# iKrishneel/fcn_object_detector

Hardware: AMD Instinct MI355X
Metric: frames/sec forward 448x448 @1 GPU; train imgs/sec @1/2/4/8 GPUs (higher is better)
Workload: dtype f32; 1 GPU; configs[1]: single-GPU forward, DetectNet GoogLeNet conv stack + coverage/bbox heads (graph of models/deploy.prototxt), batch=1, 448x448, random-init weights; global_batch=1, parallelism=replicas x1, frames_in_flight=4

## Files before the change

fcn_object_detector_amd/csrc/conv_fwd.hip:

```cpp
#include <cstddef>
#include <algorithm>
#include <mutex>
#include <unordered_map>
#include <type_traits>

#include "common.h"
#include "conv_common.h"

using namespace fcn;

namespace fcn {

const float* zero_page_for_current_device(int* rc) {
    static std::mutex mu;
    static const float* pages[64] = {nullptr};
    int dev = 0;
    *rc = 0;
    if (hipGetDevice(&dev) != hipSuccess || dev < 0 || dev >= 64) {
        *rc = set_err(FCN_E_STATE, "conv: no current device");
        return nullptr;
    }
    std::lock_guard<std::mutex> lock(mu);
    if (!pages[dev]) {
        void* ptr = nullptr;
// ... 813 lines not shown
    const bool out_f16 = (p.flags & FCN_CONV_OUT_F16) != 0;
    const bool half_out = (F16 && !out_f32) || (!F16 && out_f16);
    const bool vec = n + 3 < p.Cout && ((p.y_cstride | p.y_coffset) & 3) == 0 && ((p.y2_cstride | p.y2_coffset) & 3) == 0 &&
                     ((unsigned)(size_t)p.y & 15) == 0 && ((unsigned)(size_t)p.y2 & 15) == 0;
    const int wn_t = (4 * c4) / (32 * WTN), jt = ((4 * c4) / 32) % WTN, lc = (4 * c4) & 31;
    const float* lds_col = smem + (size_t)(wn_t * WAVES_K * WTM * WTN + jt) * 1024 + lc;
#pragma unroll 1
    for (int it = tid / C4; it < BM; it += C::NT / C4) {
        const int m = m0 + it;
        if (m >= p.M) break;
        const int wm_t = it / (32 * WTM), i_t = (it / 32) % WTM;
        const float* src = lds_col + (size_t)(wm_t * WAVES_N * WAVES_K * WTM * WTN + i_t * WTN) * 1024 + (it & 31) * 32;
        v4f v = *(const v4f*)src;
#pragma unroll
        for (int s = 1; s < WAVES_K; ++s) v += *(const v4f*)(src + (size_t)s * WTM * WTN * 1024);
#pragma unroll
        for (int e = 0; e < 4; ++e) v[e] += bias_v[e];
        const size_t o = (size_t)m * p.y_cstride + p.y_coffset + n;
        const size_t o2 = (size_t)m * p.y2_cstride + p.y2_coffset + n;
        if (half_out) {
            typedef f16_t v4h __attribute__((ext_vector_type(4)));
            f16_t* dst = reinterpret_cast<f16_t*>(p.y) + o;
            if (vec) {
                if (do_accum) { const v4h old = *(const v4h*)dst; for (int e = 0; e < 4; ++e) v[e] += (float)old[e]; }
                if (do_relu) for (int e = 0; e < 4; ++e) v[e] = fmaxf(v[e], 0.f);
                v4h h;
                for (int e = 0; e < 4; ++e) h[e] = (f16_t)v[e];
                *(v4h*)dst = h;
            } else {
                for (int e = 0; e < 4; ++e)
                    if (n + e < p.Cout) {
                        float t = v[e];
                        if (do_accum) t += (float)dst[e];
                        if (do_relu) t = fmaxf(t, 0.f);
                        dst[e] = (f16_t)t;
                    }
            }
        } else if (vec) {
            float* dst = p.y + o;
            if (do_accum) v += *(const v4f*)dst;
            if (do_relu) for (int e = 0; e < 4; ++e) v[e] = fmaxf(v[e], 0.f);
            if (do_mask) { const v4f a = *(const v4f*)(p.y2 + o2); for (int e = 0; e < 4; ++e) v[e] = a[e] > 0.f ? v[e] : 0.f; }
            *(v4f*)dst = v;
            if (do_sig2) {
                v4f sg;
                for (int e = 0; e < 4; ++e) sg[e] = 1.f / (1.f + expf(-v[e]));
                *(v4f*)(p.y2 + o2) = sg;
            }
        } else {
            for (int e = 0; e < 4; ++e)
                if (n + e < p.Cout) {
                    float t = v[e];
                    if (do_accum) t += p.y[o + e];
                    if (do_relu) t = fmaxf(t, 0.f);
                    if (do_mask) t = p.y2[o2 + e] > 0.f ? t : 0.f;
                    p.y[o + e] = t;
                    if (do_sig2) p.y2[o2 + e] = 1.f / (1.f + expf(-t));
                }
        }
    }
#ifdef FCN_CONV_STAMPS
    FCN_STAMP(5);
    wait_vmcnt<0>();
    FCN_STAMP(6);
    if (g_conv_stamps && (int)blockIdx.x < g_conv_stamps_cap && threadIdx.x == 0) {
        unsigned xcc = 0, hwid = 0;
        asm volatile("s_getreg_b32 %0, hwreg(HW_REG_XCC_ID)" : "=s"(xcc));
        asm volatile("s_getreg_b32 %0, hwreg(HW_REG_HW_ID)" : "=s"(hwid));
        g_conv_stamps[(size_t)blockIdx.x * kStampWords + 30] = xcc;
        g_conv_stamps[(size_t)blockIdx.x * kStampWords + 31] = hwid;
    }
#endif
}

__device__ __forceinline__ const GroupArgs& group_of(const GroupArgs& a) { return a; }
__device__ __forceinline__ const GroupArgs& group_of(const GroupArgsTail& a) { return a.g; }
#ifdef FCN_EXP_TAIL_NOLDS
constexpr int kTailLdsFloats = 0;
#else
constexpr int kTailLdsFloats = kTailRows * 32 + 4;
#endif

template <typename T, int WTM, int WTN, int WAVES_M, int WAVES_N, int WAVES_K, int BK, int NBUF, bool PF, bool TAIL = false>
__global__ __launch_bounds__((Cfg<WTM, WTN, WAVES_M, WAVES_N, WAVES_K, BK, NBUF, PF>::NT)) void conv_fwd_group(const int nprob, const int te0, const int te1, const int te2,
                                                                                  const int te3, const int te4, const int te5, const int te6,
                                                                                  const int te7, const int pool_wgs, const int snake,
                                                                                  const std::conditional_t<TAIL, GroupArgsTail, GroupArgs> a_) {
    __shared__ __attribute__((aligned(16))) float smem[Cfg<WTM, WTN, WAVES_M, WAVES_N, WAVES_K, BK, NBUF, PF>::LDS_FLOATS + (TAIL ? kTailLdsFloats : 0)];
    const GroupArgs& a = group_of(a_);
    typedef unsigned u32x16 __attribute__((ext_vector_type(16)));
    typedef unsigned u32x8 __attribute__((ext_vector_type(8)));
    typedef const GroupArgs __attribute__((address_space(4))) * karg_ptr;
    static_assert(alignof(GroupArgsTail) == alignof(GroupArgs) && offsetof(GroupArgsTail, g) == 0, "the group leads its tail");
    constexpr size_t kArgsOffset = (11 * sizeof(int) + alignof(GroupArgs) - 1) / alignof(GroupArgs) * alignof(GroupArgs);
    karg_ptr ka = (karg_ptr)((const char __attribute__((address_space(4)))*)__builtin_amdgcn_kernarg_segment_ptr() + kArgsOffset);
    const int head[1 + kMaxGroup] = {nprob, te0, te1, te2, te3, te4, te5, te6, te7};
    static_assert(kMaxGroup == 8, "the tile prefix travels as eight scalar kernel arguments");
    const int pool_first = pool_wgs > 0 ? pool_wgs : 0;
    if ((int)blockIdx.x < pool_first || (pool_wgs < 0 && (int)blockIdx.x >= te7)) {
        const int w = pool_wgs < 0 ? (int)blockIdx.x - te7 : (int)blockIdx.x;
        if (w < a.pool[0].wg_end) pool_body<T, Cfg<WTM, WTN, WAVES_M, WAVES_N, WAVES_K, BK, NBUF, PF>::NT>(a.pool[0], w);
        else pool_body<T, Cfg<WTM, WTN, WAVES_M, WAVES_N, WAVES_K, BK, NBUF, PF>::NT>(a.pool[1], w - a.pool[0].wg_end);
        return;
    }
    int pos = blockIdx.x;
    if (snake > 0) {
        const int sh = snake & 255, rounds = snake >> 8;
        const int r = pos >> sh, j = pos & ((1 << sh) - 1);
        if (r > 0 && r < rounds - 1 && ((rounds - 1 - r) & 1)) pos = (r << sh) + ((1 << sh) - 1 - j);
    }
    int tile = pos - pool_first;
    if (snake == (int)0x80000000) {
        const int x = pos & 7, sl = pos >> 3, q = te7 >> 3, r = te7 & 7;
        tile = x * q + (x < r ? x : r) + sl;
    } else if (snake < 0) {
        tile += snake;
        tile += tile < 0 ? te7 : 0;
    }
    int pi = 0, begin = 0;
#pragma unroll
    for (int i = 0; i < kMaxGroup - 1; ++i) {
        const int end_i = head[1 + i];
        const bool past = i + 1 < nprob && tile >= end_i;
        pi += past ? 1 : 0;
        begin = past ? end_i : begin;
    }
    u32x16 ra, rb;
    u32x8 rc;
    pi = __builtin_amdgcn_readfirstlane(pi);
    begin = __builtin_amdgcn_readfirstlane(begin);
    const ConvP __attribute__((address_space(4)))* pbase = &ka->p[pi];
    asm volatile("s_load_dwordx16 %0, %3, 0x0\n\ts_load_dwordx16 %1, %3, 0x40\n\ts_load_dwordx8 %2, %3, 0x80\n\ts_waitcnt lgkmcnt(0)"
                 : "=&s"(ra), "=&s"(rb), "=&s"(rc)
                 : "s"(pbase)
                 : "memory");
    ConvP prob;
    __builtin_memcpy((char*)&prob, &ra, 64);
    __builtin_memcpy((char*)&prob + 64, &rb, 64);
    __builtin_memcpy((char*)&prob + 128, &rc, 32);
    if constexpr (TAIL) {
        tail_kptr tp = (tail_kptr)((const char __attribute__((address_space(4)))*)ka + offsetof(GroupArgsTail, tail));
        conv_body<T, WTM, WTN, WAVES_M, WAVES_N, WAVES_K, BK, NBUF, PF, true>(prob, tile - begin, smem, tp);
    } else {
        conv_body<T, WTM, WTN, WAVES_M, WAVES_N, WAVES_K, BK, NBUF, PF>(prob, tile - begin, smem);
    }
}

template <typename T, int WTM, int WTN, int WAVES_M, int WAVES_N, int WAVES_K, int BK, int NBUF, bool PF>
__global__ __launch_bounds__((Cfg<WTM, WTN, WAVES_M, WAVES_N, WAVES_K, BK, NBUF, PF>::NT)) void conv_fwd_one(ConvP p) {
    __shared__ __attribute__((aligned(16))) float smem[Cfg<WTM, WTN, WAVES_M, WAVES_N, WAVES_K, BK, NBUF, PF>::LDS_FLOATS];
    conv_body<T, WTM, WTN, WAVES_M, WAVES_N, WAVES_K, BK, NBUF, PF>(p, blockIdx.x, smem);
}

constexpr int kD7Th = 8, kD7Tw = 32;
constexpr int kD7Ph = 2 * kD7Th + 5, kD7Pw = 2 * kD7Tw + 6;
constexpr int kD7RowF = kD7Pw * 3;
constexpr int kD7PatchF = kD7Ph * kD7RowF;
constexpr int kD7WRowF = 22, kD7WPitchF = 7 * kD7WRowF;
constexpr int kD7WOff = (kD7PatchF + 3) / 4 * 4;
constexpr int kD7EpiPitch = 68;
constexpr int kD7StageF = kD7WOff + 64 * kD7WPitchF;
constexpr int kD7EpiF = 4 * 2 * 32 * kD7EpiPitch;
constexpr int kD7LdsBytes = (kD7StageF > kD7EpiF ? kD7StageF : kD7EpiF) * 4;
constexpr int kD7Threads = 256;
static_assert(kD7LdsBytes <= 80 * 1024, "first-layer kernel: two workgroups per CU");

__global__ __launch_bounds__(kD7Threads) void conv_first7_kernel(const ConvP p) {
#if defined(__HIP_DEVICE_COMPILE__)
    __shared__ __attribute__((aligned(16))) float smem[kD7LdsBytes / 4];
    const int tid = threadIdx.x, lane = tid & 63, wave = __builtin_amdgcn_readfirstlane(tid >> 6);
    FCN_STAMP(0);
    const int tiles_x = (p.OW + kD7Tw - 1) / kD7Tw, tiles_y = (p.OH + kD7Th - 1) / kD7Th;
    int t = blockIdx.x;
    const int tx = t % tiles_x;
    t /= tiles_x;
    const int ty = t % tiles_y, n = t / tiles_y;
    const int oy0 = ty * kD7Th, ox0 = tx * kD7Tw;
    const int iy0 = 2 * oy0 - 3, ix0 = 2 * ox0 - 3;
    const v4f zero4 = {0.f, 0.f, 0.f, 0.f};
    constexpr int PI = (kD7Ph * kD7Pw + kD7Threads - 1) / kD7Threads, WI = (64 * 49 + kD7Threads - 1) / kD7Threads;
    v4f px[PI], wv[WI];
    const float* xn = p.x + (size_t)n * p.H * p.W * 4;
#pragma unroll
    for (int i = 0; i < PI; ++i) {
        const int s = tid + kD7Threads * i;
        const int pr = s / kD7Pw, pc = s - pr * kD7Pw;
        const int iy = iy0 + pr, ix = ix0 + pc;
        const bool ok = s < kD7Ph * kD7Pw && (unsigned)iy < (unsigned)p.H && (unsigned)ix < (unsigned)p.W;
        px[i] = ok ? *reinterpret_cast<const v4f*>(xn + ((size_t)iy * p.W + ix) * 4) : zero4;
    }
#pragma unroll
    for (int i = 0; i < WI; ++i) {
        const int tp = tid + kD7Threads * i;
        wv[i] = tp < p.Cout * 49 ? *reinterpret_cast<const v4f*>(p.w + (size_t)tp * 4) : zero4;
    }
#pragma unroll
    for (int i = 0; i < PI; ++i) {
        const int s = tid + kD7Threads * i;
        if (s < kD7Ph * kD7Pw) {
            float* d = smem + s * 3;
            d[0] = px[i][0]; d[1] = px[i][1]; d[2] = px[i][2];
        }
    }
#pragma unroll
    for (int i = 0; i < WI; ++i) {
        const int tp = tid + kD7Threads * i;
        if (tp < 64 * 49) {
            const int co = tp / 49, rq = tp - co * 49;
            const int r = rq / 7, q = rq - r * 7;
            float* d = smem + kD7WOff + co * kD7WPitchF + r * kD7WRowF + q * 3;
            d[0] = wv[i][0]; d[1] = wv[i][1]; d[2] = wv[i][2];
        }
    }
    for (int i = tid; i < 64 * 7; i += kD7Threads) smem[kD7WOff + i * kD7WRowF + 21] = 0.f;
    const int c4 = (lane & 15) * 4;
    const v4f bias_v = (p.bias && c4 < p.Cout) ? *reinterpret_cast<const v4f*>(p.bias + c4) : zero4;
    FCN_STAMP(1);
    const int nl = lane & 31, h = lane >> 5;
    const float* a_base = smem + (4 * wave) * kD7RowF + 6 * nl + h;
    const float* b_base = smem + kD7WOff + nl * kD7WPitchF + h;
    typedef float v16f __attribute__((ext_vector_type(16)));
    v16f acc[2][2];
#pragma unroll
    for (int i = 0; i < 2; ++i)
#pragma unroll
        for (int j = 0; j < 2; ++j)
#pragma unroll
            for (int e = 0; e < 16; ++e) acc[i][j][e] = 0.f;
    __syncthreads();
    FCN_STAMP(2);
    auto frag = [&](const int step, float (&a)[2], float (&b)[2]) {
        const int r = step / 11, j = step - 11 * r;
#pragma unroll
        for (int mt = 0; mt < 2; ++mt) a[mt] = a_base[(2 * mt + r) * kD7RowF + 2 * j];
#pragma unroll
        for (int nt = 0; nt < 2; ++nt) b[nt] = b_base[nt * 32 * kD7WPitchF + r * kD7WRowF + 2 * j];
    };
    float fa[3][2], fb[3][2];
    frag(0, fa[0], fb[0]);
    frag(1, fa[1], fb[1]);
#pragma unroll
    for (int step = 0; step < 77; ++step) {
        if (step + 2 < 77) frag(step + 2, fa[(step + 2) % 3], fb[(step + 2) % 3]);
        __builtin_amdgcn_sched_barrier(0);
#pragma unroll
        for (int mt = 0; mt < 2; ++mt)
#pragma unroll
            for (int nt = 0; nt < 2; ++nt)
                acc[mt][nt] = __builtin_amdgcn_mfma_f32_32x32x2f32(fa[step % 3][mt], fb[step % 3][nt], acc[mt][nt], 0, 0, 0);
    }
    FCN_STAMP(3);
    __syncthreads();
    float* epi = smem + wave * (2 * 32 * kD7EpiPitch);
#pragma unroll
    for (int mt = 0; mt < 2; ++mt)
#pragma unroll
        for (int nt = 0; nt < 2; ++nt)
#pragma unroll
            for (int v = 0; v < 16; ++v) epi[(mt * 32 + (v & 3) + 8 * (v >> 2) + 4 * h) * kD7EpiPitch + nl + 32 * nt] = acc[mt][nt][v];
    asm volatile("s_waitcnt lgkmcnt(0)" ::: "memory");
    __builtin_amdgcn_sched_barrier(0);
    const bool do_relu = (p.flags & FCN_CONV_RELU) != 0;
#pragma unroll
    for (int mt = 0; mt < 2; ++mt) {
        const int oy = oy0 + 2 * wave + mt;
        float* yrow = p.y + ((size_t)(n * p.OH + oy) * p.OW + ox0) * p.y_cstride + p.y_coffset + c4;
#pragma unroll
        for (int i = 0; i < 8; ++i) {
            const int ox = (lane >> 4) + 4 * i;
            v4f v = *reinterpret_cast<const v4f*>(epi + (mt * 32 + ox) * kD7EpiPitch + c4) + bias_v;
            if (do_relu)
#pragma unroll
                for (int e = 0; e < 4; ++e) v[e] = fmaxf(v[e], 0.f);
            if (oy < p.OH && ox0 + ox < p.OW && c4 < p.Cout) *reinterpret_cast<v4f*>(yrow + (size_t)ox * p.y_cstride) = v;
        }
    }
#ifdef FCN_CONV_STAMPS
    FCN_STAMP(5);
    wait_vmcnt<0>();
    FCN_STAMP(6);
#endif
#endif
}

constexpr int kH7PatchSlots = (kD7Ph * kD7Pw + 63) / 64 * 64;
constexpr int kH7EpiOff = 2 * kH7PatchSlots * 16;
constexpr int kH7EpiPitch = 144;
constexpr int kH7LdsBytes = kH7EpiOff + 4 * 64 * kH7EpiPitch;
static_assert(kH7LdsBytes <= 160 * 1024, "half-float first-layer kernel: LDS image");

__global__ __launch_bounds__(kD7Threads) void conv_first7_f16_kernel(const ConvP p, const int ntiles) {
#if defined(__HIP_DEVICE_COMPILE__)
    __shared__ __attribute__((aligned(16))) char smem[kH7LdsBytes];
    const int tid = threadIdx.x, lane = tid & 63, wave = __builtin_amdgcn_readfirstlane(tid >> 6);
    const int tiles_x = (p.OW + kD7Tw - 1) / kD7Tw, tiles_y = (p.OH + kD7Th - 1) / kD7Th;
    const f16_t* xh = reinterpret_cast<const f16_t*>(p.x);
    const f16_t* wh = reinterpret_cast<const f16_t*>(p.w);
    f16_t* yh = reinterpret_cast<f16_t*>(p.y);
    const v4f zero4 = {0.f, 0.f, 0.f, 0.f};
    constexpr int PI = (kD7Ph * kD7Pw + kD7Threads - 1) / kD7Threads;
    auto fetch_patch = [&](const int tile, v4f (&px)[PI]) {
        int t = tile;
        const int tx = t % tiles_x;
        t /= tiles_x;
        const int ty = t % tiles_y, n = t / tiles_y;
        const int iy0 = 2 * ty * kD7Th - 3, ix0 = 2 * tx * kD7Tw - 3;
// ... 557 lines not shown
    }
    return best;
}

int plan_tiles_cfg(int cfg, ConvP* ps, int n) {
    if (cfg == kDot1x1Cfg) {
        if (!dot1x1_ok(ps, n)) return -2;
        for (int i = 0; i < n; ++i) {
            ps[i].tiles_m = cdiv(ps[0].M, kDotPx);
            ps[i].tiles_n = 1;
            ps[i].tiles_n_magic = 0;
            ps[i].lean_chunks = 0;
            ps[i].tile_end = ps[i].tiles_m;
        }
        return ps[0].tiles_m;
    }
    if (cfg == kFirst7Cfg) {
        if (n != 1 || !(first7_ok(ps[0]) || first7_f16_ok(ps[0]))) return -2;
        ps[0].tiles_m = ps[0].N * cdiv(ps[0].OH, kD7Th) * cdiv(ps[0].OW, kD7Tw);
        ps[0].tiles_n = 1;
        ps[0].tiles_n_magic = 0;
        ps[0].lean_chunks = 0;
        ps[0].tile_end = ps[0].tiles_m;
        return ps[0].tiles_m;
    }
    if (is_stream_cfg(cfg)) {
        const StreamCfgInfo sc = stream_cfg_info(cfg - kStreamCfg0);
        int total = 0;
        for (int i = 0; i < n; ++i) {
            ConvP& q = ps[i];
            const long long xb = (((long long)q.N * q.H * q.W - 1) * q.x_cstride + q.Cin) * 2, wb = (long long)q.Cout * q.K * 2;
            const long long yb = (((long long)q.M - 1) * q.y_cstride + q.y_coffset + q.Cout) * 2;
            const int k = q.kh, pw = q.W + 2 * q.pad;
            const int wraps = (sc.bm - 2 + q.W) / q.W;
            const int rows = sc.bm - 1 + 2 * q.pad * wraps + 2 * q.pad + 1;
            if ((q.flags & ~FCN_CONV_RELU) != FCN_CONV_F16 || (q.Cout | q.y_cstride | q.y_coffset) % 8 != 0 || ((uintptr_t)q.y & 15) != 0 ||
                ((uintptr_t)q.bias & 15) != 0 || xb >= (1ll << 31) || wb >= (1ll << 31) || yb >= (1ll << 31) ||
                q.kh != q.kw || (k != 1 && k != 3 && k != 5) || q.stride != 1 || q.pad != (k - 1) / 2 || rows > sc.slab_rows ||
                (k == 1 && sc.slab_buffers < 3) || pw < 16 || (long long)q.N * q.H * pw * pw >= (1ll << 32))
                return -2;
            q.tiles_m = cdiv(q.M, sc.bm);
            q.tiles_n = cdiv(q.Cout, sc.bn);
            q.tiles_n_magic = q.tiles_n > 1 ? (unsigned)(((1ull << 32) + q.tiles_n - 1) / q.tiles_n) : 0u;
            total += q.tiles_m * q.tiles_n;
            q.tile_end = total;
            static const bool pack_ok = !(getenv("FCN_STREAM_PACK") && atoi(getenv("FCN_STREAM_PACK")) == 0);
            int tsh = 0;
            if (pack_ok && k > 1 && q.x_cstride == q.Cin && ((uintptr_t)q.x & 15) == 0) tsh = q.Cin == 16 ? 2 : q.Cin == 32 ? 1 : 0;
            if (tsh && cdiv(k, 1 << tsh) < 2) tsh = 0;
            q.lean_chunks = tsh;
            q.cin_magic24 = (unsigned)(((1ull << 32) + pw - 1) / pw);
        }
        return total;
    }
    const int bm = kCfgs[cfg].bm, bn = kCfgs[cfg].bn;
    if (n > 1) std::stable_sort(ps, ps + n, [&](const ConvP& a, const ConvP& b) { return cdiv(a.K, kCfgs[cfg].bk) > cdiv(b.K, kCfgs[cfg].bk); });
    static const bool lean_ok = !(getenv("FCN_CONV_LEAN") && atoi(getenv("FCN_CONV_LEAN")) == 0);
    int total = 0;
    for (int i = 0; i < n; ++i) {
        ps[i].tiles_m = cdiv(ps[i].M, bm);
        ps[i].tiles_n = cdiv(ps[i].Cout, bn);
        const long long tl = (long long)ps[i].tiles_m * ps[i].tiles_n;
        if (tl * ps[i].tiles_n >= (1ll << 32)) return -1;
        ps[i].tiles_n_magic = ps[i].tiles_n > 1 ? (unsigned)(((1ull << 32) + ps[i].tiles_n - 1) / ps[i].tiles_n) : 0u;
        total += ps[i].tiles_m * ps[i].tiles_n;
        ps[i].tile_end = total;
        const int esz = (ps[i].flags & FCN_CONV_F16) ? 2 : 4;
        const int bke = kCfgs[cfg].bk * 4 / esz;
        const int taps = ps[i].kh * ps[i].kw, cpt = cdiv(ps[i].Cin, bke);
        const long long xb = (((long long)ps[i].N * ps[i].H * ps[i].W - 1) * ps[i].x_cstride + ps[i].Cin) * esz;
        const long long wb = (long long)ps[i].Cout * ps[i].K * esz;
        const bool lean = lean_ok && xb < (1ll << 31) && wb < (1ll << 31) && taps <= 31 && (taps == 1 || 2ll * cpt * bke <= 3ll * ps[i].Cin);
        ps[i].lean_chunks = lean ? taps * cpt : 0;
        static const int light_min = getenv("FCN_CONV_LIGHT") ? atoi(getenv("FCN_CONV_LIGHT")) : 4;
        ps[i].kw_magic = (65536 + ps[i].kw - 1) / ps[i].kw;
        const bool big_tile = bm * bn > 32 * 32;
        if (lean && kCfgRoles[cfg] && light_min > 0 && (taps == 1 || cpt >= light_min || big_tile)) ps[i].kw_magic = -1;
    }
    return total;
}

int device_cus() {
    static int cached[64] = {};
    int dev = 0;
    if (hipGetDevice(&dev) != hipSuccess || dev < 0 || dev >= 64) return 256;
    if (cached[dev] == 0) {
        int v = 0;
        cached[dev] = (hipDeviceGetAttribute(&v, hipDeviceAttributeMultiprocessorCount, dev) == hipSuccess && v > 0) ? v : 256;
    }
    return cached[dev];
}

template <typename T>
void launch_one_cfg(int cfg, const ConvP& p, int total, hipStream_t st) {
    if (cfg == kFirst7Cfg) {
        if (p.flags & FCN_CONV_F16) {
            static const bool x4_ok = !(getenv("FCN_FIRST7_X4") && atoi(getenv("FCN_FIRST7_X4")) == 0);
            const bool small = (long long)p.N * p.H * p.W * 16 < (1ll << 31) &&
                               (((long long)p.N * p.OH * p.OW - 1) * p.y_cstride + p.y_coffset + p.Cout) * 2 < (1ll << 31);
            if ((p.flags & FCN_CONV_IMAGE_ONES) && x4_ok && small) {
                const int grid = total < 2 * device_cus() ? total : 2 * device_cus();
                hipLaunchKernelGGL(conv_first7_f16x4_kernel, dim3(grid), dim3(kD7Threads), 0, st, p, total);
                return;
            }
            const int grid = total < device_cus() ? total : device_cus();
            hipLaunchKernelGGL(conv_first7_f16_kernel, dim3(grid), dim3(kD7Threads), 0, st, p, total);
        } else {
            hipLaunchKernelGGL(conv_first7_kernel, dim3(total), dim3(kD7Threads), 0, st, p);
        }
        return;
    }
    switch (cfg) {
#define X(I, A, B, C_, D, E, F, G, H)                                                                                                 \
    case I:                                                                                                                           \
        hipLaunchKernelGGL((conv_fwd_one<T, A, B, C_, D, E, F, G, H>), dim3(total), dim3(Cfg<A, B, C_, D, E, F, G, H>::NT), 0, st, p); \
        break;
        FCN_CONV_CONFIGS(X)
#undef X
    }
}

template <typename T>
void launch_group_cfg(int cfg, const GroupArgs& ga, int pool_wgs, int snake, int total, hipStream_t st) {
    switch (cfg) {
#define X(I, A, B, C_, D, E, F, G, H)                                                                                                     \
    case I:                                                                                                                               \
        hipLaunchKernelGGL((conv_fwd_group<T, A, B, C_, D, E, F, G, H>), dim3(total), dim3(Cfg<A, B, C_, D, E, F, G, H>::NT), 0, st, ga.nprob,      \
                           ga.tile_end[0], ga.tile_end[1], ga.tile_end[2], ga.tile_end[3], ga.tile_end[4], ga.tile_end[5], ga.tile_end[6],          \
                           ga.tile_end[7], pool_wgs, snake, ga);                                                                                   \
        break;
        FCN_CONV_CONFIGS(X)
#undef X
    }
}

constexpr bool tail_cfg_ok(int cfg) { return cfg == 23 || cfg == 24 || cfg == 25 || cfg == 27; }
void launch_group_tail(int cfg, const GroupArgsTail& ga, int pool_wgs, int snake, int total, hipStream_t st) {
    const GroupArgs& g = ga.g;
    switch (cfg) {
#define XT(I, A, B, C_, D, E, F, G, H)                                                                                                         \
    case I:                                                                                                                                    \
        hipLaunchKernelGGL((conv_fwd_group<float, A, B, C_, D, E, F, G, H, true>), dim3(total), dim3(Cfg<A, B, C_, D, E, F, G, H>::NT), 0, st, g.nprob, \
                           g.tile_end[0], g.tile_end[1], g.tile_end[2], g.tile_end[3], g.tile_end[4], g.tile_end[5], g.tile_end[6],             \
                           g.tile_end[7], pool_wgs, snake, ga);                                                                                \
        break;
        XT(23, 1, 1, 1, 1, 4, 32, 16 + 4, true)
        XT(24, 1, 1, 1, 1, 4, 64, 16 + 4, true)
        XT(25, 1, 1, 2, 1, 2, 32, 16 + 4, true)
        XT(27, 1, 1, 1, 1, 4, 32, 16 + 6, true)
#undef XT
    }
}

struct HostTail { bool on; int finalize; int n; fcn_conv_desc heads[kTailMaxSlices]; float* scratch; unsigned* arrive; TailP t; };
struct HostGroup { int n; ConvP ps[16]; int npool; PoolP pools[kMaxPool]; HostTail tail; };
std::unordered_map<const void*, HostTail> g_tails;
std::mutex g_groups_mu;
std::unordered_map<const void*, HostGroup> g_groups;

}

extern "C" {

#ifdef FCN_CONV_STAMPS
int fcn_debug_conv_stamps(void* d_buf, int cap) {
    FCN_HIP(hipMemcpyToSymbol(HIP_SYMBOL(g_conv_stamps), &d_buf, sizeof(d_buf)));
    FCN_HIP(hipMemcpyToSymbol(HIP_SYMBOL(g_conv_stamps_cap), &cap, sizeof(cap)));
    return 0;
}
#endif

int fcn_conv2d_fwd_f32(const fcn_conv_desc* h_desc, fcn_stream_t s) {
    FCN_REQUIRE(h_desc, FCN_E_ARG, "fcn_conv2d_fwd_f32: null desc");
    int rc = validate(*h_desc);
    if (rc) return rc;
    const float* zp = zero_page_for_current_device(&rc);
    if (rc) return rc;
    ConvP p;
    fill(p, *h_desc, zp);
    const int cfg = choose_cfg(&p, 1);
    const int total = plan_tiles_cfg(cfg, &p, 1);
    FCN_REQUIRE(total > 0, FCN_E_UNSUPPORTED, "conv: too many tiles for the 32-bit tile decode");
    if (h_desc->flags & FCN_CONV_F16) launch_one_cfg<f16_t>(cfg, p, total, as_stream(s));
    else launch_one_cfg<float>(cfg, p, total, as_stream(s));
    FCN_LAUNCH_CHECK("conv_fwd_one");
    return 0;
}

size_t fcn_conv2d_group_workspace_bytes(int n) { return sizeof(ConvP) * (size_t)(n > 0 ? n : 0); }

int fcn_conv2d_num_configs(void) { return num_cfgs(); }

int fcn_conv2d_first_layer_config(void) { return kFirst7Cfg; }

int fcn_conv2d_config_lds_bytes(int cfg) {
    if (is_stream_cfg(cfg)) return stream_cfg_info(cfg - kStreamCfg0).lds_bytes;
    return cfg == kFirst7Cfg ? kD7LdsBytes :       cfg == kDot1x1Cfg ? kDotMaxSlices * kDotRedPx * kDotOut * kDotRedPitch * 4 : cfg >= 0 && cfg < kNumTileCfg ? kCfgLdsBytes[cfg] : -1;
}

int fcn_conv2d_config_waves_k(int cfg) { return cfg == kFirst7Cfg || cfg == kDot1x1Cfg || is_stream_cfg(cfg) ? 1 : cfg >= 0 && cfg < kNumTileCfg ? kCfgWavesK[cfg] : -1; }

int fcn_conv2d_group_prepare(const fcn_conv_desc* h_descs, int n, void* d_workspace, int cfg_request, fcn_conv_group* h_out) {
    return fcn_conv2d_group_prepare_fused(h_descs, n, nullptr, 0, d_workspace, cfg_request, h_out);
}

int fcn_conv2d_group_prepare_fused(const fcn_conv_desc* h_descs, int n, const fcn_pool_desc* h_pools, int npools, void* d_workspace,
                                   int cfg_request, fcn_conv_group* h_out) {
    FCN_REQUIRE(h_descs && h_out && d_workspace && n > 0 && n <= 16, FCN_E_ARG, "fcn_conv2d_group_prepare: need 1..16 problems, workspace, out");
    FCN_REQUIRE(cfg_request >= -1 && cfg_request < num_cfgs(), FCN_E_ARG, "fcn_conv2d_group_prepare: tile configuration %d out of range", cfg_request);
    FCN_REQUIRE(npools >= 0 && npools <= kMaxPool && (npools == 0 || (h_pools && n <= kMaxGroup)), FCN_E_ARG,
                "fcn_conv2d_group_prepare_fused: at most %d poolings, and only beside at most %d convolutions", kMaxPool, kMaxGroup);
    ConvP ps[16];
    int zrc = 0;
    const float* zp = zero_page_for_current_device(&zrc);
    if (zrc) return zrc;
    for (int i = 0; i < n; ++i) {
        int rc = validate(h_descs[i]);
        if (rc) return rc;
        FCN_REQUIRE(((h_descs[i].flags ^ h_descs[0].flags) & FCN_CONV_F16) == 0, FCN_E_ARG, "conv group: f32 and f16 problems cannot share a launch");
        fill(ps[i], h_descs[i], zp);
    }
    const int group_f16 = (h_descs[0].flags & FCN_CONV_F16) ? 1 : 0;
    PoolP pools[kMaxPool] = {};
    for (int i = 0; i < npools; ++i) {
        const fcn_pool_desc& d = h_pools[i];
        FCN_REQUIRE(d.x && d.y && d.N > 0 && d.H > 0 && d.W > 0 && d.C > 0 && d.k > 0 && d.stride > 0 && d.pad >= 0 && d.pad < d.k && d.OH > 0 &&
                        d.OW > 0, FCN_E_ARG, "fused maxpool: bad args");
        FCN_REQUIRE((d.OH - 1) * d.stride - d.pad < d.H && (d.OW - 1) * d.stride - d.pad < d.W, FCN_E_ARG,
                    "fused maxpool: last window starts outside the image");
        const int peps = group_f16 ? 8 : 4;
        FCN_REQUIRE((d.f16 ? 1 : 0) == group_f16, FCN_E_ARG, "fused maxpool: element type differs from the group's convolutions");
        FCN_REQUIRE(d.C % peps == 0 && d.x_cstride % peps == 0 && d.y_cstride % peps == 0 && d.y_coffset % peps == 0 && d.x_cstride >= d.C &&
                        d.y_coffset >= 0 && d.y_cstride >= d.y_coffset + d.C, FCN_E_ALIGN, "fused maxpool: channels / strides must be multiples of %d", peps);
        FCN_REQUIRE((((uintptr_t)d.x | (uintptr_t)d.y | (uintptr_t)d.idx) & 15) == 0, FCN_E_ALIGN, "fused maxpool: pointers must be 16-byte aligned");
        FCN_REQUIRE((long long)d.N * d.OH * d.OW * (d.C / peps) < (1ll << 30), FCN_E_UNSUPPORTED, "fused maxpool: too large");
        PoolP& q = pools[i];
        q.x = d.x; q.y = d.y; q.idx = d.idx;
        q.N = d.N; q.H = d.H; q.W = d.W; q.C = d.C; q.x_cstride = d.x_cstride; q.k = d.k; q.stride = d.stride; q.pad = d.pad;
        q.OH = d.OH; q.OW = d.OW; q.y_cstride = d.y_cstride; q.y_coffset = d.y_coffset;
        q.items = d.N * d.OH * d.OW * (d.C / peps);
        q.wg_end = 0;
    }
    HostTail tail = {};
    {
        std::lock_guard<std::mutex> lock(g_groups_mu);
        auto it = g_tails.find(d_workspace);
        if (it != g_tails.end()) tail = it->second;
    }
    if (tail.on) {
        const fcn_conv_desc& h0 = tail.heads[0];
        int contributors = 0;
        FCN_REQUIRE(n <= kMaxGroup && !group_f16, FCN_E_UNSUPPORTED, "conv tail: at most %d float32 problems in the launch", kMaxGroup);
        for (int i = 0; i < n; ++i) {
            const ConvP& q = ps[i];
            if ((const float*)q.y != h0.x) continue;
            FCN_REQUIRE(q.y_cstride == h0.x_cstride && q.M == h0.N * h0.H * h0.W && q.Cout % 32 == 0 && q.y_coffset % 32 == 0 && q.y_coffset + q.Cout <= h0.Cin &&
                            (q.flags & ~FCN_CONV_RELU) == 0 && ((uintptr_t)q.y & 15) == 0 && q.y_cstride % 4 == 0 && (!q.bias || ((uintptr_t)q.bias & 15) == 0),
                        FCN_E_UNSUPPORTED, "conv tail: a producer of the narrow problems' input must be a float32 bias + ReLU convolution over the same pixels "
                                           "that writes whole 32-channel groups of it");
            ps[i].flags |= FCN_CONV_TAILF;
            ++contributors;
        }
        FCN_REQUIRE(contributors > 0, FCN_E_ARG, "conv tail: no problem of this group writes the narrow problems' input");
    }
    int cfg = cfg_request >= 0 ? cfg_request : choose_cfg(ps, n);
    if (tail.on && cfg_request < 0 && !tail_cfg_ok(cfg)) cfg = 23;
    FCN_REQUIRE(!tail.on || tail_cfg_ok(cfg), FCN_E_UNSUPPORTED, "conv tail: configuration %d has no tail variant (23, 24, 25, 27 do)", cfg);
    const int total = plan_tiles_cfg(cfg, ps, n);
    if (tail.on && total > 0) {
        TailP& t = tail.t;
        t = TailP{};
        t.h.scratch = tail.scratch;
        t.h.arrive = tail.arrive;
        t.h.K = tail.heads[0].Cin;
        t.h.M = tail.heads[0].N * tail.heads[0].H * tail.heads[0].W;
        t.h.nslices = tail.n;
        int rows = 0;
        for (int i = 0; i < tail.n; ++i) {
            const fcn_conv_desc& h = tail.heads[i];
            TailSlice& sl = t.s[i];
            sl.bias = h.bias; sl.y = h.y; sl.y2 = h.y2;
            sl.o0 = rows; sl.nout = h.Cout; sl.y_cstride = h.y_cstride; sl.y_coffset = h.y_coffset; sl.y2_cstride = h.y2_cstride; sl.y2_coffset = h.y2_coffset;
            sl.flags = h.flags;
            for (int r = 0; r < h.Cout; r += 4) t.h.gw[(rows + r) / 4] = h.w + (size_t)r * h.Cin;
            rows += h.Cout;
        }
        for (int j = rows / 4; j < kTailRows / 4; ++j) t.h.gw[j] = t.h.gw[0];
        t.h.rows = rows;
        t.h.dbg = getenv("FCN_TAIL_DEBUG") ? atoi(getenv("FCN_TAIL_DEBUG")) : 0;
        t.h.need = 0;
        if (tail.finalize)
            for (int i = 0; i < n; ++i)
                if (ps[i].flags & FCN_CONV_TAILF) t.h.need += ps[i].tiles_n;
    }
    FCN_REQUIRE(!(is_stream_cfg(cfg) && (total == -2 || npools || n > kMaxGroup)), FCN_E_UNSUPPORTED,
                "conv group: configuration %d (persistent half-float streaming kernel) takes at most %d half problems with half outputs, "
                "bias + ReLU only, Cout / y_cstride / y_coffset multiples of 8, stride-1 1x1 / 3x3 / 5x5 filters with pad (k - 1) / 2 on images wide "
                "enough for its slab buffer (1x1 filters: the configurations with three slab buffers), and no poolings", cfg, kMaxGroup);
    FCN_REQUIRE(total != -2 && !((cfg == kFirst7Cfg || cfg == kDot1x1Cfg) && npools), FCN_E_UNSUPPORTED,
                "conv group: configuration %d is shape-specific (%d: one 7x7 / stride 2 / pad 3 problem on 4-channel pixels, 33..64 outputs; "
                "%d: 1x1 / stride 1 float32 problems over the same pixels, at most 32 output channels in slices of 8) and takes no poolings",
                cfg, kFirst7Cfg, kDot1x1Cfg);
    FCN_REQUIRE(total > 0, FCN_E_UNSUPPORTED, "conv group: too many tiles for the 32-bit tile decode");
    FCN_HIP(hipMemcpy(d_workspace, ps, sizeof(ConvP) * n, hipMemcpyHostToDevice));
    {
        std::lock_guard<std::mutex> lock(g_groups_mu);
        HostGroup& hg = g_groups[d_workspace];
        hg.n = n;
        for (int i = 0; i < n; ++i) hg.ps[i] = ps[i];
        hg.npool = npools;
        for (int i = 0; i < kMaxPool; ++i) hg.pools[i] = pools[i];
        hg.tail = tail;
    }
    h_out->d_probs = d_workspace;
    h_out->n = n;
    h_out->cfg = cfg;
    h_out->total_tiles = total;
    return 0;
}

int fcn_conv2d_group_release(void* d_workspace) {
    std::lock_guard<std::mutex> lock(g_groups_mu);
    g_groups.erase(d_workspace);
    g_tails.erase(d_workspace);
    return 0;
}

namespace {
int tail_check(const fcn_conv_tail* t) {
    FCN_REQUIRE(t && t->n >= 1 && t->n <= kTailMaxSlices, FCN_E_ARG, "conv tail: 1..%d narrow problems", kTailMaxSlices);
    int rows = 0;
    const fcn_conv_desc& h0 = t->heads[0];
    for (int i = 0; i < t->n; ++i) {
        const fcn_conv_desc& h = t->heads[i];
        int rc = validate(h);
        if (rc) return rc;
        FCN_REQUIRE(h.kh == 1 && h.kw == 1 && h.stride == 1 && h.pad == 0 && (h.flags & ~(FCN_CONV_RELU | FCN_CONV_SIGMOID2)) == 0, FCN_E_UNSUPPORTED,
                    "conv tail: the narrow problems are float32 1x1 / stride 1 convolutions (bias, ReLU, sigmoid second output)");
        FCN_REQUIRE(h.x == h0.x && h.x_cstride == h0.x_cstride && h.Cin == h0.Cin && h.N == h0.N && h.H == h0.H && h.W == h0.W, FCN_E_ARG,
                    "conv tail: the narrow problems read the same blob");
        FCN_REQUIRE(h.Cout % 4 == 0 && h.Cin % 32 == 0 && h.Cin <= 1024 && h.y_cstride % 4 == 0 && h.y_coffset % 4 == 0 && ((uintptr_t)h.y & 15) == 0 &&
                        (!h.bias || ((uintptr_t)h.bias & 15) == 0) && (!h.y2 || (((uintptr_t)h.y2 & 15) == 0 && h.y2_cstride % 4 == 0 && h.y2_coffset % 4 == 0)),
                    FCN_E_UNSUPPORTED, "conv tail: outputs in whole, 16-byte aligned groups of four channels; input channels in whole groups of 32, at most 1024");
        rows += h.Cout;
    }
    FCN_REQUIRE(rows <= kTailRows, FCN_E_UNSUPPORTED, "conv tail: at most %d output channels in all", kTailRows);
    return 0;
}
}

size_t fcn_conv2d_tail_scratch_bytes(const fcn_conv_tail* t) {
    if (tail_check(t)) return 0;
    size_t rows = 0;
    for (int i = 0; i < t->n; ++i) rows += (size_t)t->heads[i].Cout;
    return (size_t)(t->heads[0].Cin / 32) * (size_t)t->heads[0].N * t->heads[0].H * t->heads[0].W * rows * sizeof(float);
}

size_t fcn_conv2d_tail_arrive_bytes(const fcn_conv_tail* t) {
    if (tail_check(t)) return 0;
    return ((size_t)t->heads[0].N * t->heads[0].H * t->heads[0].W / 32 + 1) * sizeof(unsigned);
}

int fcn_conv2d_group_attach_tail(void* d_workspace, const fcn_conv_tail* t) {
    FCN_REQUIRE(d_workspace, FCN_E_ARG, "fcn_conv2d_group_attach_tail: null workspace");
    if (!t) {
        std::lock_guard<std::mutex> lock(g_groups_mu);
        g_tails.erase(d_workspace);
        return 0;
    }
    int rc = tail_check(t);
    if (rc) return rc;
    FCN_REQUIRE(t->scratch && t->arrive && ((uintptr_t)t->scratch & 15) == 0, FCN_E_ARG, "fcn_conv2d_group_attach_tail: scratch (16-byte aligned) and arrival words");
    HostTail ht = {};
    ht.on = true;
    ht.finalize = t->finalize ? 1 : 0;
    ht.n = t->n;
    for (int i = 0; i < t->n; ++i) ht.heads[i] = t->heads[i];
    ht.scratch = t->scratch;
    ht.arrive = reinterpret_cast<unsigned*>(t->arrive);
    std::lock_guard<std::mutex> lock(g_groups_mu);
    g_tails[d_workspace] = ht;
    return 0;
}

int fcn_conv2d_fwd_group_f32(const fcn_conv_group* g, fcn_stream_t s) {
    FCN_REQUIRE(g && g->d_probs && g->n > 0 && g->total_tiles > 0, FCN_E_ARG, "fcn_conv2d_fwd_group_f32: unprepared group");
    FCN_REQUIRE(g->cfg >= 0 && g->cfg < num_cfgs(), FCN_E_ARG, "fcn_conv2d_fwd_group_f32: bad cfg %d", g->cfg);
    HostGroup hg;
    {
        std::lock_guard<std::mutex> lock(g_groups_mu);
        auto it = g_groups.find(g->d_probs);
        FCN_REQUIRE(it != g_groups.end() && it->second.n == g->n, FCN_E_STATE, "fcn_conv2d_fwd_group_f32: group was not prepared by this library instance");
        hg = it->second;
    }
    if (g->cfg == kDot1x1Cfg) {
        FCN_REQUIRE(hg.npool == 0 && dot1x1_ok(hg.ps, hg.n), FCN_E_STATE, "fcn_conv2d_fwd_group_f32: group was not prepared for the lane-split 1x1 kernel");
        DotArgs da = {};
        da.M = hg.ps[0].M;
        for (int i = 0; i < hg.n; ++i)
            for (int n0 = 0; n0 < hg.ps[i].Cout; n0 += kDotOut) {
                const ConvP& q = hg.ps[i];
                DotSlice& d = da.s[da.nslices++];
                d.x = q.x; d.w = q.w + (size_t)n0 * q.K; d.bias = q.bias ? q.bias + n0 : nullptr; d.y = q.y; d.y2 = q.y2;
                d.K = q.K; d.x_cstride = q.x_cstride; d.y_cstride = q.y_cstride; d.y_coffset = q.y_coffset + n0;
                d.y2_cstride = q.y2_cstride; d.y2_coffset = q.y2_coffset + n0;
                d.nout = q.Cout - n0 < kDotOut ? q.Cout - n0 : kDotOut;
                d.flags = q.flags;
            }
        hipLaunchKernelGGL(conv_dot1x1_kernel, dim3(g->total_tiles), dim3(64 * kDotMaxSlices), 0, as_stream(s), da);
        FCN_LAUNCH_CHECK("conv_dot1x1");
        return 0;
    }
    if (g->cfg == kFirst7Cfg) {
        FCN_REQUIRE(hg.n == 1 && hg.npool == 0 && (first7_ok(hg.ps[0]) || first7_f16_ok(hg.ps[0])), FCN_E_STATE,
                    "fcn_conv2d_fwd_group_f32: group was not prepared for the first-layer kernel");
        launch_one_cfg<float>(kFirst7Cfg, hg.ps[0], g->total_tiles, as_stream(s));
        FCN_LAUNCH_CHECK("conv_first7");
        return 0;
    }
    if (is_stream_cfg(g->cfg)) {
        FCN_REQUIRE(hg.npool == 0 && hg.n <= kMaxGroup && (hg.ps[0].flags & FCN_CONV_F16), FCN_E_STATE, "fcn_conv2d_fwd_group_f32: group was not prepared for the streaming kernel");
        GroupArgs ga;
        ga.npool = 0;
        for (int i = 0; i < kMaxPool; ++i) ga.pool[i] = PoolP{};
        ga.nprob = hg.n;
        for (int i = 0; i < kMaxGroup; ++i) {
            const ConvP& src = hg.ps[i < hg.n ? i : hg.n - 1];
            ga.p[i] = src;
            ga.tile_end[i] = src.tile_end;
        }
        launch_stream(g->cfg - kStreamCfg0, ga, g->total_tiles, as_stream(s));
        FCN_LAUNCH_CHECK("conv_stream_f16");
        return 0;
    }
    for (int first = 0; first < hg.n; first += kMaxGroup) {
        GroupArgs ga;
        ga.npool = 0;
        for (int i = 0; i < kMaxPool; ++i) ga.pool[i] = PoolP{};
        ga.nprob = hg.n - first < kMaxGroup ? hg.n - first : kMaxGroup;
        const int base = first ? hg.ps[first - 1].tile_end : 0;
        for (int i = 0; i < kMaxGroup; ++i) {
            const ConvP& src = hg.ps[first + (i < ga.nprob ? i : ga.nprob - 1)];
            ga.p[i] = src;
            ga.tile_end[i] = src.tile_end - base;
        }
        int grid = ga.tile_end[ga.nprob - 1];
        int pool_wgs = 0;
        if (hg.npool > 0) {
            int end = 0;
            ga.npool = hg.npool;
            for (int i = 0; i < kMaxPool; ++i) {
                ga.pool[i] = hg.pools[i < hg.npool ? i : hg.npool - 1];
                const int per_wg = kCfgThreads[g->cfg] * (ga.pool[i].items <= kPoolSmallItems ? 1 : kPoolItemsPerThread);
                if (i < hg.npool) end += (ga.pool[i].items + per_wg - 1) / per_wg;
                ga.pool[i].wg_end = end;
            }
            grid += end;
            static const bool pool_last = getenv("FCN_POOL_LAST") && atoi(getenv("FCN_POOL_LAST")) == 1;
            pool_wgs = pool_last ? -end : end;
        }
        int snake = 0;
        {
            static const bool snake_ok = !(getenv("FCN_CONV_SNAKE") && atoi(getenv("FCN_CONV_SNAKE")) == 0);
            const int cus = device_cus();
            if (snake_ok && ga.nprob > 1 && (cus & (cus - 1)) == 0 && grid > 2 * cus && pool_wgs >= 0 && pool_wgs < cus) {
                int sh = 0;
                while ((1 << sh) < cus) ++sh;
                snake = ((grid + cus - 1) / cus) << 8 | sh;
            } else if (getenv("FCN_CONV_XCD") && atoi(getenv("FCN_CONV_XCD")) == 1 && pool_wgs == 0 && first == 0 && hg.n <= kMaxGroup) {
                snake = (int)0x80000000;
            } else if (snake_ok && ga.nprob > 1 && pool_wgs == 0 && grid > cus && grid <= 2 * cus) {
                snake = -(grid - cus);
            }
        }
        if (hg.tail.on) {
            FCN_REQUIRE(tail_cfg_ok(g->cfg) && hg.n <= kMaxGroup, FCN_E_STATE, "fcn_conv2d_fwd_group_f32: group was not prepared with its tail");
            GroupArgsTail gt;
            gt.g = ga;
            gt.tail = hg.tail.t;
            launch_group_tail(g->cfg, gt, pool_wgs, snake, grid, as_stream(s));
        } else if (hg.ps[0].flags & FCN_CONV_F16) launch_group_cfg<f16_t>(g->cfg, ga, pool_wgs, snake, grid, as_stream(s));
        else launch_group_cfg<float>(g->cfg, ga, pool_wgs, snake, grid, as_stream(s));
        FCN_LAUNCH_CHECK("conv_fwd_group");
    }
    return 0;
}

}
```

fcn_object_detector_amd/detector.py:

```python
from __future__ import annotations

import ctypes as C
import os
import math
from typing import Dict, List, Optional, Sequence, Tuple

import numpy as np

from . import lib as L
from .engine import DeviceBuffer, Engine, PinnedArray, replica_streams

F32 = np.float32


class HeadMapping:

    def __init__(self, cvg_blob: str, bbox_blob: str, stride: int, skip_background: bool):
        self.cvg_blob, self.bbox_blob, self.stride, self.skip_background = cvg_blob, bbox_blob, int(stride), bool(skip_background)

    @classmethod
    def reference_node(cls) -> "HeadMapping":
        return cls("pool_score", "upscore_pool5_bbox", 8, True)

    @classmethod
# ... 262 lines not shown
                offs.append(off)
                off += f.nbytes if same else (f.nbytes + 15) // 16 * 16
            L.call("fcn_memcpy_h2d_async", self._frame_dev.ptr, stage.ctypes.data, off, eng.stream)
            self._enqueue_batch(self._frame_dev.ptr, [(o, f.shape[0], f.shape[1]) for o, f in zip(offs, frames)], same)
            self._outstanding = [f.shape for f in frames]

    def _enqueue_batch(self, dev_ptr: int, layout: Sequence[Tuple[int, int, int]], same: bool) -> None:
        eng = self.engine
        data = eng.blobs["data"]
        if same:
            L.call("fcn_preprocess_bgr8_batch", dev_ptr, len(layout), layout[0][1], layout[0][2], data.ptr, self._half_flag(data),
                   self.im_height, self.im_width, data.cstride, data.upload_shift, self._minmax_batch_holder[0].ptr, eng.stream)
        else:
            for i, (off, h, w) in enumerate(layout):
                L.call("fcn_preprocess_bgr8_batch", dev_ptr + off, 1, h, w, data.ptr + data.esize * i * self.im_height * self.im_width * data.cstride,
                       self._half_flag(data), self.im_height, self.im_width, data.cstride, data.upload_shift, self._minmax.ptr, eng.stream)
        eng.forward_enqueue()
        self.decoder.launch(*self._cvg_args, *self._box_args, eng.stream)
        self.decoder.fetch_begin(eng.stream)
        data.host_valid = False

    def run_detector2(self, frame: np.ndarray, stride: int = 2) -> Tuple[np.ndarray, List[Tuple[np.ndarray, np.ndarray]]]:
        eng = self.engine
        frame = np.ascontiguousarray(frame, np.uint8)
        if frame.ndim != 3 or frame.shape[2] != 3:
            raise ValueError("expected a BGR uint8 frame")
        rects = detection_window_roi(frame.shape, stride)
        if len(rects) != self.batch:
            raise ValueError("stride %d makes %d windows; the engine's batch is %d" % (stride, len(rects), self.batch))
        if getattr(self, "_outstanding", None) is not None:
            raise RuntimeError("a batch is already in flight: collect it first")
        h, w, _c = frame.shape
        with eng.lock:
            L.call("fcn_init", eng.device)
            if self._frame_dev is None or self._frame_dev.nbytes < frame.nbytes:
                self._frame_dev = DeviceBuffer(frame.nbytes, zero=False)
                self._frame_pinned = PinnedArray(((frame.nbytes + 3) // 4,))
            stage = self._frame_pinned.array.view(np.uint8)[:frame.nbytes]
            stage[...] = frame.reshape(-1)
            data = eng.blobs["data"]
            L.call("fcn_memcpy_h2d_async", self._frame_dev.ptr, stage.ctypes.data, frame.nbytes, eng.stream)
            L.call("fcn_preprocess_bgr8_rois", self._frame_dev.ptr, h, w, rects.ctypes.data, len(rects), data.ptr, self._half_flag(data),
                   self.im_height, self.im_width, data.cstride, data.upload_shift, self._minmax.ptr, eng.stream)
            eng.forward_enqueue()
            self.decoder.launch(*self._cvg_args, *self._box_args, eng.stream)
            self.decoder.fetch_begin(eng.stream)
            data.host_valid = False
            res = self.decoder.fetch(eng.stream, begun=True)
        out = []
        for (x, y, rw, rh), (dets, labels) in zip(rects.tolist(), res):
            boxes = np.asarray(dets, dtype=np.int64).reshape(-1, 5)
            if len(boxes):
                boxes = resize_detection((rh, rw), boxes, self.im_width, self.im_height)
                boxes[:, 0] += x; boxes[:, 2] += x
                boxes[:, 1] += y; boxes[:, 3] += y
            out.append((boxes, labels))
        return rects, out

    def run_detector2_masks(self, frame: np.ndarray, stride: int = 1, score_blob: str = "score", padding: int = 10):
        eng = self.engine
        frame = np.ascontiguousarray(frame, np.uint8)
        if frame.ndim != 3 or frame.shape[2] != 3:
            raise ValueError("expected a BGR uint8 frame")
        rects = detection_window_roi(frame.shape, stride)
        if len(rects) != self.batch:
            raise ValueError("stride %d makes %d windows; the engine's batch is %d" % (stride, len(rects), self.batch))
        sb = eng.blobs[score_blob]
        if sb.esize != 4 or len(sb.shape) != 4:
            raise NotImplementedError("score blob %s must be a 4-d float32 blob" % score_blob)
        h, w, _c = frame.shape
        _n, C_, sh, sw = sb.shape
        key = (len(rects), C_, int(rects[0][2]), int(rects[0][3]), h, w)
        if getattr(self, "_score_masks_key", None) != key:
            self._score_masks = ScoreMasks(*key)
            self._score_masks_key = key
        with eng.lock:
            L.call("fcn_init", eng.device)
            if self._frame_dev is None or self._frame_dev.nbytes < frame.nbytes:
                self._frame_dev = DeviceBuffer(frame.nbytes, zero=False)
                self._frame_pinned = PinnedArray(((frame.nbytes + 3) // 4,))
            stage = self._frame_pinned.array.view(np.uint8)[:frame.nbytes]
            stage[...] = frame.reshape(-1)
            data = eng.blobs["data"]
            L.call("fcn_memcpy_h2d_async", self._frame_dev.ptr, stage.ctypes.data, frame.nbytes, eng.stream)
            L.call("fcn_preprocess_bgr8_rois", self._frame_dev.ptr, h, w, rects.ctypes.data, len(rects), data.ptr, self._half_flag(data),
                   self.im_height, self.im_width, data.cstride, data.upload_shift, self._minmax.ptr, eng.stream)
            eng.forward_enqueue()
            for op in eng._lazy_blob_ops.get(score_blob, ()):
                op.run(eng.stream)
            self._score_masks.launch(sb.buf.ptr, sh, sw, sb.cstride, sb.coffset, rects, self.prob_thresh, eng.stream)
            data.host_valid = False
            return self._score_masks.fetch(eng.stream, padding)

    def collect_batch(self) -> List[Tuple[np.ndarray, np.ndarray]]:
        if getattr(self, "_outstanding", None) is None:
            raise RuntimeError("no batch in flight")
        shapes, self._outstanding = self._outstanding, None
        with self.engine.lock:
            res = self.decoder.fetch(self.engine.stream, begun=True)
        out = []
        for shape, (dets, labels) in zip(shapes, res):
            boxes = np.asarray(dets, dtype=np.int64).reshape(-1, 5)
            out.append((resize_detection(shape, boxes, self.im_width, self.im_height) if len(boxes) else boxes, labels))
        return out

    def submit(self, frame: np.ndarray) -> None:
        eng = self.engine
        if self.batch != 1:
            raise ValueError("run_detector handles one frame; build the engine with batch 1")
        if getattr(self, "_outstanding", None) is not None:
            raise RuntimeError("a frame is already in flight: collect() it first")
        frame = np.ascontiguousarray(frame, np.uint8)
        if frame.ndim != 3 or frame.shape[2] != 3:
            raise ValueError("expected a BGR uint8 frame")
        h, w, _c = frame.shape
        with eng.lock:
            L.call("fcn_init", eng.device)
            if self._frame_dev is None or self._frame_dev.nbytes < frame.nbytes:
                self._frame_dev = DeviceBuffer(frame.nbytes, zero=False)
                self._frame_pinned = PinnedArray(((frame.nbytes + 3) // 4,))
            stage = self._frame_pinned.array.view(np.uint8)[:frame.nbytes]
            stage[...] = frame.reshape(-1)
            data = eng.blobs["data"]
            L.call("fcn_memcpy_h2d_async", self._frame_dev.ptr, stage.ctypes.data, frame.nbytes, eng.stream)
            L.call("fcn_preprocess_bgr8_batch", self._frame_dev.ptr, 1, h, w, data.ptr, self._half_flag(data), self.im_height, self.im_width,
                   data.cstride, data.upload_shift, self._minmax.ptr, eng.stream)
            eng.forward_enqueue()
            self.decoder.launch(*self._cvg_args, *self._box_args, eng.stream)
            self.decoder.fetch_begin(eng.stream)
            data.host_valid = False
            self._outstanding = frame.shape

    def collect(self) -> Tuple[np.ndarray, np.ndarray]:
        if getattr(self, "_outstanding", None) is None:
            raise RuntimeError("no frame in flight")
        shape, self._outstanding = self._outstanding, None
        with self.engine.lock:
            dets, labels = self.decoder.fetch(self.engine.stream, begun=True)[0]
        boxes = np.asarray(dets, dtype=np.int64).reshape(-1, 5)
        if not len(boxes):
            return boxes, labels
        return resize_detection(shape, boxes, self.im_width, self.im_height), labels

    def run_detector(self, frame: np.ndarray) -> Tuple[np.ndarray, np.ndarray]:
        self.submit(frame)
        return self.collect()


class DetectorPipeline:

    def __init__(self, make_engine, depth: int = 3, **detector_kw):
        self.detectors: List[FCNObjectDetector] = []
        first = None
        with replica_streams():
            for _ in range(max(int(depth), 1)):
                eng = make_engine(first)
                first = first or eng
                self.detectors.append(FCNObjectDetector(eng, **detector_kw))
        self._queue: List[FCNObjectDetector] = []
        self._next = 0

    def submit(self, frame: np.ndarray) -> None:
        if len(self._queue) >= len(self.detectors):
            raise RuntimeError("DetectorPipeline: %d frames already in flight" % len(self._queue))
        d = self.detectors[self._next]
        self._next = (self._next + 1) % len(self.detectors)
        d.submit(frame)
        self._queue.append(d)

    def collect(self) -> Tuple[np.ndarray, np.ndarray]:
        if not self._queue:
            raise RuntimeError("DetectorPipeline: nothing in flight")
        return self._queue.pop(0).collect()

    def run_detector_batches(self, batches) -> List[List[Tuple[np.ndarray, np.ndarray]]]:
        out, queue, nxt = [], [], 0
        for frames in batches:
            if len(queue) == len(self.detectors):
                out.append(queue.pop(0).collect_batch())
            d = self.detectors[nxt]
            nxt = (nxt + 1) % len(self.detectors)
            d.submit_batch(frames)
            queue.append(d)
        while queue:
            out.append(queue.pop(0).collect_batch())
        return out

    def run_detector_stream(self, frames) -> List[Tuple[np.ndarray, np.ndarray]]:
        out = []
        for f in frames:
            if len(self._queue) == len(self.detectors):
                out.append(self.collect())
            self.submit(f)
        while self._queue:
            out.append(self.collect())
        return out

    def close(self) -> None:
        for d in self.detectors:
            d.engine.close()
```

fcn_object_detector_amd/engine.py:

```python
from __future__ import annotations

import ctypes as C
import os
import threading
from collections import namedtuple
from dataclasses import dataclass, field
from typing import Callable, Dict, List, Optional, Sequence, Tuple, Union

import numpy as np

from . import lib as L
from . import region as RG
from . import ssd as SSD
from . import storage as S
from . import tune as T
from .netspec import Layer, NetSpec, bn_global_stats, crop_window, interp_size, is_rectangular, kernel_stride_pad, layer_dilation, layer_geometry
from .storage import _r4, _ra, ip_pack_bank, ip_unpack_bank

F32 = np.float32


def graphs_enabled() -> bool:
    return os.environ.get("FCN_NO_GRAPH", "0") in ("", "0")


_replica_ctx = threading.local()


class replica_streams:

    def __enter__(self) -> "replica_streams":
        self._outer = getattr(_replica_ctx, "next", None)
        _replica_ctx.next = 0
        return self

    def __exit__(self, *exc) -> None:
        _replica_ctx.next = self._outer


def _take_replica_index() -> Optional[int]:
    i = getattr(_replica_ctx, "next", None)
    if i is not None:
        _replica_ctx.next = i + 1
    return i


def dropout_layer_salt(spec: NetSpec, l: Layer) -> int:
    k = [q.name for q in spec.layers if q.type == "Dropout"].index(l.name)
    return (k << 28) & 0xFFFFFFFF


class ConvGeom(namedtuple("ConvGeom", "n cin h w cout oh ow k s pad")):
    __slots__ = ()

    @property
    def flops(self) -> float:
        return 2.0 * self.n * self.cout * self.oh * self.ow * self.cin * self.k * self.k

    def swapped(self) -> "ConvGeom":
        return self._replace(cin=self.cout, h=self.oh, w=self.ow, cout=self.cin, oh=self.h, ow=self.w)


def conv_desc(x: "Blob", y: "Blob", g: ConvGeom, w: Optional[int] = None, bias: Optional[int] = None, flags: int = 0) -> L.ConvDesc:
    d = L.ConvDesc()
    d.x, d.w, d.bias, d.y = x.ptr, w, bias, y.buf.ptr
    d.N, d.H, d.W, d.Cin, d.x_cstride = g.n, g.h, g.w, g.cin, x.cstride
    d.Cout, d.kh, d.kw, d.pad, d.stride, d.OH, d.OW = g.cout, g.k, g.k, g.pad, g.s, g.oh, g.ow
    d.y_cstride, d.y_coffset = y.cstride, y.coffset
    d.flags = flags
    return d


def tconv_desc(a: "Blob", b: "Blob", g: ConvGeom, bank: int, bias: Optional[int] = None, flags: int = 0) -> L.TConvDesc:
    d = L.TConvDesc()
    d.a, d.w, d.bias, d.b = a.ptr, bank, bias, b.buf.ptr
    d.N, d.H, d.W, d.Ca, d.a_cstride = g.n, g.h, g.w, g.cin, a.cstride
    d.Cb, d.kh, d.kw, d.pad, d.stride, d.OH, d.OW = g.cout, g.k, g.k, g.pad, g.s, g.oh, g.ow
    d.b_cstride, d.b_coffset = b.cstride, b.coffset
    d.flags = flags
    return d


class RectGeom(namedtuple("RectGeom", "n cin h w cout oh ow kh kw sh sw ph pw d")):
    __slots__ = ()

    @property
    def flops(self) -> float:
        return 2.0 * self.n * self.oh * self.ow * self.cin * self.cout * self.kh * self.kw

    @property
    def bytes(self) -> float:
        return 4.0 * (self.n * self.cin * self.h * self.w + self.n * self.cout * self.oh * self.ow + self.cout * self.cin * self.kh * self.kw + self.cout)

    def swapped(self) -> "RectGeom":
        return self._replace(cin=self.cout, h=self.oh, w=self.ow, cout=self.cin, oh=self.h, ow=self.w)


def rconv_desc(x: "Blob", y: "Blob", g: RectGeom, w: Optional[int] = None, bias: Optional[int] = None, flags: int = 0) -> L.RConvDesc:
    d = L.RConvDesc()
    d.x, d.w, d.bias, d.y = x.ptr, w, bias, y.buf.ptr
    d.N, d.H, d.W, d.Cin, d.x_cstride = g.n, g.h, g.w, g.cin, x.cstride
    d.Cout, d.kh, d.kw, d.pad_h, d.pad_w, d.stride_h, d.stride_w, d.OH, d.OW = g.cout, g.kh, g.kw, g.ph, g.pw, g.sh, g.sw, g.oh, g.ow
    d.y_cstride, d.y_coffset = y.cstride, y.coffset
    d.flags, d.dilation = flags, g.d
    return d


class DwGeom(namedtuple("DwGeom", "n c h w oh ow kh kw sh sw ph pw d")):
    __slots__ = ()

    @property
    def flops(self) -> float:
        return 2.0 * self.n * self.oh * self.ow * self.c * self.kh * self.kw

    @property
    def bytes(self) -> float:
        return 4.0 * (self.n * self.h * self.w * self.c + self.n * self.oh * self.ow * self.c + self.kh * self.kw * self.c + self.c)


def dwconv_desc(x: "Blob", y: "Blob", g: DwGeom, w: Optional[int] = None, bias: Optional[int] = None, flags: int = 0) -> L.DwConvDesc:
    return L.dwconv_desc(x.ptr, w, bias, y.buf.ptr, g.n, g.h, g.w, g.c, x.cstride, g.kh, g.kw, g.ph, g.pw, g.sh, g.sw, g.d,
                         y.cstride, y.coffset, flags)


class DeviceBuffer:

    def __init__(self, nbytes: int, zero: bool = True):
        p = C.c_void_p()
        L.call("fcn_malloc", C.byref(p), nbytes)
        self.ptr = int(p.value)
        self.nbytes = int(nbytes)
        if zero:
            L.call("fcn_memset_async", self.ptr, 0, self.nbytes, None)
            L.call("fcn_device_sync")

    def free(self) -> None:
        if getattr(self, "ptr", 0):
            try:
                L.load().fcn_free(self.ptr)
            finally:
                self.ptr = 0

    def __del__(self):
        try:
            self.free()
        except Exception:
            pass


class DevView:

    __slots__ = ("ptr", "nbytes")

    def __init__(self, ptr: int, nbytes: int):
        self.ptr, self.nbytes = int(ptr), int(nbytes)


class PinnedArray:

    def __init__(self, shape: Tuple[int, ...]):
        n = int(np.prod(shape)) if len(shape) else 1
        p = C.c_void_p()
        L.call("fcn_host_malloc", C.byref(p), max(n, 1) * 4)
        self.ptr = int(p.value)
        buf = (C.c_float * max(n, 1)).from_address(self.ptr)
        self.array = np.frombuffer(buf, dtype=F32, count=n).reshape(shape)
        self.array[...] = 0

    def free(self) -> None:
        if getattr(self, "ptr", 0):
            self.array = None
            try:
                L.load().fcn_host_free(self.ptr)
            finally:
                self.ptr = 0

    def __del__(self):
        try:
            self.free()
        except Exception:
            pass


class Blob:

    def __init__(self, name: str, shape: Tuple[int, ...]):
        self.name = name
        self.shape = tuple(shape)
        self.buf: Optional[DeviceBuffer] = None
        self.coffset = 0
        self.cstride = 0
        self.esize = 4
        self.lazy_shift = 0.0
        self.upload_shift = 0.0
        self.host: Optional[np.ndarray] = None
        self.pinned: Optional[PinnedArray] = None
        self.host_valid = False
        self.is_input = False
        self.rows = False

    @property
    def nchw(self) -> Optional[Tuple[int, int, int, int]]:
        return S.blob_nchw(self.shape, self.rows)

    @property
    def channels(self) -> int:
        return self.nchw[1] if self.nchw is not None else 1

    @property
    def pixels(self) -> int:
        g = self.nchw
        return g[0] * g[2] * g[3] if g is not None else 1

    @property
    def ptr(self) -> int:
        return self.buf.ptr + self.esize * self.coffset

    @property
    def contiguous(self) -> bool:
        return self.coffset == 0 and self.cstride == self.channels


class Op:

    def __init__(self, kind: str, name: str, run: Callable[[Optional[int]], None], flops: float = 0.0, bytes_: float = 0.0):
        self.kind = kind
        self.name = name
        self.run = run
        self.flops = flops
        self.bytes = bytes_


Range = Tuple[int, int, int]


@dataclass(eq=False)
class ConvTask:
    layer: Layer
    desc: L.ConvDesc
    flops: float
    bytes: float
    reads: List[Range]
    writes: List[Range]


@dataclass(eq=False)
class OpTask:
    layer: Layer
    ops: List[Op]
    reads: List[Range]
    writes: List[Range]
    pool_desc: Optional[L.PoolDesc] = None
    rconv: Optional[L.RConvDesc] = None
    dwconv: Optional[L.DwConvDesc] = None


Task = Union[ConvTask, OpTask]


@dataclass(eq=False)
class BnChain:
    x: str
    y: str
    bn: Optional[Layer] = None
    scale: Optional[Layer] = None
    relu: Optional[Layer] = None
    mids: List[str] = field(default_factory=list)
    save: Optional["DeviceBuffer"] = None
    global_stats: bool = False


def ranges_hit(a: Sequence[Range], b: Sequence[Range]) -> bool:
    return any(x[0] == y[0] and x[1] < y[2] and y[1] < x[2] for x in a for y in b)


def task_waits(later: Task, earlier: Task) -> bool:
    return ranges_hit(later.reads, earlier.writes) or ranges_hit(later.writes, earlier.writes) or ranges_hit(later.writes, earlier.reads)


def task_levels(tasks: Sequence[Task], group_convs: bool = True) -> List[int]:
    levels: List[int] = []
    for i, ti in enumerate(tasks):
        levels.append(max([levels[j] + 1 for j in range(i) if task_waits(ti, tasks[j])], default=0) if group_convs else i)
    return levels


def task_floats(tasks: Sequence[Task], levels: Sequence[int], i: int) -> bool:
    return not any(levels[j] == levels[i] + 1 and task_waits(tj, tasks[i]) for j, tj in enumerate(tasks) if j != i)


class Engine:

    def __init__(self, spec: NetSpec, data_shapes: Optional[Dict[str, Tuple[int, ...]]] = None,
                 params: Optional[Dict[str, List[np.ndarray]]] = None, device: int = 0,
                 fuse: bool = True, group_convs: bool = True, autotune: bool = True, dtype: str = "f32",
                 tune_from: Optional["Engine"] = None, tune_max_lds_kb: Optional[int] = None,
                 share_params: Optional["Engine"] = None, score_outputs: bool = False, replica: Optional[int] = None):
        if dtype not in ("f32", "f16"):
            raise ValueError("dtype must be 'f32' or 'f16'")
        if share_params is not None and (dtype != "f32" or share_params.f16):
            raise NotImplementedError("share_params: only between float32 engines (a half-float engine packs its weights differently)")
        self._share_from = share_params
        self.shared_layers: set = set()
        self.score_outputs = bool(score_outputs)
        self.score_acc: Dict[str, DeviceBuffer] = {}
        self.graph_score: Optional[int] = None
        if dtype == "f16" and spec.phase != "TEST":
            raise NotImplementedError("the half-float path is inference only (BASELINE configs[4])")
        self.dtype, self.f16 = dtype, dtype == "f16"
        self.spec = spec
        self.device = device
        self.fuse = fuse
        self.group_convs = group_convs
        self.autotune = autotune
        L.call("fcn_init", device)
        sp = C.c_void_p()
        self.replica = replica if replica is not None else _take_replica_index()
        if self.replica is None:
            L.call("fcn_stream_create", C.byref(sp))
        else:
            L.call("fcn_stream_create_replica", C.byref(sp), int(self.replica))
        self.stream = int(sp.value)
        yes = C.c_int(0)
        L.call("fcn_stream_is_prioritized", self.stream, C.byref(yes))
        self.stream_prioritized = bool(yes.value)
        self.lock = threading.RLock()
        self.shapes = spec.infer(data_shapes)
        self.blobs: Dict[str, Blob] = {}
        self.params_host: Dict[str, List[np.ndarray]] = {}
        self.params_dev: Dict[str, List[DevView]] = {}
        self.ops: List[Op] = []
        self.graph_io: Optional[int] = None
        self.graph_core: Optional[int] = None
        self._staging: Dict[str, DeviceBuffer] = {}
        self._keep: List[object] = []
        self._conv_layer_meta: Dict[str, dict] = {}
        self._group_workspaces: List[DeviceBuffer] = []
        self.aux_dev: Dict[str, DeviceBuffer] = {}
        self._bn_chains: Dict[str, BnChain] = {}
        self._bn_ws_bytes = 0
        self._bn_ws: Optional[DeviceBuffer] = None
        self._lazy_blob_ops: Dict[str, List[Op]] = {}
        self.loss_blobs: Dict[str, float] = {}
        self.device_fed: set = set()
        self.dropout_seed = 0
        self.dropout_index_offset = 0
        self.inputs = spec.data_tops()
        self.outputs = [b for b in spec.output_blobs() if b in self.shapes and b not in spec.mask_blobs]
        max_lds = int(tune_max_lds_kb if tune_max_lds_kb is not None else os.environ.get("FCN_TUNE_MAX_LDS_KB", "160")) * 1024
        self.tuner = T.Tuner(self.stream, T.key_suffix(self.shapes.get(self.inputs[0], ()) if self.inputs else None, self.f16, max_lds),
                             spec.phase == "TEST", max_lds, tune_from._chosen_cfgs if tune_from is not None else None)
        self._plan_buffers()
        self._alloc_params(params)
        self._build_ops()
        self.tuner.release()

    @property
    def _chosen_cfgs(self) -> Dict[str, object]:
        return self.tuner.chosen

    def _plan_buffers(self) -> None:
        plan = S.plan_blobs(self.spec, self.shapes, self.inputs, self.outputs, self.f16, self.fuse, os.environ.get("FCN_F16_IMAGE", "1") != "0")
        self.producers, self.consumers = plan.producers, plan.consumers
        self.alias, self.shift, self.copy_concats, self.copy_slices = plan.alias, plan.shift, plan.copy_concats, plan.copy_slices
        self._half_inputs = plan.half_inputs
        self.permutes, self.gathers, self.detections = plan.permutes, plan.gathers, plan.detections
        self.pair_softmax, self.rpn_views = plan.pair_softmax, plan.rpn_views
        self.roi_counts: Dict[str, DeviceBuffer] = {}
        self._roi_count_host: Dict[str, "PinnedArray"] = {}
        self._roi_caps: Dict[str, int] = {}
        self._counts_valid = False
        bufs = {root: DeviceBuffer(nbytes) for root, nbytes in plan.root_bytes.items()}
        for name, v in plan.views.items():
            b = self.blobs[name] = Blob(name, v.shape)
            b.esize, b.rows, b.is_input = v.esize, v.rows, name in self.inputs
            b.buf, b.coffset, b.cstride = bufs[v.root], v.coffset, v.cstride
            b.upload_shift, b.lazy_shift = v.upload_shift, v.lazy_shift
        self._upload_priors()
        for d in self._half_inputs:
            b = self.blobs[d]
            ones = np.zeros((b.pixels, b.cstride), np.float16)
            ones[:, 3:5] = 1.0
            L.call("fcn_memcpy_h2d_async", b.buf.ptr, ones.ctypes.data, ones.nbytes, None)
            L.call("fcn_device_sync")

    def _upload_priors(self) -> None:
        self.prior_consts: Dict[str, np.ndarray] = {}
        for name, l in self.spec.prior_blobs.items():
            if l.type == "PriorBox":
                _, _, fh, fw = self.shapes[l.bottoms[0]]
                _, _, dh, dw = self.shapes[l.bottoms[1]]
                a = SSD.prior_boxes(SSD.priorbox_params(l), fh, fw, dh, dw)
            else:
                a = np.concatenate([self.prior_consts[b] for b in l.bottoms], axis=2)
            if a.shape != tuple(self.shapes[name]):
                raise RuntimeError("layer %s: %s prior constants for the blob %s" % (l.name, a.shape, self.shapes[name]))
            self.prior_consts[name] = a = np.ascontiguousarray(a, F32)
            b = self.blobs[name]
            if b.coffset or b.cstride != a.size:
                raise NotImplementedError("layer %s: the prior blob %s is a window of another buffer" % (l.name, name))
            L.call("fcn_memcpy_h2d_async", b.buf.ptr, a.ctypes.data, a.nbytes, None)
            L.call("fcn_device_sync")

    def _alloc_params(self, params: Optional[Dict[str, List[np.ndarray]]]) -> None:
        from .netspec import fill_params
        if params is None:
            params = fill_params(self.spec, seed=0)
        self.param_segs: Dict[Tuple[str, int], S.ParamSeg] = {}
        src = self._share_from
        if src is not None:
            self._shared_keep = [src.param_flat] + list(getattr(src, "_shared_keep", []))
            for l in self.spec.param_layers():
                if l.name not in src.params_dev:
                    continue
                mine, theirs = [tuple(x) for x in self.spec.param_shapes[l.name]], [tuple(x) for x in src.spec.param_shapes[l.name]]
                if mine != theirs:
                    raise ValueError("share_params: layer %s has blobs %s here and %s in the source net" % (l.name, mine, theirs))
                self.shared_layers.add(l.name)
                self.params_host[l.name] = src.params_host[l.name]
                self.params_dev[l.name] = [DevView(v.ptr, v.nbytes) for v in src.params_dev[l.name]]
                self.param_segs.update({(l.name, i): src.param_segs[(l.name, i)] for i in range(len(mine))})
        self.param_layout, self.param_count = S.param_layout(self.spec, self.blobs, self.f16, self.shared_layers)
        for l in self.spec.param_layers():
            if l.name in self.shared_layers:
                continue
            shapes = self.spec.param_shapes[l.name]
            blobs = params.get(l.name)
            if blobs is None:
                raise KeyError("no parameters for layer %s" % l.name)
            host = []
            for arr, shp in zip(blobs, shapes):
                a = np.ascontiguousarray(arr, dtype=F32)
                if a.shape != tuple(shp):
                    if a.size != int(np.prod(shp)):
                        raise ValueError("layer %s: parameter shape %s does not match %s" % (l.name, a.shape, shp))
                    a = a.reshape(shp)
                host.append(a.copy())
            self.params_host[l.name] = host
        self.param_flat = DeviceBuffer(max(self.param_count, 4) * 4, zero=True)
        for seg in self.param_layout:
            self.param_segs[(seg.layer, seg.index)] = seg
            self.params_dev.setdefault(seg.layer, []).append(DevView(self.param_flat.ptr + 4 * seg.offset, seg.nbytes))
        for l in self.spec.param_layers():
            if l.name not in self.shared_layers:
                self._upload_params(l)

    def _folded_shift(self, l: Layer) -> float:
        return next((sh for t, sh in self._half_inputs.values() if t == l.bottoms[0]), 0.0) if l.type == "Convolution" else 0.0

    def _upload_params(self, l: Layer) -> None:
        if l.name in self.shared_layers:
            raise RuntimeError("layer %s reads the parameters of another engine (share_params): set them there" % l.name)
        packed = [S.pack(self.param_segs[(l.name, i)], h, self._folded_shift(l) if i == 0 else 0.0) for i, h in enumerate(self.params_host[l.name])]
        for arr, dev in zip(packed, self.params_dev[l.name]):
            L.call("fcn_memcpy_h2d_async", dev.ptr, arr.ctypes.data, arr.nbytes, None)
        L.call("fcn_device_sync")

    def set_params(self, layer: str, blobs: Sequence[np.ndarray]) -> None:
        lay = next(l for l in self.spec.layers if l.name == layer)
        if layer in self.shared_layers:
            raise RuntimeError("layer %s reads the parameters of another engine (share_params): set them there" % layer)
        shapes = self.spec.param_shapes[layer]
        self.params_host[layer] = [np.ascontiguousarray(b, dtype=F32).reshape(s).copy() for b, s in zip(blobs, shapes)]
        self._upload_params(lay)

    def read_param(self, layer: str, index: int) -> np.ndarray:
        with self.lock:
# ... 372 lines not shown
            return [OpTask(l, [Op("pair_softmax", l.name, run, 0.0, 16.0 * pix * a)], reads=[self._range(src)], writes=[self._range(dst)])]
        if t == "Proposal":
            pp = RG.proposal_params(l)
            RG.proposal_shapes(l, [self.shapes[b] for b in l.bottoms])
            sb, db, ib = (B[b] for b in l.bottoms)
            rb = B[l.tops[0]]
            tb = B[l.tops[1]] if len(l.tops) > 1 else None
            if any(x.esize != 4 for x in (sb, db, ib)) or rb.cstride < rb.coffset + 8 or (tb is not None and tb.cstride < tb.coffset + 4):
                raise NotImplementedError("layer %s: a top of Proposal is a channel window that ends inside a 16-byte group" % l.name)
            base = RG.anchors(pp.base_size, pp.ratios, pp.scales).astype(F32).reshape(-1)
            par = L.ProposalParams()
            par.H, par.W, par.A, par.feat_stride = sb.shape[2], sb.shape[3], base.size // 4, pp.feat_stride
            par.pre_nms_topn, par.post_nms_topn, par.min_size, par.nms_thresh = pp.pre_nms_topn, pp.post_nms_topn, pp.min_size, pp.nms_thresh
            par.score_cstride, par.score_coffset, par.delta_cstride, par.delta_coffset = sb.cstride, sb.coffset, db.cstride, db.coffset
            par.rois_cstride, par.rois_coffset = rb.cstride, rb.coffset
            par.top_score_cstride, par.top_score_coffset = (tb.cstride, tb.coffset) if tb is not None else (0, 0)
            for i, v in enumerate(base):
                par.anchors[i] = float(v)
            nbytes = int(lib.fcn_proposal_workspace_bytes(C.byref(par)))
            if nbytes <= 0:
                L.check(lib.fcn_proposal_f32(None, None, None, C.byref(par), None, None, None, None, 0, None))
                raise RuntimeError("layer %s: Proposal has no plan" % l.name)
            ws, cnt = DeviceBuffer(nbytes, zero=True), DeviceBuffer(16, zero=True)
            self.roi_counts[l.name], self._roi_caps[l.name] = cnt, pp.post_nms_topn
            self._keep.extend([ws, par])
            m, k = par.H * par.W * par.A, min(pp.pre_nms_topn, par.H * par.W * par.A)
            run = lambda st: L.check(lib.fcn_proposal_f32(sb.buf.ptr, db.buf.ptr, ib.ptr, C.byref(par), rb.buf.ptr, tb.buf.ptr if tb is not None else None,
                                                          cnt.ptr, ws.ptr, nbytes, st))
            return [OpTask(l, [Op("proposal", l.name, run, 30.0 * m + 2.0 * m * m + 20.0 * k * k / 2, 24.0 * m + 8.0 * m * ((m + 255) // 256) + k * k / 4.0)],
                           reads=[self._range(b) for b in l.bottoms], writes=[self._range(tp) for tp in l.tops])]
        xb, rb, yb = B[l.bottoms[0]], B[l.bottoms[1]], B[l.tops[0]]
        if any(x.esize != 4 for x in (xb, rb, yb)) or yb.cstride < yb.coffset + _r4(yb.channels):
            raise NotImplementedError("layer %s: the top %s is a channel window that ends inside a 16-byte group" % (l.name, l.tops[0]))
        n, c, h, w = xb.nchw
        r = rb.shape[0]
        if t == "ROIPooling":
            rp = RG.roi_pool_params(l)
            run = lambda st: L.check(lib.fcn_roi_pool_fwd_f32(xb.buf.ptr, rb.buf.ptr, yb.buf.ptr, None, n, h, w, c, xb.cstride, xb.coffset, r, rb.cstride,
                                                              rb.coffset, rp.pooled_h, rp.pooled_w, rp.spatial_scale, yb.cstride, yb.coffset, st))
            return [OpTask(l, [Op("roi_pool", l.name, run, 0.0, 4.0 * (n * h * w * c + r * rp.pooled_h * rp.pooled_w * c))],
                           reads=[self._range(b) for b in l.bottoms], writes=[self._range(l.tops[0])])]
        if t == "PSROIPooling":
            sp = RG.psroi_pool_params(l)
            RG.psroi_pool_shape(l, [self.shapes[b] for b in l.bottoms])
            run = lambda st: L.check(lib.fcn_psroi_pool_fwd_f32(xb.buf.ptr, rb.buf.ptr, yb.buf.ptr, n, h, w, c, xb.cstride, xb.coffset, r, rb.cstride,
                                                                rb.coffset, sp.output_dim, sp.group_size, sp.spatial_scale, yb.cstride, yb.coffset, st))
            return [OpTask(l, [Op("psroi_pool", l.name, run, 1.0 * r * c * 4, 4.0 * (n * h * w * c + r * c))],
                           reads=[self._range(b) for b in l.bottoms], writes=[self._range(l.tops[0])])]
        raise NotImplementedError("layer type %r (layer %s) has no forward kernel yet" % (t, l.name))

    def _download_counts(self, stream: Optional[int]) -> None:
        for name, cnt in self.roi_counts.items():
            host = self._roi_count_host.get(name)
            if host is None:
                host = self._roi_count_host[name] = PinnedArray((4,))
            L.check(L.load().fcn_memcpy_d2h_async(host.array.ctypes.data, cnt.ptr, 4, stream))

    def _roi_count(self, name: str) -> int:
        if not self._counts_valid:
            with self.lock:
                self._download_counts(self.stream)
                L.call("fcn_stream_sync", self.stream)
                self._counts_valid = True
        return min(max(int(self._roi_count_host[name].array.view(np.int32)[0]), 0), self._roi_caps[name])

    def _cut_rois(self, name: str, a: np.ndarray) -> np.ndarray:
        if name not in self.spec.roi_blobs or not getattr(self, "_ran", False):
            return a
        return a[:self._roi_count(self.spec.roi_blobs[name].name)]

    def _compose_detections(self, name: str) -> np.ndarray:
        raw = self.blobs[name].host
        cap = self.detections[name]
        count = int(raw[7 * cap:7 * cap + 1].view(np.int32)[0])
        l = self.spec.detection_blobs[name]
        return SSD.compose_detections(raw, min(max(count, 0), cap), self.shapes[l.bottoms[0]][0])

    def _dwconv_task(self, li: int, l: Layer, skip: set) -> OpTask:
        lib = L.load()
        g = self._dwgeom(l)
        xb, yb = self.blobs[l.bottoms[0]], self.blobs[l.tops[0]]
        eps = 16 // xb.esize
        if xb.coffset % eps or xb.cstride % eps:
            raise NotImplementedError("depthwise Convolution %s: input view is not 16-byte aligned" % l.name)
        if xb.esize == 4 and yb.esize != 4:
            raise NotImplementedError("f16 engine: depthwise Convolution %s reads the float32 blob %s and writes halves" % (l.name, l.bottoms[0]))
        relu = self._relu_after(li, l, skip)
        self._conv_layer_meta[l.name] = dict(relu=relu, sigmoid_top=None)
        pd = self.params_dev[l.name]
        flags = (L.CONV_RELU if relu else 0) | (L.CONV_OUT_F32 if xb.esize == 2 and yb.esize == 4 else 0)
        d = dwconv_desc(xb, yb, g, pd[0].ptr, pd[1].ptr if len(pd) > 1 else None, flags)
        fn = lib.fcn_dwconv2d_fwd_f16 if xb.esize == 2 else lib.fcn_dwconv2d_fwd_f32
        op = Op("dwconv", "%s [%dx%d]" % (l.name, g.kh, g.kw), lambda st: L.check(fn(C.byref(d), -1, st)), g.flops, g.bytes)
        return OpTask(l, [op], reads=[self._range(l.bottoms[0])], writes=[self._range(l.tops[0])], dwconv=d)

    def _rconv_task(self, li: int, l: Layer, skip: set) -> OpTask:
        rect, dil, ng = is_rectangular(l), layer_dilation(l), self._conv_groups(l)
        who = "rectangular Convolution %s (%dx%d stride %dx%d pad %dx%d)" % (l.name, *layer_geometry(l)) if rect else \
            "Convolution %s with dilation %d" % (l.name, dil)
        if self.f16:
            raise NotImplementedError("f16 engine: %s has no half-float kernel" % who)
        if ng > 1:
            raise NotImplementedError("%s: group %d" % (who, ng) if rect else "Convolution %s: group %d together with dilation %d" % (l.name, ng, dil))
        g = self._rgeom(l)
        xb, yb = self.blobs[l.bottoms[0]], self.blobs[l.tops[0]]
        if xb.coffset % 4 or xb.cstride % 4:
            raise NotImplementedError("%s Convolution %s: input view is not 16-byte aligned" % ("rectangular" if rect else "dilated", l.name))
        relu = self._relu_after(li, l, skip)
        self._conv_layer_meta[l.name] = dict(relu=relu, sigmoid_top=None)
        pd = self.params_dev[l.name]
        d = rconv_desc(xb, yb, g, pd[0].ptr, pd[1].ptr if len(pd) > 1 else None, L.CONV_RELU if relu else 0)
        return OpTask(l, [], reads=[self._range(l.bottoms[0])], writes=[self._range(l.tops[0])], rconv=d)

    def _emit_rconvs(self, items: List[OpTask]) -> None:
        lib = L.load()
        groups: Dict[Tuple[bool, Range], List[OpTask]] = {}
        for it in items:
            groups.setdefault((is_rectangular(it.layer), it.reads[0]), []).append(it)
        for (rect, _), chunk in sorted(groups.items(), key=lambda kv: kv[0][0]):
            arr = (L.RConvDesc * len(chunk))(*[it.rconv for it in chunk])
            ws = DeviceBuffer(int(lib.fcn_rconv2d_workspace_bytes(arr, len(chunk))), zero=False)
            plan = L.RConvPlan()
            L.call("fcn_rconv2d_prepare", arr, len(chunk), ws.ptr, -1, C.byref(plan))
            self._keep.extend([arr, ws, plan])
            geoms = [self._rgeom(it.layer) for it in chunk]
            shows = ",".join("%dx%d" % (g.kh, g.kw) for g in geoms) if rect else "d" + ",".join(str(g.d) for g in geoms)
            label = "%s [%s %dwg]" % ("+".join(it.layer.name for it in chunk), shows, plan.total_tiles)
            self.ops.append(Op("rconv" if rect else "dconv", label, lambda st, p=plan: L.check(lib.fcn_rconv2d_f32(C.byref(p), st)),
                               sum(g.flops for g in geoms), sum(g.bytes for g in geoms)))

    def _emit_group(self, chunk: List[ConvTask], fused: List[OpTask], tail: Optional[dict]) -> None:
        lib = L.load()
        name = "+".join(it.layer.name for it in chunk)
        flops = sum(it.flops for it in chunk)
        byts = sum(it.bytes for it in chunk)
        arr = (L.ConvDesc * len(chunk))(*[it.desc for it in chunk])
        ws = DeviceBuffer(int(lib.fcn_conv2d_group_workspace_bytes(len(chunk))), zero=False)
        self._group_workspaces.append(ws)
        grp = L.ConvGroup()
        parr = (L.PoolDesc * max(len(fused), 1))(*[pt.pool_desc for pt in fused])
        tune_key = name + ("{+%d pool}" % len(fused) if fused else "")
        tailed = tail is not None and any(id(it) in tail["producers"] for it in chunk)
        if tailed:
            fin = 1 if any(tail["producers"][id(it)] == tail["final_level"] for it in chunk if id(it) in tail["producers"]) else 0
            tail["desc"].finalize = fin
            L.call("fcn_conv2d_group_attach_tail", ws.ptr, C.byref(tail["desc"]))
            tune_key += "{+tail%d}" % fin
            if fin:
                flops += sum(ht.flops for ht in tail["heads"])
                byts += sum(4.0 * ht.desc.Cout * (ht.desc.N * ht.desc.OH * ht.desc.OW + ht.desc.Cin) for ht in tail["heads"])
        cfg = self.tuner.conv_cfg(tune_key, arr, len(chunk), ws, parr, len(fused)) if self.autotune else -1
        L.call("fcn_conv2d_group_prepare_fused", arr, len(chunk), parr, len(fused), ws.ptr, cfg, C.byref(grp))
        self._keep.extend([arr, parr, ws, grp])
        kind = "conv_group" if len(chunk) > 1 else "conv"
        label = "%s [cfg%d %dwg]" % (name, grp.cfg, grp.total_tiles)
        if fused:
            label = "%s {+%s}" % (label, "+".join(pt.layer.name for pt in fused))
            byts += sum(pt.ops[0].bytes for pt in fused)
        if tailed:
            label = "%s {%s %s}" % (label, "tail:" if tail["desc"].finalize else "partial sums of", "+".join(ht.layer.name for ht in tail["heads"]))
        self.ops.append(Op(kind, label, lambda st, g=grp: L.check(lib.fcn_conv2d_fwd_group_f32(C.byref(g), st)), flops, byts))

    def _emit_convs(self, items: List[ConvTask], pools: List[OpTask], tail: Optional[dict]) -> None:
        for base in range(0, len(items), 16):
            chunk = items[base:base + 16]
            fused = pools[:2] if base == 0 and len(chunk) <= 8 else []
            parts = [chunk]
            if self.f16 and self.autotune and not fused and len(chunk) > 1:
                parts = self.tuner.split_level(chunk)
            for part in parts:
                self._emit_group(part, fused, tail)
                fused = []
            if base == 0 and len(chunk) <= 8:
                del pools[:2]
        for pt in pools:
            self.ops.extend(pt.ops)
        pools.clear()

    def _emit_score_ops(self) -> None:
        lib = L.load()
        for nm in self.outputs:
            b = self.blobs[nm]
            if b.esize != 4 or b.lazy_shift:
                raise NotImplementedError("score_outputs: output blob %s is not a plain float32 blob" % nm)
            count = int(np.prod(b.shape)) if b.shape else 1
            acc = DeviceBuffer(max(4 * count, 16), zero=True)
            self.score_acc[nm] = acc
            if b.nchw is not None:
                n, c, h, w = b.nchw
                args = (acc.ptr, b.buf.ptr, n, h * w, c, b.cstride, b.coffset)
            else:
                args = (acc.ptr, b.ptr, 1, 1, count, count, 0)
            self.ops.append(Op("score", "score:" + nm, lambda st, a=args: L.check(lib.fcn_score_accumulate_f32(*a, st)), 0.0, 12.0 * count))

    def _plan_tail(self, tasks: List[Task], levels: List[int]) -> Optional[dict]:
        if self.f16 or self.spec.phase != "TEST" or not (self.fuse and self.group_convs) or os.environ.get("FCN_CONV_TAIL", "0") != "1":
            return None
        conv_idx = [i for i, t in enumerate(tasks) if isinstance(t, ConvTask)]
        if not conv_idx:
            return None
        lh = max(levels[i] for i in conv_idx)
        heads = [i for i in conv_idx if levels[i] == lh]
        if any(levels[i] >= lh for i, t in enumerate(tasks) if not isinstance(t, ConvTask)) or not 1 <= len(heads) <= 4:
            return None
        d0 = tasks[heads[0]].desc
        m = d0.N * d0.OH * d0.OW
        rows = 0
        for i in heads:
            d = tasks[i].desc
            if (d.kh, d.kw, d.stride, d.pad) != (1, 1, 1, 0) or d.x != d0.x or d.x_cstride != d0.x_cstride or d.Cin != d0.Cin or d.Cin % 32 or d.Cin > 1024 or d.Cout % 4 \
                    or (d.flags & ~(L.CONV_RELU | L.CONV_SIGMOID2)) or d.y_cstride % 4 or d.y_coffset % 4 or (d.y2 and (d.y2_cstride % 4 or d.y2_coffset % 4)):
                return None
            rows += d.Cout
        if rows > 24 or m > 4096:
            return None
        xr = tasks[heads[0]].reads
        producers: Dict[int, int] = {}
        covered = 0
        for i, t in enumerate(tasks):
            if i in heads or not ranges_hit(t.writes, xr):
                continue
            if not isinstance(t, ConvTask):
                return None
            d = t.desc
            if levels[i] not in (lh - 1, lh - 2) or d.y != d0.x or d.y_cstride != d0.x_cstride or d.N * d.OH * d.OW != m \
                    or d.Cout % 32 or d.y_coffset % 32 or d.y_coffset + d.Cout > d0.Cin or (d.flags & ~L.CONV_RELU) or d.y_cstride % 4:
                return None
            producers[id(t)] = levels[i]
            covered += d.Cout
        if covered != d0.Cin or not producers:
            return None
        for lv in set(producers.values()):
            if sum(1 for i in conv_idx if levels[i] == lv) > 8:
                return None
        lib = L.load()
        desc = L.ConvTail()
        desc.n = len(heads)
        for j, i in enumerate(heads):
            desc.heads[j] = tasks[i].desc
        sb, ab = int(lib.fcn_conv2d_tail_scratch_bytes(C.byref(desc))), int(lib.fcn_conv2d_tail_arrive_bytes(C.byref(desc)))
        if sb <= 0 or ab <= 0:
            return None
        scratch, arrive = DeviceBuffer(sb, zero=False), DeviceBuffer(ab, zero=True)
        desc.scratch, desc.arrive = scratch.ptr, arrive.ptr
        self._keep.extend([scratch, arrive, desc])
        return dict(desc=desc, heads=[tasks[i] for i in heads], producers=producers, final_level=max(producers.values()))

    def _fuse_pool_lrn(self, tasks: List[Task]) -> List[Task]:
        B, lib = self.blobs, L.load()
        out: List[Task] = []
        i = 0
        while i < len(tasks):
            a = tasks[i]
            b = tasks[i + 1] if i + 1 < len(tasks) else None
            op = None
            if isinstance(a, OpTask) and isinstance(b, OpTask):
                la, lb = a.layer, b.layer
                if {la.type, lb.type} == {"Pooling", "LRN"} and len(la.tops) == 1 and lb.bottoms == [la.tops[0]] and la.tops[0] != la.bottoms[0]:
                    op = self._pool_lrn_op(la, lb)
            if op is None:
                out.append(a)
                i += 1
                continue
            self._lazy_blob_ops[a.layer.tops[0]] = list(a.ops)
            c = tasks[i + 2] if i + 2 < len(tasks) else None
            op3 = self._pool_lrn_conv_op(a.layer, b.layer, c) if isinstance(c, ConvTask) else None
            if op3 is not None:
                self._lazy_blob_ops[b.layer.tops[0]] = [op]
                out.append(OpTask(c.layer, [op3], reads=a.reads, writes=c.writes))
                i += 3
                continue
            out.append(OpTask(b.layer, [op], reads=a.reads, writes=b.writes))
            i += 2
        return out

    def _pool_lrn_conv_op(self, la: Layer, lb: Layer, ct: ConvTask) -> Optional[Op]:
        if os.environ.get("FCN_FUSE_POOL_LRN_CONV", "1") == "0" or la.type != "Pooling":
            return None
        B, lib = self.blobs, L.load()
        lc, d = ct.layer, ct.desc
        mid = lb.tops[0]
        if lc.bottoms != [mid] or [q.name for q in self.consumers.get(mid, [])] != [lc.name] or len(self.producers.get(mid, [])) != 1 \
                or mid in self.outputs or mid in self.alias:
            return None
        xb, nb = B[la.bottoms[0]], B[mid]
        k, s, pad = kernel_stride_pad(la.sub("pooling_param"))
        lp = lb.sub("lrn_param")
        esz = xb.esize
        want = (L.CONV_F16 if esz == 2 else 0)
        if (d.kh, d.kw, d.stride, d.pad) != (1, 1, 1, 0) or d.Cin != 64 or d.Cout != 64 or xb.channels != 64 or k != 3 or nb.esize != esz \
                or (d.flags & ~L.CONV_RELU) != want or d.in_shift != 0.0 or nb.coffset or d.y_cstride % (16 // esz) or d.y_coffset % (16 // esz) or B[lc.tops[0]].esize != esz:
            return None
        n, c, h, w = xb.shape
        oh, ow = d.OH, d.OW
        if (oh + 3) // 4 > 65535 or n > 65535:
            return None
        if esz == 2 and ((s, pad) != (2, 0) or n * c * h * w < 1 << 22):
            return None
        al, be, kk = float(lp.get("alpha", 1.0)), float(lp.get("beta", 0.75)), float(lp.get("k", 1.0))
        relu = 1 if d.flags & L.CONV_RELU else 0
        fn = lib.fcn_maxpool_lrn5_conv1x1_fwd_f16 if esz == 2 else lib.fcn_maxpool_lrn5_conv1x1_fwd_f32
        return Op("pool_lrn_conv", "%s+%s+%s" % (la.name, lb.name, lc.name), lambda st: L.check(fn(
            xb.ptr, n, h, w, c, xb.cstride, k, s, pad, oh, ow, al, be, kk, d.w, d.bias, d.Cout, relu, d.y, d.y_cstride, d.y_coffset, st)),
            ct.flops, float(esz) * (xb.pixels * c + n * oh * ow * d.Cout))

    def _pool_lrn_op(self, la: Layer, lb: Layer) -> Optional[Op]:
        B, lib = self.blobs, L.load()
        pool, lrn = (la, lb) if la.type == "Pooling" else (lb, la)
# ... 703 lines not shown
    def forward_end(self) -> Dict[str, np.ndarray]:
        with self.lock:
            L.call("fcn_stream_sync", self.stream)
            for b in self.blobs.values():
                b.host_valid = False
            self._ran = self._counts_valid = True
            out = {}
            for nm in self.outputs:
                b = self.blobs[nm]
                if b.lazy_shift:
                    b.host += F32(b.lazy_shift)
                b.host_valid = True
                out[nm] = self._cut_rois(nm, b.host) if nm not in self.detections else self._compose_detections(nm)
            for nm in self.inputs:
                self.blobs[nm].host_valid = nm not in self.device_fed
            return out

    def upload_inputs(self) -> None:
        with self.lock:
            for nm in self.inputs:
                self._enqueue_upload(nm, self.stream)
            L.call("fcn_stream_sync", self.stream)

    def forward_enqueue(self) -> None:
        with self.lock:
            if graphs_enabled():
                if self.graph_core is None:
                    self.graph_core = self._capture(with_io=False)
                L.call("fcn_graph_launch", self.graph_core, self.stream)
            else:
                self.run_ops(self.stream)
            for b in self.blobs.values():
                if not b.is_input:
                    b.host_valid = False
            self._ran, self._counts_valid = True, False

    def forward_resident(self, iters: int = 1, use_graph: bool = True) -> float:
        use_graph = use_graph and graphs_enabled()
        with self.lock:
            L.call("fcn_init", self.device)
            if use_graph and self.graph_core is None:
                self.graph_core = self._capture(with_io=False)
            e0, e1 = C.c_void_p(), C.c_void_p()
            L.call("fcn_event_create", C.byref(e0))
            L.call("fcn_event_create", C.byref(e1))
            L.call("fcn_event_record", e0, self.stream)
            for _ in range(iters):
                if use_graph:
                    L.call("fcn_graph_launch", self.graph_core, self.stream)
                else:
                    self.run_ops(self.stream)
            L.call("fcn_event_record", e1, self.stream)
            L.call("fcn_event_sync", e1)
            ms = C.c_float()
            L.call("fcn_event_elapsed_ms", e0, e1, C.byref(ms))
            L.call("fcn_event_destroy", e0)
            L.call("fcn_event_destroy", e1)
            for b in self.blobs.values():
                if not b.is_input:
                    b.host_valid = False
            self._counts_valid = False
            return float(ms.value)

    def time_ops(self, reps: int = 20, ops: Optional[Sequence["Op"]] = None) -> List[Tuple[str, str, float, float, float]]:
        out = []
        with self.lock:
            e0, e1 = C.c_void_p(), C.c_void_p()
            L.call("fcn_event_create", C.byref(e0))
            L.call("fcn_event_create", C.byref(e1))
            for op in (self.ops if ops is None else ops):
                op.run(self.stream)
                L.call("fcn_event_record", e0, self.stream)
                for _ in range(reps):
                    op.run(self.stream)
                L.call("fcn_event_record", e1, self.stream)
                L.call("fcn_event_sync", e1)
                ms = C.c_float()
                L.call("fcn_event_elapsed_ms", e0, e1, C.byref(ms))
                out.append((op.kind, op.name, ms.value / reps, op.flops, op.bytes))
            L.call("fcn_event_destroy", e0)
            L.call("fcn_event_destroy", e1)
        return out

    def time_ops_in_sequence(self, reps: int = 10) -> List[Tuple[str, str, float, float, float]]:
        out = []
        with self.lock:
            e0, e1 = C.c_void_p(), C.c_void_p()
            L.call("fcn_event_create", C.byref(e0))
            L.call("fcn_event_create", C.byref(e1))
            ms = C.c_float()
            empty = []
            for _ in range(10):
                self.ops[0].run(self.stream)
                L.call("fcn_event_record", e0, self.stream)
                L.call("fcn_event_record", e1, self.stream)
                L.call("fcn_event_sync", e1)
                L.call("fcn_event_elapsed_ms", e0, e1, C.byref(ms))
                empty.append(ms.value)
            floor = float(np.median(empty))
            for i, op in enumerate(self.ops):
                acc = []
                for _ in range(reps):
                    for prev in self.ops[:i]:
                        prev.run(self.stream)
                    L.call("fcn_event_record", e0, self.stream)
                    op.run(self.stream)
                    L.call("fcn_event_record", e1, self.stream)
                    L.call("fcn_event_sync", e1)
                    L.call("fcn_event_elapsed_ms", e0, e1, C.byref(ms))
                    acc.append(ms.value)
                out.append((op.kind, op.name, float(np.median(acc)), op.flops, op.bytes))
            L.call("fcn_event_destroy", e0)
            L.call("fcn_event_destroy", e1)
        self.event_pair_floor_ms = floor
        return out

    def close(self) -> None:
        with self.lock:
            lib = L.load()
            for g in (self.graph_io, self.graph_core, self.graph_score):
                if g:
                    lib.fcn_graph_destroy(g)
            self.graph_io = self.graph_core = self.graph_score = None
            if self.stream:
                lib.fcn_stream_sync(self.stream)
                lib.fcn_stream_destroy(self.stream)
                self.stream = 0
            for ws in getattr(self, "_group_workspaces", []):
                if ws.ptr:
                    lib.fcn_conv2d_group_release(ws.ptr)
                    ws.free()
            self._group_workspaces = []
            self.ops = []
            self.tuner.release()

    def __del__(self):
        try:
            self.close()
        except Exception:
            pass


class ForwardPipeline:

    def __init__(self, make_spec: Callable[[], NetSpec], params: Optional[Dict[str, List[np.ndarray]]] = None, device: int = 0, depth: int = 4,
                 max_lds_kb: Optional[int] = 36, **engine_kw):
        if depth < 1:
            raise ValueError("depth must be at least 1")
        self.engines: List[Engine] = []
        if os.environ.get("FCN_PIPE_LDS_KB"):
            max_lds_kb = int(os.environ["FCN_PIPE_LDS_KB"]) or None
        if max_lds_kb is not None:
            engine_kw.setdefault("tune_max_lds_kb", max_lds_kb)
        for i in range(depth):
            self.engines.append(Engine(make_spec(), params=params, device=device, tune_from=self.engines[0] if i else None, replica=i,
                                       **engine_kw))
        self._pending: List[Engine] = []
        self._next = 0

    @property
    def depth(self) -> int:
        return len(self.engines)

    def submit(self, inputs: Dict[str, np.ndarray]) -> None:
        if len(self._pending) >= len(self.engines):
            raise RuntimeError("ForwardPipeline: %d frames already in flight, collect() one first" % len(self._pending))
        eng = self.engines[self._next]
        self._next = (self._next + 1) % len(self.engines)
        for nm, arr in inputs.items():
            eng.host_array(nm)[...] = arr
        eng.forward_begin()
        self._pending.append(eng)

    def collect(self) -> Dict[str, np.ndarray]:
        if not self._pending:
            raise RuntimeError("ForwardPipeline: nothing in flight")
        eng = self._pending.pop(0)
        return {k: v.copy() for k, v in eng.forward_end().items()}

    def map(self, frames: Sequence[Dict[str, np.ndarray]]) -> List[Dict[str, np.ndarray]]:
        out: List[Dict[str, np.ndarray]] = []
        for f in frames:
            if len(self._pending) == len(self.engines):
                out.append(self.collect())
            self.submit(f)
        while self._pending:
            out.append(self.collect())
        return out

    def calibrate(self, depths: Sequence[int] = (3, 4), iters: int = 60) -> int:
        best, best_t = None, 1e30
        for d in depths:
            if 1 <= d <= len(self.engines):
                self.run_resident(iters, depth=d)
                t = self.run_resident(iters, depth=d)
                if t < best_t:
                    best, best_t = d, t
        self.active = best or len(self.engines)
        return self.active

    def run_resident(self, iters: int, depth: Optional[int] = None) -> float:
        import time
        lib = L.load()
        engines = self.engines[:depth or getattr(self, "active", None) or len(self.engines)]
        return self._run_resident(engines, iters, lib, time)

    def run_io(self, iters: int, depth: Optional[int] = None) -> float:
        import time
        engines = self.engines[:depth or getattr(self, "active", None) or len(self.engines)]
        pending: List[Engine] = []
        t0 = time.perf_counter()
        for i in range(iters):
            e = engines[i % len(engines)]
            if len(pending) == len(engines):
                pending.pop(0).forward_end()
            e.forward_begin()
            pending.append(e)
        while pending:
            pending.pop(0).forward_end()
        return time.perf_counter() - t0

    def warm_io(self, depth: Optional[int] = None) -> None:
        for e in self.engines[:depth or getattr(self, "active", None) or len(self.engines)]:
            e.forward_begin()
            e.forward_end()

    def _run_resident(self, engines, iters, lib, time) -> float:
        for e in engines:
            if e.graph_core is None:
                e.forward_resident(1)
            L.call("fcn_stream_sync", e.stream)
        no_graph = not graphs_enabled()
        t0 = time.perf_counter()
        for i in range(iters):
            e = engines[i % len(engines)]
            if no_graph:
                e.run_ops(e.stream)
            else:
                L.check(lib.fcn_graph_launch(e.graph_core, e.stream))
        for e in engines:
            L.call("fcn_stream_sync", e.stream)
        return time.perf_counter() - t0

    def close(self) -> None:
        for e in self.engines:
            e.close()
```

fcn_object_detector_amd/lib.py:

```python
from __future__ import annotations

import ctypes as C
import os
import threading
from typing import Optional

_HERE = os.path.dirname(os.path.abspath(__file__))
LIB_PATH = os.environ.get("FCN_LIB_PATH") or os.path.join(_HERE, "libfcnhip.so")


class FcnLibraryError(RuntimeError):
    pass


class FcnError(RuntimeError):
    def __init__(self, code: int, msg: str):
        super().__init__("libfcnhip error %d: %s" % (code, msg))
        self.code = code


class ConvDesc(C.Structure):
    _fields_ = [
        ("x", C.c_void_p), ("w", C.c_void_p), ("bias", C.c_void_p), ("y", C.c_void_p), ("y2", C.c_void_p),
        ("N", C.c_int32), ("H", C.c_int32), ("W", C.c_int32), ("Cin", C.c_int32), ("x_cstride", C.c_int32),
        ("Cout", C.c_int32), ("kh", C.c_int32), ("kw", C.c_int32), ("pad", C.c_int32), ("stride", C.c_int32),
        ("OH", C.c_int32), ("OW", C.c_int32),
        ("y_cstride", C.c_int32), ("y_coffset", C.c_int32), ("y2_cstride", C.c_int32), ("y2_coffset", C.c_int32),
        ("flags", C.c_int32), ("in_shift", C.c_float),
    ]


class ConvTail(C.Structure):
    _fields_ = [("n", C.c_int32), ("finalize", C.c_int32), ("heads", ConvDesc * 4), ("scratch", C.c_void_p), ("arrive", C.c_void_p)]


class ConvGroup(C.Structure):
    _fields_ = [("d_probs", C.c_void_p), ("n", C.c_int32), ("cfg", C.c_int32), ("total_tiles", C.c_int32)]


class TConvDesc(C.Structure):
    _fields_ = [
        ("a", C.c_void_p), ("w", C.c_void_p), ("bias", C.c_void_p), ("b", C.c_void_p), ("y2", C.c_void_p),
        ("N", C.c_int32), ("H", C.c_int32), ("W", C.c_int32), ("Ca", C.c_int32), ("a_cstride", C.c_int32),
        ("Cb", C.c_int32), ("kh", C.c_int32), ("kw", C.c_int32), ("pad", C.c_int32), ("stride", C.c_int32),
        ("OH", C.c_int32), ("OW", C.c_int32),
        ("b_cstride", C.c_int32), ("b_coffset", C.c_int32), ("y2_cstride", C.c_int32), ("y2_coffset", C.c_int32),
        ("flags", C.c_int32),
    ]


class TConvPlan(C.Structure):
    _fields_ = [("d_probs", C.c_void_p), ("n", C.c_int32), ("cfg", C.c_int32), ("grid_x", C.c_int32), ("grid_y", C.c_int32),
                ("total_tiles", C.c_int32)]


class RConvDesc(C.Structure):
    _fields_ = [
        ("x", C.c_void_p), ("w", C.c_void_p), ("bias", C.c_void_p), ("y", C.c_void_p), ("y2", C.c_void_p),
        ("N", C.c_int32), ("H", C.c_int32), ("W", C.c_int32), ("Cin", C.c_int32), ("x_cstride", C.c_int32),
        ("Cout", C.c_int32), ("kh", C.c_int32), ("kw", C.c_int32), ("pad_h", C.c_int32), ("pad_w", C.c_int32),
        ("stride_h", C.c_int32), ("stride_w", C.c_int32), ("OH", C.c_int32), ("OW", C.c_int32),
        ("y_cstride", C.c_int32), ("y_coffset", C.c_int32), ("y2_cstride", C.c_int32), ("y2_coffset", C.c_int32),
        ("flags", C.c_int32), ("dilation", C.c_int32),
    ]


class RConvPlan(C.Structure):
    _fields_ = [("d_probs", C.c_void_p), ("n", C.c_int32), ("cfg", C.c_int32), ("grid_x", C.c_int32), ("grid_y", C.c_int32),
                ("total_tiles", C.c_int32)]


class DwConvDesc(C.Structure):
    _fields_ = [
        ("x", C.c_void_p), ("w", C.c_void_p), ("bias", C.c_void_p), ("y", C.c_void_p), ("y2", C.c_void_p),
        ("N", C.c_int32), ("H", C.c_int32), ("W", C.c_int32), ("C", C.c_int32), ("x_cstride", C.c_int32),
        ("kh", C.c_int32), ("kw", C.c_int32), ("pad_h", C.c_int32), ("pad_w", C.c_int32),
        ("stride_h", C.c_int32), ("stride_w", C.c_int32), ("OH", C.c_int32), ("OW", C.c_int32),
        ("y_cstride", C.c_int32), ("y_coffset", C.c_int32), ("y2_cstride", C.c_int32), ("y2_coffset", C.c_int32),
        ("flags", C.c_int32), ("dilation", C.c_int32),
    ]


def dwconv_desc(x: int, w: Optional[int], bias: Optional[int], y: int, n: int, h: int, wd: int, c: int, x_cstride: int, kh: int, kw: int,
                ph: int, pw: int, sh: int, sw: int, dilation: int, y_cstride: int, y_coffset: int, flags: int = 0) -> DwConvDesc:
    d = DwConvDesc()
    d.x, d.w, d.bias, d.y = x, w, bias, y
    d.N, d.H, d.W, d.C, d.x_cstride = n, h, wd, c, x_cstride
    d.kh, d.kw, d.pad_h, d.pad_w, d.stride_h, d.stride_w = kh, kw, ph, pw, sh, sw
    d.OH = (h + 2 * ph - (dilation * (kh - 1) + 1)) // sh + 1
    d.OW = (wd + 2 * pw - (dilation * (kw - 1) + 1)) // sw + 1
    d.y_cstride, d.y_coffset, d.flags, d.dilation = y_cstride, y_coffset, flags, dilation
    return d


class SolverSeg(C.Structure):
    _fields_ = [("offset", C.c_uint64), ("count", C.c_uint64), ("lr_mult", C.c_float), ("decay_mult", C.c_float)]


class LayoutDesc(C.Structure):
    _fields_ = [("src", C.c_void_p), ("dst", C.c_void_p)] + [(k, C.c_int32) for k in ("N", "C", "H", "W", "src_cstride", "src_coffset")]


class PoolDesc(C.Structure):
    _fields_ = [("x", C.c_void_p), ("y", C.c_void_p), ("idx", C.c_void_p)] + [(k, C.c_int32) for k in (
        "N", "H", "W", "C", "x_cstride", "k", "stride", "pad", "OH", "OW", "y_cstride", "y_coffset", "f16")]


class SceneObj(C.Structure):
    _fields_ = [("img", C.c_void_p), ("mask", C.c_void_p)] + [(k, C.c_int32) for k in (
        "src_h", "src_w", "flip", "roi_x", "roi_y", "roi_w", "roi_h", "out_w", "out_h", "cx", "cy", "label1")]


class ColorParams(C.Structure):
    _fields_ = [("sharpen_centre", C.c_float), ("sharpen_off", C.c_float), ("add", C.c_int32 * 3), ("mul", C.c_float * 3),
                ("gray_alpha", C.c_float), ("gray_keep", C.c_float)]


GAUSS_MAX_RADIUS = 15
REPLICA_STREAMS = 4


class FlipSeg(C.Structure):
    _fields_ = [("w_offset", C.c_uint64), ("wt_offset", C.c_uint64), ("Cout", C.c_int32), ("kh", C.c_int32), ("kw", C.c_int32),
                ("Cin", C.c_int32), ("Cin4", C.c_int32), ("Cout4", C.c_int32)]


class DetectParams(C.Structure):
    _fields_ = [
        ("num_classes", C.c_int32), ("gy", C.c_int32), ("gx", C.c_int32), ("cell_w", C.c_int32), ("cell_h", C.c_int32),
        ("cvg_cstride", C.c_int32), ("cvg_coffset", C.c_int32), ("box_cstride", C.c_int32), ("box_coffset", C.c_int32),
        ("prob_thresh", C.c_float), ("group_thresh", C.c_int32), ("eps", C.c_double), ("min_height", C.c_int32),
        ("round_mode", C.c_int32), ("max_out", C.c_int32),
    ]


class SsdHead(C.Structure):
    _fields_ = [("src", C.c_void_p)] + [(k, C.c_int32) for k in ("pixels", "C", "cstride", "coffset", "dst_col", "reserved")]


class DetOutParams(C.Structure):
    _fields_ = [(k, C.c_int32) for k in ("N", "P", "num_classes", "background", "code_type", "variance_encoded", "top_k", "keep_top_k")] + [
        ("conf_threshold", C.c_float), ("nms_threshold", C.c_float)] + [(k, C.c_int32) for k in ("loc_rstride", "conf_rstride", "capacity", "reserved")]


class ProposalParams(C.Structure):
    _fields_ = [(k, C.c_int32) for k in ("H", "W", "A", "feat_stride", "pre_nms_topn", "post_nms_topn")] + [
        ("min_size", C.c_float), ("nms_thresh", C.c_float)] + [(k, C.c_int32) for k in (
            "score_cstride", "score_coffset", "delta_cstride", "delta_coffset", "rois_cstride", "rois_coffset", "top_score_cstride",
            "top_score_coffset")] + [("anchors", C.c_float * 128)]


PROPOSAL_MAX_ANCHORS = 32
PROPOSAL_MAX_CANDIDATES = 65536
PROPOSAL_MAX_PRE_NMS = 6144
SSD_MAX_HEADS = 16
DETOUT_MAX_TOPK = 1024
CODE_CORNER, CODE_CENTER_SIZE = 1, 2
CONV_RELU, CONV_SIGMOID2, CONV_ACCUM, CONV_OUT_F32, CONV_F16, CONV_OUT_F16, CONV_MASK = 1, 2, 4, 8, 16, 32, 64
IP_MAX_ROWS = 32
IP_WEIGHTS_NT = 256
CONV_IMAGE_ONES = 128
ELT_PROD, ELT_SUM, ELT_MAX = 0, 1, 2
SOLVER_KINDS = {"SGD": 0, "NESTEROV": 1, "ADAGRAD": 2, "RMSPROP": 3, "ADADELTA": 4, "ADAM": 5}
REG_L2, REG_L1 = 0, 1
RECT_ROUND_NEAREST_EVEN, RECT_ROUND_TRUNCATE = 0, 1

_vp, _i, _f, _d, _sz = C.c_void_p, C.c_int, C.c_float, C.c_double, C.c_size_t

PROTOTYPES = {
    "fcn_abi_version": (_i, []),
    "fcn_last_error_string": (C.c_char_p, []),
    "fcn_device_count": (_i, [C.POINTER(_i)]),
    "fcn_init": (_i, [_i]),
    "fcn_device_name": (_i, [C.c_char_p, _i]),
    "fcn_device_sync": (_i, []),
    "fcn_malloc": (_i, [C.POINTER(_vp), _sz]),
    "fcn_free": (_i, [_vp]),
    "fcn_host_malloc": (_i, [C.POINTER(_vp), _sz]),
    "fcn_host_free": (_i, [_vp]),
    "fcn_memset_async": (_i, [_vp, _i, _sz, _vp]),
    "fcn_memcpy_h2d_async": (_i, [_vp, _vp, _sz, _vp]),
    "fcn_memcpy_d2h_async": (_i, [_vp, _vp, _sz, _vp]),
    "fcn_memcpy_d2d_async": (_i, [_vp, _vp, _sz, _vp]),
    "fcn_stream_create": (_i, [C.POINTER(_vp)]),
    "fcn_stream_destroy": (_i, [_vp]),
    "fcn_stream_sync": (_i, [_vp]),
    "fcn_event_create": (_i, [C.POINTER(_vp)]),
    "fcn_event_destroy": (_i, [_vp]),
    "fcn_event_record": (_i, [_vp, _vp]),
    "fcn_event_sync": (_i, [_vp]),
    "fcn_event_elapsed_ms": (_i, [_vp, _vp, C.POINTER(_f)]),
    "fcn_graph_begin": (_i, [_vp]),
    "fcn_graph_end": (_i, [_vp, C.POINTER(_vp)]),
    "fcn_graph_launch": (_i, [_vp, _vp]),
    "fcn_graph_destroy": (_i, [_vp]),
    "fcn_stream_create_replica": (_i, [C.POINTER(_vp), _i]),
    "fcn_stream_is_prioritized": (_i, [_vp, C.POINTER(_i)]),
    "fcn_nchw_to_nhwc_f32": (_i, [_vp, _vp, _i, _i, _i, _i, _i, _i, _f, _vp]),
    "fcn_nhwc_to_nchw_f32": (_i, [_vp, _vp, _i, _i, _i, _i, _i, _i, _vp]),
    "fcn_nhwc_to_nchw_multi_f32": (_i, [C.POINTER(LayoutDesc), _i, _vp]),
    "fcn_conv2d_fwd_f32": (_i, [C.POINTER(ConvDesc), _vp]),
    "fcn_conv2d_group_workspace_bytes": (_sz, [_i]),
    "fcn_conv2d_num_configs": (_i, []),
    "fcn_conv2d_first_layer_config": (_i, []),
    "fcn_conv2d_config_lds_bytes": (_i, [_i]),
    "fcn_conv2d_config_waves_k": (_i, [_i]),
    "fcn_conv2d_group_prepare": (_i, [C.POINTER(ConvDesc), _i, _vp, _i, C.POINTER(ConvGroup)]),
    "fcn_conv2d_group_prepare_fused": (_i, [C.POINTER(ConvDesc), _i, C.POINTER(PoolDesc), _i, _vp, _i, C.POINTER(ConvGroup)]),
    "fcn_conv2d_fwd_group_f32": (_i, [C.POINTER(ConvGroup), _vp]),
    "fcn_conv2d_group_release": (_i, [_vp]),
    "fcn_conv2d_tail_scratch_bytes": (C.c_size_t, [C.POINTER(ConvTail)]),
    "fcn_conv2d_tail_arrive_bytes": (C.c_size_t, [C.POINTER(ConvTail)]),
    "fcn_conv2d_group_attach_tail": (_i, [_vp, C.POINTER(ConvTail)]),
    "fcn_maxpool_fwd_f32": (_i, [_vp, _vp, _vp] + [_i] * 12 + [_vp]),
    "fcn_avepool_fwd_f32": (_i, [_vp, _vp] + [_i] * 12 + [_vp]),
    "fcn_lrn_fwd_f32": (_i, [_vp, _vp, _vp, _i, _i, _i, _i, _i, _f, _f, _f, _vp]),
    "fcn_maxpool_lrn5_fwd_f32": (_i, [_vp, _vp] + [_i] * 12 + [_f, _f, _f, _vp]),
    "fcn_maxpool_lrn5_fwd_f16": (_i, [_vp, _vp] + [_i] * 12 + [_f, _f, _f, _vp]),
    "fcn_maxpool_lrn5_conv1x1_fwd_f32": (_i, [_vp] + [_i] * 10 + [_f, _f, _f, _vp, _vp, _i, _i, _vp, _i, _i, _vp]),
    "fcn_maxpool_lrn5_conv1x1_fwd_f16": (_i, [_vp] + [_i] * 10 + [_f, _f, _f, _vp, _vp, _i, _i, _vp, _i, _i, _vp]),
    "fcn_relu_fwd_f32": (_i, [_vp, _vp, _sz, _f, _vp]),
    "fcn_sigmoid_fwd_f32": (_i, [_vp, _vp, _sz, _vp]),
    "fcn_power_fwd_f32": (_i, [_vp, _vp, _sz, _f, _f, _f, _vp]),
    "fcn_eltwise_fwd_f32": (_i, [_vp, _vp, _vp, _sz, _i, _f, _f, _vp]),
    "fcn_copy_channels_f32": (_i, [_vp, _vp, _i, _i, _i, _i, _i, _i, _vp]),
    "fcn_deconv_depthwise_fwd_f32": (_i, [_vp, _vp, _vp, _vp] + [_i] * 12 + [_vp]),
    "fcn_preprocess_bgr8": (_i, [_vp, _i, _i, _vp, _i, _i, _i, _f, _vp, _vp]),
    "fcn_detect_workspace_bytes": (_sz, [C.POINTER(DetectParams), _i]),
    "fcn_detect_decode_group": (_i, [_vp, _vp, _i, _sz, _sz, C.POINTER(DetectParams), _vp, _vp, _vp, _vp, _vp]),
    "fcn_score_masks_workspace_bytes": (_sz, [_i, _i, _i, _i]),
    "fcn_score_masks": (_i, [_vp, _i, _i, _i, _i, _i, _i, _vp, _f, _vp, _i, _i, _vp, _vp, _vp]),
    "fcn_gen_targets": (_i, [_vp, _vp, _vp, _i, _i, _i, _i, _i, _d, _vp, _vp, _vp, _vp, _vp, _vp]),
    "fcn_gen_targets_nhwc": (_i, [_vp, _vp, _vp, _i, _i, _i, _i, _i, _d, _vp, _i, _vp, _vp, _vp, _vp, _i, _vp]),
    "fcn_conv2d_wgrad_workspace_floats": (_sz, [C.POINTER(ConvDesc), C.POINTER(_i)]),
    "fcn_conv2d_wgrad_f32": (_i, [C.POINTER(ConvDesc), _vp, _vp, _vp, _vp]),
    "fcn_conv2d_wgrad_group_workspace_floats": (_sz, [C.POINTER(ConvDesc), _i]),
    "fcn_conv2d_wgrad_group_f32": (_i, [C.POINTER(ConvDesc), _vp, _vp, _i, _vp, _vp]),
    "fcn_conv2d_wgrad_num_configs": (_i, []),
    "fcn_conv2d_wgrad_split_config": (_i, []),
    "fcn_conv2d_wgrad_workspace_floats_cfg": (_sz, [C.POINTER(ConvDesc), _i, C.POINTER(_i)]),
    "fcn_conv2d_wgrad_cfg_f32": (_i, [C.POINTER(ConvDesc), _vp, _vp, _vp, _i, _vp]),
    "fcn_conv2d_wgrad_group_workspace_floats_cfg": (_sz, [C.POINTER(ConvDesc), _i, _i]),
    "fcn_conv2d_wgrad_group_cfg_f32": (_i, [C.POINTER(ConvDesc), _vp, _vp, _i, _vp, _i, _vp]),
    "fcn_conv_weights_flip_f32": (_i, [_vp, _vp, _i, _i, _i, _i, _i, _i, _vp]),
    "fcn_nchw_f32_to_nhwc_f16": (_i, [_vp, _vp, _i, _i, _i, _i, _i, _i, _f, _vp]),
    "fcn_nhwc_f16_to_nchw_f32": (_i, [_vp, _vp, _i, _i, _i, _i, _i, _i, _vp]),
    "fcn_maxpool_fwd_f16": (_i, [_vp, _vp] + [_i] * 12 + [_vp]),
    "fcn_lrn_fwd_f16": (_i, [_vp, _vp, _i, _i, _i, _i, _i, _f, _f, _f, _vp]),
    "fcn_avepool_fwd_f16": (_i, [_vp, _vp] + [_i] * 12 + [_vp]),
    "fcn_deconv_depthwise_fwd_f16": (_i, [_vp, _vp, _vp, _vp] + [_i] * 13 + [_vp]),
    "fcn_eltwise_fwd_f16": (_i, [_vp, _vp, _vp, _sz, _i, _f, _f, _vp]),
    "fcn_softmax_fwd_f16": (_i, [_vp, _vp, _i, _i, _i, _i, _i, _vp]),
    "fcn_copy_channels_f16": (_i, [_vp, _vp, _i, _i, _i, _i, _i, _i, _vp]),
    "fcn_preprocess_bgr8_batch": (_i, [_vp, _i, _i, _i, _vp, _i, _i, _i, _i, _f, _vp, _vp]),
    "fcn_preprocess_bgr8_rois": (_i, [_vp, _i, _i, _vp, _i, _vp, _i, _i, _i, _i, _f, _vp, _vp]),
    "fcn_preprocess_bgr8_f16": (_i, [_vp, _i, _i, _vp, _i, _i, _i, _f, _vp, _vp]),
    "fcn_compose_scene_bgr8": (_i, [_vp, _i, _i, _i, _i, _i, _i, _vp, _i, _i, _vp, _vp, _i, _i, _vp]),
    "fcn_mask_to_label_f32": (_i, [_vp, _i, _i, _vp, _i, _i, _i, _vp]),
    "fcn_compose_scene_view_bgr8": (_i, [_vp, _i, _i, _i, _i, _i, _i, _vp, _i, _i, _vp, _vp, _i, _i, _i, _i, _i, _i, _vp]),
    "fcn_blur_gauss_bgr8": (_i, [_vp, _vp, _vp, _i, _i, _vp, _i, _vp]),
    "fcn_blur_box_bgr8": (_i, [_vp, _vp, _i, _i, _i, _vp]),
    "fcn_blur_median_bgr8": (_i, [_vp, _vp, _i, _i, _i, _vp]),
    "fcn_color_augment_bgr8": (_i, [_vp, _vp, _i, _i, _vp, _vp]),
    "fcn_softmax_fwd_f32": (_i, [_vp, _vp, _i, _i, _i, _i, _vp]),
    "fcn_softmax_loss_workspace_bytes": (_sz, []),
    "fcn_softmax_loss_f32": (_i, [_vp, _vp, _vp, _vp, _i, _i, _i, _i, _i, _i, _i, _i, _f, _vp, _vp]),
    "fcn_deconv_depthwise_bwd_f32": (_i, [_vp, _vp, _vp] + [_i] * 13 + [_vp]),
    "fcn_conv_weights_flip_batch_f32": (_i, [_vp, _vp, _vp, _i, _vp]),
    "fcn_relu_bwd_f32": (_i, [_vp, _vp, _vp, _i, _i, _i, _vp]),
    "fcn_relu_bwd_slope_f32": (_i, [_vp, _vp, _vp, _i, _i, _i, _f, _i, _vp]),
    "fcn_sigmoid_bwd_f32": (_i, [_vp, _vp, _vp, _sz, _i, _vp]),
    "fcn_maxpool_bwd_f32": (_i, [_vp, _vp, _vp] + [_i] * 14 + [_vp]),
    "fcn_maxpool_bwd_mask_f32": (_i, [_vp, _vp, _vp] + [_i] * 14 + [_vp, _i, _i, _vp]),
    "fcn_avepool_bwd_f32": (_i, [_vp, _vp] + [_i] * 14 + [_vp]),
    "fcn_lrn_bwd_f32": (_i, [_vp, _vp, _vp, _vp, _vp, _i, _i, _i, _i, _i, _f, _f, _i, _vp]),
    "fcn_dropout_f32": (_i, [_vp, _vp] + [_i] * 8 + [_f, C.c_uint, C.c_uint, _vp]),
    "fcn_stream_wait_event": (_i, [_vp, _vp]),
    "fcn_comm_unique_id": (_i, [C.c_char_p]),
    "fcn_comm_init": (_i, [C.POINTER(_vp), C.c_char_p, _i, _i]),
    "fcn_comm_allreduce_sum_f32": (_i, [_vp, _vp, _sz, _vp]),
    "fcn_comm_destroy": (_i, [_vp]),
    "fcn_loss_f32": (_i, [_i, _vp, _vp, _vp, _vp, _i, _i, _i, _i, _f, _vp]),
    "fcn_sgd_update_f32": (_i, [_vp, _vp, _vp, _vp, _i, _f, _f, _f, _f, _vp]),
    "fcn_adam_update_f32": (_i, [_vp, _vp, _vp, _vp, _vp, _i, _f, _f, _f, _f, _f, _i, _f, _vp]),
    "fcn_solver_update_f32": (_i, [_i, _vp, _vp, _vp, _vp, _vp, _i, _f, _f, _f, _f, _f, _f, _i, _i, _f, _vp, _vp]),
    "fcn_grad_clip_workspace_bytes": (_sz, []),
    "fcn_grad_clip_f32": (_i, [_vp, _vp, _i, _f, _f, _vp, _vp, _vp, _vp]),
    "fcn_grad_accumulate_f32": (_i, [_vp, _vp, _sz, _i, _vp]),
    "fcn_score_accumulate_f32": (_i, [_vp, _vp, _i, _i, _i, _i, _i, _vp]),
    "fcn_accuracy_workspace_bytes": (_sz, []),
    "fcn_accuracy_f32": (_i, [_vp, _vp, _vp, _vp, _i, _i, _i, _i, _i, _i, _i, _i, _vp, _vp]),
    "fcn_tconv2d_num_configs": (_i, []),
    "fcn_tconv2d_workspace_bytes": (_sz, [C.POINTER(TConvDesc), _i]),
    "fcn_tconv2d_prepare": (_i, [C.POINTER(TConvDesc), _i, _vp, _i, C.POINTER(TConvPlan)]),
    "fcn_tconv2d_f32": (_i, [C.POINTER(TConvPlan), _vp]),
    "fcn_tconv_bank_floats": (_sz, [_i, _i, _i, _i]),
    "fcn_tconv_bank_pack_f32": (_i, [_vp, _vp, _i, _i, _i, _i, _i, _vp]),
    "fcn_channel_sum_f32": (_i, [_vp, _vp, _i, _i, _i, _i, _vp]),
    "fcn_rconv2d_num_configs": (_i, []),
    "fcn_rconv2d_workspace_bytes": (_sz, [C.POINTER(RConvDesc), _i]),
    "fcn_rconv2d_prepare": (_i, [C.POINTER(RConvDesc), _i, _vp, _i, C.POINTER(RConvPlan)]),
    "fcn_rconv2d_f32": (_i, [C.POINTER(RConvPlan), _vp]),
    "fcn_rconv2d_wgrad_workspace_floats": (_sz, [C.POINTER(RConvDesc)]),
    "fcn_rconv2d_wgrad_f32": (_i, [C.POINTER(RConvDesc), _vp, _vp, _vp, _vp]),
    "fcn_dwconv2d_num_configs": (_i, []),
    "fcn_dwconv2d_fwd_f32": (_i, [C.POINTER(DwConvDesc), _i, _vp]),
    "fcn_dwconv2d_fwd_f16": (_i, [C.POINTER(DwConvDesc), _i, _vp]),
    "fcn_dwconv2d_dgrad_f32": (_i, [C.POINTER(DwConvDesc), _i, _vp]),
    "fcn_dwconv2d_wgrad_workspace_floats": (_sz, [C.POINTER(DwConvDesc), _i]),
    "fcn_dwconv2d_wgrad_f32": (_i, [C.POINTER(DwConvDesc), _vp, _vp, _vp, _i, _vp]),
    "fcn_crop_fwd_f32": (_i, [_vp, _vp] + [_i] * 12 + [_vp]),
    "fcn_crop_fwd_f16": (_i, [_vp, _vp] + [_i] * 12 + [_vp]),
    "fcn_crop_bwd_f32": (_i, [_vp, _vp] + [_i] * 13 + [_vp]),
    "fcn_interp_fwd_f32": (_i, [_vp, _vp] + [_i] * 12 + [_vp]),
    "fcn_interp_fwd_f16": (_i, [_vp, _vp] + [_i] * 13 + [_vp]),
    "fcn_interp_bwd_f32": (_i, [_vp, _vp] + [_i] * 13 + [_vp]),
    "fcn_unpool_fwd_f32": (_i, [_vp, _vp, _vp] + [_i] * 13 + [_vp]),
    "fcn_unpool_fwd_f16": (_i, [_vp, _vp, _vp] + [_i] * 14 + [_vp]),
    "fcn_unpool_bwd_f32": (_i, [_vp, _vp, _vp] + [_i] * 14 + [_vp]),
    "fcn_maxpool_idx_fwd_f16": (_i, [_vp, _vp, _vp] + [_i] * 12 + [_vp]),
    "fcn_pool_mask_to_nchw_f32": (_i, [_vp, _vp] + [_i] * 4 + [_vp]),
    "fcn_inner_product_workspace_bytes": (_sz, [_i, _i, _i]),
    "fcn_inner_product_fwd_workspace_bytes": (_sz, [_i, _i, _i, _i]),
    "fcn_inner_product_fwd_f32": (_i, [_vp, _i, _vp, _vp, _vp] + [_i] * 6 + [_vp, _vp]),
    "fcn_inner_product_fwd_f16": (_i, [_vp, _i, _vp, _vp, _vp] + [_i] * 6 + [_vp, _vp]),
    "fcn_inner_product_bwd_data_f32": (_i, [_vp, _i, _i, _vp, _vp] + [_i] * 5 + [_vp, _vp]),
    "fcn_inner_product_bwd_weights_f32": (_i, [_vp, _i, _vp, _i, _i, _vp, _vp] + [_i] * 4 + [_vp]),
    "fcn_batchnorm_workspace_bytes": (_sz, [_i, _i]),
    "fcn_batchnorm_stats_f32": (_i, [_vp] + [_i] * 4 + [_vp, _vp, _vp, _f, _f, _vp, _vp, _vp]),
    "fcn_batchnorm_apply_f32": (_i, [_vp, _vp, _vp] + [_i] * 7 + [_vp, _vp, _vp, _vp, _f, _vp, _vp, _i, _vp]),
    "fcn_batchnorm_apply_f16": (_i, [_vp, _vp] + [_i] * 6 + [_vp, _vp, _vp, _f, _vp, _vp, _i, _vp]),
    "fcn_batchnorm_bwd_reduce_f32": (_i, [_vp, _vp, _vp] + [_i] * 8 + [_vp, _vp, _vp, _vp]),
    "fcn_batchnorm_bwd_apply_f32": (_i, [_vp, _vp, _vp, _vp] + [_i] * 10 + [_vp, _vp, _vp, _f, _vp, _vp, _vp, _i, _vp]),
    "fcn_ssd_gather_f32": (_i, [C.POINTER(SsdHead), _i, _i, _vp, _i, _i, _vp]),
    "fcn_normalize_fwd_f32": (_i, [_vp, _vp, _vp] + [_i] * 7 + [_f, _vp]),
    "fcn_detection_output_workspace_bytes": (_sz, [C.POINTER(DetOutParams)]),
    "fcn_detection_output_f32": (_i, [_vp, _vp, _vp, C.POINTER(DetOutParams), _vp, _vp, _vp, _sz, _vp]),
    "fcn_pair_softmax_f32": (_i, [_vp, _vp] + [_i] * 6 + [_vp]),
    "fcn_proposal_workspace_bytes": (_sz, [C.POINTER(ProposalParams)]),
    "fcn_proposal_f32": (_i, [_vp, _vp, _vp, C.POINTER(ProposalParams), _vp, _vp, _vp, _vp, _sz, _vp]),
    "fcn_roi_pool_fwd_f32": (_i, [_vp, _vp, _vp, _vp] + [_i] * 11 + [_f, _i, _i, _vp]),
    "fcn_psroi_pool_fwd_f32": (_i, [_vp, _vp, _vp] + [_i] * 11 + [_f, _i, _i, _vp]),
}

HW_QUEUES: dict = {}
_lib: Optional[C.CDLL] = None
_lock = threading.Lock()


def load() -> C.CDLL:
    global _lib
    if _lib is not None:
        return _lib
    with _lock:
        if _lib is not None:
            return _lib
        if not os.path.isfile(LIB_PATH):
            raise FcnLibraryError(
                "libfcnhip.so not found at %s — build it with `python -c 'import __graft_entry__ as g; g.build()'` "
# ... 46 lines not shown
```

fcn_object_detector_amd/tune.py:

```python
from __future__ import annotations

import ctypes as C
import json
import os
from typing import Callable, Dict, Iterable, List, NamedTuple, Optional, Sequence, Tuple

import numpy as np

from . import engine as E
from . import lib as L


def lower_quartile(samples: Sequence[float]) -> float:
    return float(np.percentile(samples, 25))


class Protocol(NamedTuple):
    warm: int
    reps: int
    evict: bool
    samples: int
    stat: Callable[[Sequence[float]], float]
    contenders: int
    margin: float
    look: int
    carry: bool


COLD = Protocol(warm=1, reps=1, evict=True, samples=7, stat=lower_quartile, contenders=4, margin=1.05, look=31, carry=False)
WARM = Protocol(warm=2, reps=6, evict=False, samples=1, stat=min, contenders=3, margin=1.04, look=5, carry=True)
WGRAD = Protocol(warm=2, reps=5, evict=False, samples=1, stat=min, contenders=3, margin=1.04, look=4, carry=True)

FLUSH_BYTES = 64 << 20


def set_partitions(n: int) -> Iterable[List[int]]:
    def rec(labels: List[int], groups: int):
        if len(labels) == n:
            yield list(labels)
            return
        for g in range(groups + 1):
            labels.append(g)
            yield from rec(labels, max(groups, g + 1))
            labels.pop()
    yield from rec([], 0)


def key_suffix(input_shape: Optional[Sequence[int]], f16: bool, max_lds: int) -> str:
    key = "|" + ("x".join(str(d) for d in input_shape) if input_shape is not None else "")
    return key + ("|f16" if f16 else "") + ("|lds%d" % (max_lds // 1024) if max_lds < 160 * 1024 else "")


class Tuner:
    def __init__(self, stream: int, key_suffix: str, cold: bool, max_lds: int, tune_from: Optional[Dict[str, object]] = None):
        self.stream, self.key_suffix, self.cold, self.max_lds, self.tune_from = stream, key_suffix, cold, max_lds, tune_from
        self.chosen: Dict[str, object] = {}
        self.events: Optional[Tuple[C.c_void_p, C.c_void_p]] = None
        self.flush: Optional["E.DeviceBuffer"] = None
        self.cache_path = os.environ.get("FCN_TUNE_CACHE") or None
        self.cache: Optional[dict] = None
        if self.cache_path:
            try:
                with open(self.cache_path) as f:
                    self.cache = json.load(f)
            except (OSError, ValueError):
                self.cache = {}
            if not isinstance(self.cache, dict):
                self.cache = {}

    def key(self, name: str) -> str:
        return name + self.key_suffix

    def release(self) -> None:
        if self.events is not None:
            for ev in self.events:
                L.call("fcn_event_destroy", ev)
            self.events = None
        if self.flush is not None:
            self.flush.free()
            self.flush = None

    def measure(self, launch: Callable[[], None], reps: int, evict: bool = False) -> float:
        if self.events is None:
            e0, e1 = C.c_void_p(), C.c_void_p()
            L.call("fcn_event_create", C.byref(e0))
            L.call("fcn_event_create", C.byref(e1))
            self.events = (e0, e1)
        e0, e1 = self.events
        if evict:
            if self.flush is None:
                self.flush = E.DeviceBuffer(FLUSH_BYTES, zero=False)
            L.call("fcn_memset_async", self.flush.ptr, 0, self.flush.nbytes, self.stream)
        L.call("fcn_event_record", e0, self.stream)
        for _ in range(reps):
            launch()
        L.call("fcn_event_record", e1, self.stream)
        L.call("fcn_event_sync", e1)
        ms = C.c_float()
        L.call("fcn_event_elapsed_ms", e0, e1, C.byref(ms))
        return ms.value / reps

    def fastest(self, cfgs: Iterable[int], prepare: Callable[[int], bool], launch: Callable[[], None], p: Protocol,
                second_look: bool = True) -> Tuple[int, float]:
        timed: List[Tuple[float, int]] = []
        for cfg in cfgs:
            if not prepare(cfg):
                continue
            for _ in range(p.warm):
                launch()
            timed.append((p.stat([self.measure(launch, p.reps, p.evict) for _ in range(p.samples)]), cfg))
        if not timed:
            return -1, 1e30
        best_ms, best = min(timed)
        if second_look and len(timed) > 1:
            finals = []
            for t1, cfg in sorted(timed)[:p.contenders]:
                if t1 > p.margin * best_ms:
                    break
                if prepare(cfg):
                    finals.append((p.stat(([t1] if p.carry else []) + [self.measure(launch, p.reps, p.evict) for _ in range(p.look)]), cfg))
            if finals:
                best_ms, best = min(finals)
        return best, best_ms

    def time_conv_cfgs(self, arr, n: int, ws: "E.DeviceBuffer", parr=None, npool: int = 0) -> Tuple[int, float]:
        lib = L.load()
        grp = L.ConvGroup()
        first_layer = int(lib.fcn_conv2d_first_layer_config())
        cold = self.cold and os.environ.get("FCN_TUNE_COLD", "1") != "0"

        def admitted(cfg: int) -> bool:
            if cfg == first_layer:
                return os.environ.get("FCN_CONV_FIRST7", "1") != "0"
            return int(lib.fcn_conv2d_config_lds_bytes(cfg)) <= self.max_lds

        def prepare(cfg: int) -> bool:
            return lib.fcn_conv2d_group_prepare_fused(arr, n, parr, npool, ws.ptr, cfg, C.byref(grp)) == 0

        return self.fastest([c for c in range(int(lib.fcn_conv2d_num_configs())) if admitted(c)], prepare,
                            lambda: L.check(lib.fcn_conv2d_fwd_group_f32(C.byref(grp), self.stream)), COLD if cold else WARM,
                            cold or os.environ.get("FCN_TUNE_SECOND_LOOK", "1") != "0")

    def _subset_ms(self, descs: Sequence[L.ConvDesc], pools: Sequence[L.PoolDesc] = ()) -> float:
        lib = L.load()
        arr = (L.ConvDesc * len(descs))(*descs)
        parr = (L.PoolDesc * max(len(pools), 1))(*pools) if pools else None
        ws = E.DeviceBuffer(int(lib.fcn_conv2d_group_workspace_bytes(len(descs))), zero=False)
        try:
            return self.time_conv_cfgs(arr, len(descs), ws, parr, len(pools))[1]
        finally:
            L.call("fcn_conv2d_group_release", ws.ptr)
            ws.free()

    def choose(self, key: str, valid: Callable[[object], bool], search: Callable[[], object]):
        for known in (self.tune_from, self.cache):
            if known is not None and valid(known.get(key)):
                value = known[key]
                break
        else:
            value = search()
            if self.cache is not None:
                self.cache[key] = value
                try:
                    with open(self.cache_path, "w") as f:
                        json.dump(self.cache, f, indent=0, sort_keys=True)
                except OSError:
                    pass
        self.chosen[key] = value
        return value

    @staticmethod
    def _valid_cfg(ncfg: int) -> Callable[[object], bool]:
        return lambda v: type(v) is int and 0 <= v < ncfg

    def conv_cfg(self, name: str, arr, n: int, ws: "E.DeviceBuffer", parr=None, npool: int = 0) -> int:
        return self.choose(self.key(name), self._valid_cfg(int(L.load().fcn_conv2d_num_configs())),
                           lambda: self.time_conv_cfgs(arr, n, ws, parr, npool)[0])

    def wgrad_cfgs(self, ops: Sequence["E.Op"]) -> None:
        ncfg = int(L.load().fcn_conv2d_wgrad_num_configs())
        for op in ops:
            if op.kind != "wgrad" or op.sel is None:
                continue

            def select(cfg: int) -> bool:
                op.sel["cfg"] = cfg
                return True

            op.sel["cfg"] = self.choose(self.key("wgrad:" + "+".join(op.layers)), self._valid_cfg(ncfg),
                                        lambda: self.fastest(range(ncfg), select, lambda: op.run(self.stream), WGRAD)[0])
            op.name += " [cfg%d]" % op.sel["cfg"]

    def split_level(self, chunk: List["E.ConvTask"]) -> List[List["E.ConvTask"]]:
        n = len(chunk)
        if n < 2 or n > 4:
            return [chunk]

        def valid(code) -> bool:
            return isinstance(code, str) and len(code) == n and all(ch.isdigit() and int(ch) < n for ch in code)

        def search() -> str:
            memo: Dict[Tuple[int, ...], float] = {}

            def cost(sub: Tuple[int, ...]) -> float:
                if sub not in memo:
                    memo[sub] = self._subset_ms([chunk[i].desc for i in sub])
                return memo[sub]

            best, best_ms = None, 1e30
            for labels in set_partitions(n):
                ms = sum(cost(tuple(i for i in range(n) if labels[i] == g)) for g in sorted(set(labels)))
                if ms < best_ms - 1e-7:
                    best, best_ms = labels, ms
            return "".join(str(g) for g in best)

        choice = self.choose("cut|" + self.key("+".join(it.layer.name for it in chunk)), valid, search)
        groups: Dict[str, List[E.ConvTask]] = {}
        for it, g in zip(chunk, choice):
            groups.setdefault(g, []).append(it)
        return [groups[g] for g in sorted(groups)]

    def move_floaters(self, tasks: Sequence[object], levels: List[int]) -> None:
        for lv in range(max(levels, default=-1)):
            a_idx, b_idx = ([i for i, t in enumerate(tasks) if levels[i] == l2 and isinstance(t, E.ConvTask)] for l2 in (lv, lv + 1))
            if len(a_idx) < 2 or not b_idx or len(a_idx) > 8:
                continue
            fl = [i for i in a_idx if E.task_floats(tasks, levels, i)]
            if not fl or len(fl) > 3 or len(b_idx) + len(fl) > 8:
                continue

            def valid(code) -> bool:
                return isinstance(code, str) and len(code) == len(fl) and set(code) <= {"0", "1"} and (len(fl) < len(a_idx) or "0" in code)

            def search() -> str:
                pools = {l2: [t.pool_desc for j, t in enumerate(tasks) if levels[j] == l2 and isinstance(t, E.OpTask) and t.pool_desc is not None][:2]
                         for l2 in (lv, lv + 1)}
                memo: Dict[Tuple[int, Tuple[int, ...]], float] = {}

                def cost(l2: int, sub: Tuple[int, ...]) -> float:
                    if (l2, sub) not in memo:
                        memo[(l2, sub)] = min(self._subset_ms([tasks[i].desc for i in sub], pools[l2]) for _ in range(2))
                    return memo[(l2, sub)]

                best, best_ms, base_ms = "0" * len(fl), None, None
                for code in range(1 << len(fl)):
                    moved = [fl[b] for b in range(len(fl)) if code >> b & 1]
                    stay = tuple(i for i in a_idx if i not in moved)
                    if not stay:
                        continue
                    ms = cost(lv, stay) + cost(lv + 1, tuple(b_idx + moved))
                    if code == 0:
                        base_ms = ms
                    if best_ms is None or ms < best_ms:
                        best, best_ms = "".join("1" if code >> b & 1 else "0" for b in range(len(fl))), ms
                if best_ms > float(os.environ.get("FCN_MOVE_MARGIN", "0.99")) * base_ms:
                    best = "0" * len(fl)
                return best

            names = ("+".join(tasks[i].layer.name for i in idx) for idx in (a_idx, b_idx))
            choice = self.choose("move|" + self.key(">".join(names)), valid, search)
            for b, i in enumerate(fl):
                if choice[b] == "1":
                    levels[i] = lv + 1
```

include/fcnhip.h:

```cpp
#ifndef FCNHIP_H_
#define FCNHIP_H_

#include <stddef.h>
#include <stdint.h>

#ifdef __cplusplus
extern "C" {
#endif

#define FCN_ABI_VERSION 2

#define FCN_E_ARG       1
#define FCN_E_ALIGN     2
#define FCN_E_UNSUPPORTED 3
#define FCN_E_STATE     4
#define FCN_E_CAPACITY  5

typedef void* fcn_stream_t;
typedef void* fcn_event_t;
typedef void* fcn_graph_t;
typedef void* fcn_comm_t;

int  fcn_abi_version(void);
const char* fcn_last_error_string(void);
int  fcn_device_count(int* count);
int  fcn_init(int device);
int  fcn_device_name(char* h_buf, int len);
int  fcn_device_sync(void);
int  fcn_malloc(void** p, size_t bytes);
int  fcn_free(void* p);
int  fcn_host_malloc(void** h_p, size_t bytes);
int  fcn_host_free(void* h_p);
int  fcn_memset_async(void* p, int value, size_t bytes, fcn_stream_t s);
int  fcn_memcpy_h2d_async(void* dst, const void* h_src, size_t bytes, fcn_stream_t s);
int  fcn_memcpy_d2h_async(void* h_dst, const void* src, size_t bytes, fcn_stream_t s);
int  fcn_memcpy_d2d_async(void* dst, const void* src, size_t bytes, fcn_stream_t s);
int  fcn_stream_create(fcn_stream_t* s);
int  fcn_stream_destroy(fcn_stream_t s);
int  fcn_stream_sync(fcn_stream_t s);
int  fcn_event_create(fcn_event_t* e);
int  fcn_event_destroy(fcn_event_t e);
int  fcn_event_record(fcn_event_t e, fcn_stream_t s);
int  fcn_event_sync(fcn_event_t e);
int  fcn_event_elapsed_ms(fcn_event_t start, fcn_event_t stop, float* h_ms);
int  fcn_stream_wait_event(fcn_stream_t s, fcn_event_t e);
int  fcn_graph_begin(fcn_stream_t s);
int  fcn_graph_end(fcn_stream_t s, fcn_graph_t* g);
int  fcn_graph_launch(fcn_graph_t g, fcn_stream_t s);
int  fcn_graph_destroy(fcn_graph_t g);
#define FCN_REPLICA_STREAMS 4
int  fcn_stream_create_replica(fcn_stream_t* s, int index);
int  fcn_stream_is_prioritized(fcn_stream_t s, int* h_yes);

int  fcn_nchw_to_nhwc_f32(const float* src, float* dst, int N, int C, int H, int W,
                          int dst_cstride, int dst_coffset, float shift, fcn_stream_t s);
int  fcn_nhwc_to_nchw_f32(const float* src, float* dst, int N, int C, int H, int W,
                          int src_cstride, int src_coffset, fcn_stream_t s);
typedef struct fcn_layout_desc {
    const float* src;
    float* dst;
    int32_t N, C, H, W, src_cstride, src_coffset;
} fcn_layout_desc;
int  fcn_nhwc_to_nchw_multi_f32(const fcn_layout_desc* h_descs, int n, fcn_stream_t s);

#define FCN_CONV_RELU      1
#define FCN_CONV_SIGMOID2  2
#define FCN_CONV_ACCUM     4
#define FCN_CONV_MASK     64
#define FCN_CONV_IMAGE_ONES 128
#define FCN_CONV_OUT_F32   8
#define FCN_CONV_OUT_F16  32
#define FCN_CONV_F16      16
typedef struct fcn_conv_desc {
    const float* x;
    const float* w;
    const float* bias;
    float*       y;
    float*       y2;
    int32_t N, H, W, Cin, x_cstride;
    int32_t Cout, kh, kw, pad, stride, OH, OW;
    int32_t y_cstride, y_coffset, y2_cstride, y2_coffset;
    int32_t flags;
    float   in_shift;
} fcn_conv_desc;
int  fcn_conv2d_fwd_f32(const fcn_conv_desc* h_desc, fcn_stream_t s);
typedef struct fcn_conv_group {
    void*   d_probs;
    int32_t n;
    int32_t cfg;
    int32_t total_tiles;
} fcn_conv_group;
size_t fcn_conv2d_group_workspace_bytes(int n);
int  fcn_conv2d_num_configs(void);
int  fcn_conv2d_first_layer_config(void);
typedef struct fcn_conv_tail {
    int32_t n;
    int32_t finalize;
    fcn_conv_desc heads[4];
    float*  scratch;
    void*   arrive;
} fcn_conv_tail;
size_t fcn_conv2d_tail_scratch_bytes(const fcn_conv_tail* t);
size_t fcn_conv2d_tail_arrive_bytes(const fcn_conv_tail* t);
int  fcn_conv2d_group_attach_tail(void* d_workspace, const fcn_conv_tail* t);
int  fcn_conv2d_config_lds_bytes(int cfg);
int  fcn_conv2d_config_waves_k(int cfg);
int  fcn_conv2d_group_prepare(const fcn_conv_desc* h_descs, int n, void* d_workspace, int cfg_request, fcn_conv_group* h_out);
int  fcn_conv2d_fwd_group_f32(const fcn_conv_group* h_group, fcn_stream_t s);
typedef struct fcn_pool_desc {
    const float* x; float* y; int32_t* idx;
    int32_t N, H, W, C, x_cstride, k, stride, pad, OH, OW, y_cstride, y_coffset;
    int32_t f16;
} fcn_pool_desc;
int  fcn_conv2d_group_prepare_fused(const fcn_conv_desc* h_descs, int n, const fcn_pool_desc* h_pools, int npools, void* d_workspace,
                                    int cfg_request, fcn_conv_group* h_out);
int  fcn_conv2d_group_release(void* d_workspace);

int  fcn_maxpool_fwd_f32(const float* x, float* y, int32_t* idx, int N, int H, int W, int C,
                         int x_cstride, int k, int stride, int pad, int OH, int OW,
                         int y_cstride, int y_coffset, fcn_stream_t s);
int  fcn_avepool_fwd_f32(const float* x, float* y, int N, int H, int W, int C, int x_cstride,
                         int k, int stride, int pad, int OH, int OW, int y_cstride, int y_coffset,
                         fcn_stream_t s);
int  fcn_lrn_fwd_f32(const float* x, float* y, float* scale, int pixels, int C, int x_cstride,
                     int y_cstride, int local_size, float alpha, float beta, float k, fcn_stream_t s);
int  fcn_maxpool_lrn5_fwd_f32(const float* x, float* y, int N, int H, int W, int C, int x_cstride, int k, int stride, int pad,
                              int OH, int OW, int y_cstride, int lrn_first, float alpha, float beta, float lrn_k, fcn_stream_t s);
int  fcn_maxpool_lrn5_conv1x1_fwd_f32(const float* x, int N, int H, int W, int C, int x_cstride, int k, int stride, int pad,
                                      int OH, int OW, float alpha, float beta, float lrn_k, const float* w, const float* bias,
                                      int Cout, int relu, float* y, int y_cstride, int y_coffset, fcn_stream_t s);
int  fcn_maxpool_lrn5_conv1x1_fwd_f16(const void* x, int N, int H, int W, int C, int x_cstride, int k, int stride, int pad,
                                      int OH, int OW, float alpha, float beta, float lrn_k, const void* w, const float* bias,
                                      int Cout, int relu, void* y, int y_cstride, int y_coffset, fcn_stream_t s);
int  fcn_relu_fwd_f32(const float* x, float* y, size_t count, float negative_slope, fcn_stream_t s);
int  fcn_sigmoid_fwd_f32(const float* x, float* y, size_t count, fcn_stream_t s);
int  fcn_power_fwd_f32(const float* x, float* y, size_t count, float power, float scale, float shift, fcn_stream_t s);
#define FCN_ELT_PROD 0
#define FCN_ELT_SUM  1
#define FCN_ELT_MAX  2
int  fcn_eltwise_fwd_f32(const float* a, const float* b, float* y, size_t count, int op,
                         float ca, float cb, fcn_stream_t s);
int  fcn_copy_channels_f32(const float* src, float* dst, int pixels, int C, int src_cstride,
                           int src_coffset, int dst_cstride, int dst_coffset, fcn_stream_t s);
int  fcn_softmax_fwd_f32(const float* x, float* y, int pixels, int C, int x_cstride, int y_cstride, fcn_stream_t s);
int  fcn_deconv_depthwise_fwd_f32(const float* x, const float* w, const float* bias, float* y,
                                  int N, int H, int W, int C, int x_cstride, int k, int stride, int pad,
                                  int OH, int OW, int y_cstride, int y_coffset, fcn_stream_t s);

int  fcn_preprocess_bgr8(const uint8_t* frame, int h, int w, float* dst, int H, int W, int dst_cstride,
                         float shift, float* d_minmax, fcn_stream_t s);

int  fcn_nchw_f32_to_nhwc_f16(const float* src, void* dst, int N, int C, int H, int W, int dst_cstride, int dst_coffset, float shift,
                              fcn_stream_t s);
int  fcn_nhwc_f16_to_nchw_f32(const void* src, float* dst, int N, int C, int H, int W, int src_cstride, int src_coffset, fcn_stream_t s);
int  fcn_maxpool_fwd_f16(const void* x, void* y, int N, int H, int W, int C, int x_cstride, int k, int stride, int pad, int OH, int OW,
                         int y_cstride, int y_coffset, fcn_stream_t s);
int  fcn_lrn_fwd_f16(const void* x, void* y, int pixels, int C, int x_cstride, int y_cstride, int local_size, float alpha, float beta,
                     float k, fcn_stream_t s);
int  fcn_maxpool_lrn5_fwd_f16(const void* x, void* y, int N, int H, int W, int C, int x_cstride, int k, int stride, int pad,
                              int OH, int OW, int y_cstride, int lrn_first, float alpha, float beta, float lrn_k, fcn_stream_t s);
int  fcn_avepool_fwd_f16(const void* x, void* y, int N, int H, int W, int C, int x_cstride, int k, int stride, int pad, int OH, int OW,
                         int y_cstride, int y_coffset, fcn_stream_t s);
int  fcn_deconv_depthwise_fwd_f16(const void* x, const float* w, const float* bias, void* y, int N, int H, int W, int C, int x_cstride,
                                  int k, int stride, int pad, int OH, int OW, int y_cstride, int y_coffset, int out_f32, fcn_stream_t s);
int  fcn_eltwise_fwd_f16(const void* a, const void* b, void* y, size_t count, int op, float ca, float cb, fcn_stream_t s);
int  fcn_softmax_fwd_f16(const void* x, void* y, int pixels, int C, int x_cstride, int y_cstride, int out_f32, fcn_stream_t s);
int  fcn_copy_channels_f16(const void* src, void* dst, int pixels, int C, int src_cstride, int src_coffset, int dst_cstride,
                           int dst_coffset, fcn_stream_t s);
int  fcn_preprocess_bgr8_rois(const uint8_t* frame, int h, int w, const int32_t* h_rois, int n, void* dst, int dst_f16, int H, int W,
                              int dst_cstride, float shift, float* d_minmax, fcn_stream_t s);
int  fcn_preprocess_bgr8_batch(const uint8_t* frames, int n, int h, int w, void* dst, int dst_f16, int H, int W, int dst_cstride,
                               float shift, float* d_minmax, fcn_stream_t s);
int  fcn_preprocess_bgr8_f16(const uint8_t* frame, int h, int w, void* dst, int H, int W, int dst_cstride, float shift, float* d_minmax,
                             fcn_stream_t s);

typedef struct fcn_scene_obj {
    const uint8_t* img;
    const uint8_t* mask;
    int32_t src_h, src_w;
    int32_t flip;
    int32_t roi_x, roi_y, roi_w, roi_h;
    int32_t out_w, out_h;
    int32_t cx, cy;
    int32_t label1;
} fcn_scene_obj;
int  fcn_compose_scene_bgr8(const uint8_t* bg, int bg_h, int bg_w, int crop_x, int crop_y, int crop_w, int crop_h,
                            const fcn_scene_obj* d_objs, int nobj, int final_flip, uint8_t* out_img, uint8_t* out_mask,
                            int H, int W, fcn_stream_t s);
int  fcn_compose_scene_view_bgr8(const uint8_t* bg, int bg_h, int bg_w, int crop_x, int crop_y, int crop_w, int crop_h,
                                 const fcn_scene_obj* d_objs, int nobj, int final_flip, uint8_t* out_img, uint8_t* out_mask,
                                 int H, int W, int view_x, int view_y, int view_w, int view_h, fcn_stream_t s);

#define FCN_GAUSS_MAX_RADIUS 15
int  fcn_blur_gauss_bgr8(const uint8_t* src, uint8_t* dst, float* tmp, int h, int w, const float* h_taps, int radius, fcn_stream_t s);
int  fcn_blur_box_bgr8(const uint8_t* src, uint8_t* dst, int h, int w, int k, fcn_stream_t s);
int  fcn_blur_median_bgr8(const uint8_t* src, uint8_t* dst, int h, int w, int k, fcn_stream_t s);
typedef struct fcn_color_params {
    float sharpen_centre;
    float sharpen_off;
    int32_t add[3];
    float mul[3];
    float gray_alpha;
    float gray_keep;
} fcn_color_params;
int  fcn_color_augment_bgr8(const uint8_t* src, uint8_t* dst, int h, int w, const fcn_color_params* h_params, fcn_stream_t s);

int  fcn_mask_to_label_f32(const uint8_t* mask, int h, int w, float* dst, int H, int W, int dst_cstride, fcn_stream_t s);

#define FCN_RECT_ROUND_NEAREST_EVEN 0
#define FCN_RECT_ROUND_TRUNCATE     1
typedef struct fcn_detect_params {
    int32_t num_classes;
    int32_t gy, gx;
    int32_t cell_w, cell_h;
    int32_t cvg_cstride, cvg_coffset;
    int32_t box_cstride, box_coffset;
    float   prob_thresh;
    int32_t group_thresh;
    double  eps;
    int32_t min_height;
    int32_t round_mode;
    int32_t max_out;
} fcn_detect_params;
size_t fcn_detect_workspace_bytes(const fcn_detect_params* h_p, int batch);
int  fcn_detect_decode_group(const float* cvg, const float* bbox, int batch,
                             size_t cvg_image_stride, size_t box_image_stride,
                             const fcn_detect_params* h_p, void* d_workspace,
                             int32_t* out_rects, int32_t* out_weights,
                             int32_t* out_count, fcn_stream_t s);

size_t fcn_score_masks_workspace_bytes(int n_windows, int num_classes, int w, int h);
int  fcn_score_masks(const float* score, int N, int C, int H, int W, int cstride, int coffset, const int32_t* h_rects, float prob_thresh,
                     uint8_t* pmap, int frame_h, int frame_w, void* d_workspace, int32_t* out, fcn_stream_t s);

int  fcn_gen_targets(const int32_t* rects, const int32_t* labels, const int32_t* rect_offsets, int batch,
                     int num_classes, int gy, int gx, int stride, double iou_thresh,
                     float* foreground, float* bbox, float* size, float* obj, float* cvg_block,
                     fcn_stream_t s);
int  fcn_gen_targets_nhwc(const int32_t* rects, const int32_t* labels, const int32_t* rect_offsets, int batch,
                          int num_classes, int gy, int gx, int stride, double iou_thresh,
                          float* foreground, int fg_cstride, float* bbox, float* size, float* obj, float* cvg_block,
                          int blk_cstride, fcn_stream_t s);

size_t fcn_conv2d_wgrad_workspace_floats(const fcn_conv_desc* h_d, int* h_splits);
int  fcn_conv2d_wgrad_f32(const fcn_conv_desc* h_d, float* dw, float* db, float* d_workspace, fcn_stream_t s);
size_t fcn_conv2d_wgrad_group_workspace_floats(const fcn_conv_desc* h_ds, int n);
int  fcn_conv2d_wgrad_group_f32(const fcn_conv_desc* h_ds, float* const* h_dws, float* const* h_dbs, int n, float* d_workspace,
                                fcn_stream_t s);
int  fcn_conv2d_wgrad_num_configs(void);
int  fcn_conv2d_wgrad_split_config(void);
size_t fcn_conv2d_wgrad_workspace_floats_cfg(const fcn_conv_desc* h_d, int cfg_request, int* h_splits);
int  fcn_conv2d_wgrad_cfg_f32(const fcn_conv_desc* h_d, float* dw, float* db, float* d_workspace, int cfg_request, fcn_stream_t s);
size_t fcn_conv2d_wgrad_group_workspace_floats_cfg(const fcn_conv_desc* h_ds, int n, int cfg_request);
int  fcn_conv2d_wgrad_group_cfg_f32(const fcn_conv_desc* h_ds, float* const* h_dws, float* const* h_dbs, int n, float* d_workspace,
                                    int cfg_request, fcn_stream_t s);
int  fcn_conv_weights_flip_f32(const float* w, float* wt, int Cout, int kh, int kw, int Cin, int Cin4, int Cout4, fcn_stream_t s);
typedef struct fcn_flip_seg { uint64_t w_offset, wt_offset; int32_t Cout, kh, kw, Cin, Cin4, Cout4; } fcn_flip_seg;
int  fcn_conv_weights_flip_batch_f32(const float* w_base, float* wt_base, const fcn_flip_seg* d_segs, int nseg, fcn_stream_t s);
int  fcn_relu_bwd_f32(const float* dy, const float* y, float* dx, int pixels, int C, int cstride, fcn_stream_t s);
// ... 236 lines not shown
```

Baseline: 4581 frames/s.

## Add chained persistent conv kernel where each workgroup processes several tiles back to back

Adds a chained variant of the K-split 32x32 grouped conv kernel. Each workgroup walks several consecutive tiles, and its loader waves prefetch the next tile's operands into the LDS ring while the compute waves finish the current one. The chain length is tuned per layer group by timing concurrent streams at the frames-in-flight depth, and a chain is kept only when it beats the single-tile launch by a margin. This targets per-tile prologue and epilogue bubbles and the cost of oversubscribed launches, at the price of fewer workgroups, more code and longer tuning.

```diff
diff --git a/fcn_object_detector_amd/csrc/conv_fwd.hip b/fcn_object_detector_amd/csrc/conv_fwd.hip
--- a/fcn_object_detector_amd/csrc/conv_fwd.hip
+++ b/fcn_object_detector_amd/csrc/conv_fwd.hip
@@ -989,6 +989,496 @@
     conv_body<T, WTM, WTN, WAVES_M, WAVES_N, WAVES_K, BK, NBUF, PF>(p, blockIdx.x, smem);
 }
 
+typedef const GroupArgs __attribute__((address_space(4))) * group_kptr;
+
+__device__ __forceinline__ int chain_fetch(group_kptr ka, const int (&head)[1 + kMaxGroup], const int tile, ConvP& prob) {
+    typedef unsigned u32x16 __attribute__((ext_vector_type(16)));
+    typedef unsigned u32x8 __attribute__((ext_vector_type(8)));
+    int pi = 0, begin = 0;
+#pragma unroll
+    for (int i = 0; i < kMaxGroup - 1; ++i) {
+        const int end_i = head[1 + i];
+        const bool past = i + 1 < head[0] && tile >= end_i;
+        pi += past ? 1 : 0;
+        begin = past ? end_i : begin;
+    }
+    u32x16 ra, rb;
+    u32x8 rc;
+    pi = __builtin_amdgcn_readfirstlane(pi);
+    begin = __builtin_amdgcn_readfirstlane(begin);
+    const ConvP __attribute__((address_space(4)))* pbase = &ka->p[pi];
+    asm volatile("s_load_dwordx16 %0, %3, 0x0\n\ts_load_dwordx16 %1, %3, 0x40\n\ts_load_dwordx8 %2, %3, 0x80\n\ts_waitcnt lgkmcnt(0)"
+                 : "=&s"(ra), "=&s"(rb), "=&s"(rc)
+                 : "s"(pbase)
+                 : "memory");
+    __builtin_memcpy((char*)&prob, &ra, 64);
+    __builtin_memcpy((char*)&prob + 64, &rb, 64);
+    __builtin_memcpy((char*)&prob + 128, &rc, 32);
+    return tile - begin;
+}
+
+template <int WAVES_K, int BK, int NBUF_>
+__device__ __forceinline__ void conv_chain_body(group_kptr ka, const int (&head)[1 + kMaxGroup], const int tile0, const int ntiles, float* smem) {
+    using C = Cfg<1, 1, 1, 1, WAVES_K, BK, NBUF_, true>;
+    static_assert(C::ROLES && C::LOADX == 1 && C::NBUF == 4 && C::NW == 4 && C::KS == 1 && C::BUF_FLOATS == 2048 && C::NW * 64 == C::BM * C::BN / 4,
+                  "the chained form is written for the 32 x 32 K-split shape: two parked waves per ring slot, one float4 of the tile per multiplying thread");
+    constexpr int NBUF = C::NBUF, D = C::D, INST = C::INST, KS = C::KS, BUF_FLOATS = C::BUF_FLOATS;
+    constexpr int BM = C::BM, SEGS = C::SEGS, RPI = C::RPI, STEP = C::STEP, IA = C::IA, IB = C::IB;
+    constexpr int EPS = 4, BKE = BK, ESZ = 4, MPS = 4;
+    const int tid = threadIdx.x;
+    const int lane = tid & 63;
+    const int wid_all = __builtin_amdgcn_readfirstlane(tid >> 6);
+    auto next = [](int b) { return b + 1 == NBUF ? 0 : b + 1; };
+
+    if (wid_all >= C::NW) {
+        const int wid = wid_all - C::NW;
+        const int lrow = RPI * wid + lane / SEGS;
+        const int lseg = (lane % SEGS) ^ swz<SEGS>(lrow);
+        const int lane_c = lseg * EPS;
+        const int lds_wave_base = RPI * wid * BK;
+        constexpr int OOB = (int)0x80000000u;
+        ConvP p;
+        int kind = 0, ne = D;
+        int a_iy0[IA], a_ix0[IA], a_off[IA], a_vo[IA], b_vo[IB];
+        unsigned long long xa_bits = 0;
+        int xa_bytes = 0;
+        __amdgpu_buffer_rsrc_t rw = __builtin_amdgcn_make_buffer_rsrc(smem, 0, 0, 0x00020000);
+        auto rsrc_x = [&]() {
+            const unsigned lo = __builtin_amdgcn_readfirstlane((unsigned)xa_bits), hi = __builtin_amdgcn_readfirstlane((unsigned)(xa_bits >> 32));
+            return __builtin_amdgcn_make_buffer_rsrc(reinterpret_cast<float*>(((unsigned long long)hi << 32) | lo), 0,
+                                                     __builtin_amdgcn_readfirstlane(xa_bytes), 0x00020000);
+        };
+        float* dst = smem;
+        unsigned okmask[IA];
+        int a_vb[IA], a_cur[IA], a_next[IA], b_last[IB], b_cur[IB], b_tap[IB];
+        bool lane_in_rem = false, partial = false;
+        int cpt = 1, s_j = 0, s_kq = -1, s_aoff = 0, s_boff = 0, s_tapb = 0, s_left = 0, s_dq = 0, s_dr = 0, tap_off = 0;
+        unsigned s_nbit = 0u;
+        int l_kr = 0, l_kq = 0, l_kc = 0, l_koff = 0, l_kb = 0, l_left = 0;
+        bool cvalid = false;
+        int kc = 0, kt = 0, bk_taps = 0, bk_rem = 0, kb = 0, taps = 1;
+        int b_off[IB];
+        const float* zero_page = nullptr;
+#pragma unroll
+        for (int i = 0; i < IA; ++i) { a_iy0[i] = a_ix0[i] = a_off[i] = a_vo[i] = a_vb[i] = a_cur[i] = a_next[i] = 0; okmask[i] = 0u; }
+#pragma unroll
+        for (int i = 0; i < IB; ++i) b_vo[i] = b_last[i] = b_cur[i] = b_tap[i] = b_off[i] = 0;
+
+        auto tap_advance = [&]() {
+            const bool live = s_left > 0;
+            s_left -= live ? 1 : 0;
+            ++s_kq;
+            const bool wq = s_kq == p.kw;
+            s_kq = wq ? 0 : s_kq;
+            tap_off += wq ? s_dr : s_dq;
+            s_aoff = tap_off;
+            s_tapb += p.Cin * ESZ;
+            s_boff = s_tapb;
+            s_j = live ? cpt : 0x7fffffff;
+            s_nbit = s_left > 0 ? s_nbit << 1 : 0u;
+#pragma unroll
+            for (int i = 0; i < IA; ++i) {
+                a_cur[i] = a_next[i];
+                a_next[i] = (okmask[i] & s_nbit) != 0 ? a_vb[i] : OOB;
+            }
+#pragma unroll
+            for (int i = 0; i < IB; ++i) b_cur[i] = live ? b_tap[i] : OOB;
+        };
+        auto setup = [&](const int tilepos) {
+            const int tile = chain_fetch(ka, head, tilepos, p);
+            const float* px = p.x;
+            const float* pw = p.w;
+            const int tile_m = fast_div(tile, p.tiles_n_magic);
+            const int tile_n = tile - tile_m * p.tiles_n;
+            const int m0 = tile_m * BM, n0 = tile_n * C::BN;
+#pragma unroll
+            for (int i = 0; i < IA; ++i) {
+                const int m = m0 + STEP * i + lrow;
+                const bool ok = m < p.M;
+                const int mm = ok ? m : 0;
+                const int t = fast_div(mm, p.ow_magic);
+                const int ox = mm - t * p.OW;
+                const int img = fast_div(t, p.oh_magic);
+                const int oy = t - img * p.OH;
+                a_iy0[i] = ok ? oy * p.stride - p.pad : -(1 << 20);
+                a_ix0[i] = ox * p.stride - p.pad;
+                a_off[i] = ((img * p.H + a_iy0[i]) * p.W + a_ix0[i]) * p.x_cstride;
+            }
+            taps = p.kh * p.kw;
+            const bool lean = p.lean_chunks > 0;
+            const int nchunks = lean ? p.lean_chunks : (p.K + BKE - 1) / BKE;
+            ne = nchunks > D ? nchunks : D;
+            kind = !lean ? 2 : p.kw_magic == -1 ? 0 : 1;
+            if (lean) {
+                rw = __builtin_amdgcn_make_buffer_rsrc(const_cast<float*>(pw), 0, p.Cout * p.K * ESZ, 0x00020000);
+#pragma unroll
+                for (int i = 0; i < IA; ++i) a_vo[i] = (a_off[i] + lane_c) * ESZ;
+#pragma unroll
+                for (int i = 0; i < IB; ++i) {
+                    const int n = n0 + STEP * i + lrow;
+                    b_vo[i] = n < p.Cout ? (n * p.K + lane_c) * ESZ : OOB;
+                }
+                const int xbytes = (int)((((long long)p.N * p.H * p.W - 1) * p.x_cstride + p.Cin) * ESZ);
+                if (kind == 0) {
+                    cpt = (p.Cin + BKE - 1) / BKE;
+                    const int rem = p.Cin - (cpt - 1) * BKE;
+                    partial = rem != BKE;
+                    const int bias = (p.pad * p.W + p.pad) * p.x_cstride * ESZ;
+                    xa_bits = reinterpret_cast<unsigned long long>(px - bias / ESZ);
+                    xa_bytes = xbytes + bias;
+                    unsigned row_bits = 0;
+                    for (int r = 0; r < p.kh; ++r) row_bits |= 1u << (r * p.kw);
+#pragma unroll
+                    for (int i = 0; i < IA; ++i) {
+                        a_vb[i] = a_vo[i] + bias;
+                        if (taps == 1) {
+                            okmask[i] = (unsigned)((int)((unsigned)a_iy0[i] < (unsigned)p.H) & (int)((unsigned)a_ix0[i] < (unsigned)p.W));
+                        } else {
+                            const int lo_r = min(max(-a_iy0[i], 0), p.kh), hi_r = min(max(p.H - a_iy0[i], 0), p.kh);
+                            const int lo_q = min(max(-a_ix0[i], 0), p.kw), hi_q = min(max(p.W - a_ix0[i], 0), p.kw);
+                            const unsigned rows = row_bits & (((1u << (max(hi_r - lo_r, 0) * p.kw)) - 1u) << (lo_r * p.kw));
+                            const unsigned cols = ((1u << max(hi_q - lo_q, 0)) - 1u) << lo_q;
+                            okmask[i] = rows * cols;
+                        }
+                    }
+                    lane_in_rem = lane_c < rem;
+                    const bool last_always = partial && cpt == 1;
+#pragma unroll
+                    for (int i = 0; i < IB; ++i) {
+                        b_last[i] = lane_in_rem ? b_vo[i] : OOB;
+                        b_tap[i] = last_always ? b_last[i] : b_vo[i];
+                    }
+                    if (last_always) {
+#pragma unroll
+                        for (int i = 0; i < IA; ++i) okmask[i] = lane_in_rem ? okmask[i] : 0u;
+                    }
+                    s_j = 0; s_kq = -1; s_aoff = 0; s_boff = 0; s_tapb = -p.Cin * ESZ; s_left = taps;
+                    s_nbit = 1u;
+                    s_dq = p.x_cstride * ESZ;
+                    s_dr = (p.W - p.kw + 1) * p.x_cstride * ESZ;
+                    tap_off = -s_dq;
+#pragma unroll
+                    for (int i = 0; i < IA; ++i) a_next[i] = (okmask[i] & s_nbit) != 0 ? a_vb[i] : OOB;
+                    tap_advance();
+                } else {
+                    xa_bits = reinterpret_cast<unsigned long long>(px);
+                    xa_bytes = xbytes;
+                    l_kr = l_kq = l_kc = l_koff = l_kb = 0;
+                    l_left = nchunks;
+                }
+            } else {
+                kc = lseg * EPS;
+                kt = (int)(((unsigned)kc * p.cin_magic24) >> 24);
+                kc -= kt * p.Cin;
+                bk_taps = (int)(((unsigned)BKE * p.cin_magic24) >> 24);
+                bk_rem = BKE - bk_taps * p.Cin;
+#pragma unroll
+                for (int i = 0; i < IB; ++i) {
+                    const int n = n0 + STEP * i + lrow;
+                    b_off[i] = n < p.Cout ? n * p.K + lseg * EPS : -1;
+                }
+                kb = lseg * EPS;
+                unsigned long long zp_bits = reinterpret_cast<unsigned long long>(p.zero_page);
+                asm volatile("" : "+v"(zp_bits));
+                zero_page = reinterpret_cast<const float*>(zp_bits);
+            }
+        };
+        auto issue_light = [&](const int buf) {
+            dst = smem + buf * BUF_FLOATS + lds_wave_base;
+#if defined(__HIP_DEVICE_COMPILE__)
+            const __amdgpu_buffer_rsrc_t rxa = rsrc_x();
+#pragma unroll
+            for (int i = 0; i < IA; ++i) __builtin_amdgcn_raw_ptr_buffer_load_lds(rxa, (lds_ptr)(dst + STEP * i * BK), 16, a_cur[i], s_aoff, 0, 0);
+#pragma unroll
+            for (int i = 0; i < IB; ++i) __builtin_amdgcn_raw_ptr_buffer_load_lds(rw, (lds_ptr)(dst + (BM + STEP * i) * BK), 16, b_cur[i], s_boff, 0, 0);
+#endif
+            s_aoff += BKE * ESZ;
+            s_boff += BKE * ESZ;
+            --s_j;
+            if (__builtin_expect(s_j <= 1, 0)) {
+                if (s_j == 0) {
+                    tap_advance();
+                } else if (partial) {
+#pragma unroll
+                    for (int i = 0; i < IA; ++i) a_cur[i] = lane_in_rem ? a_cur[i] : OOB;
+#pragma unroll
+                    for (int i = 0; i < IB; ++i) b_cur[i] = b_last[i];
+                }
+            }
+        };
+        auto issue_lean = [&](const int buf) {
+            const int thr = l_left > 0 ? p.Cin - l_kc : 0;
+            cvalid = lane_c < thr;
+            dst = smem + buf * BUF_FLOATS + lds_wave_base;
+            const __amdgpu_buffer_rsrc_t rxa = rsrc_x();
+#pragma unroll
+            for (int i = 0; i < IA; ++i) {
+                const bool ok = (int)cvalid & (int)((unsigned)(a_iy0[i] + l_kr) < (unsigned)p.H) & (int)((unsigned)(a_ix0[i] + l_kq) < (unsigned)p.W);
+                int vo = ok ? a_vo[i] + l_koff : OOB;
+                asm volatile("" : "+v"(vo));
+                __builtin_amdgcn_raw_ptr_buffer_load_lds(rxa, (lds_ptr)(dst + STEP * i * BK), 16, vo, 0, 0, 0);
+            }
+#pragma unroll
+            for (int i = 0; i < IB; ++i) {
+                int vo = cvalid ? b_vo[i] + l_kb : OOB;
+                asm volatile("" : "+v"(vo));
+                __builtin_amdgcn_raw_ptr_buffer_load_lds(rw, (lds_ptr)(dst + (BM + STEP * i) * BK), 16, vo, 0, 0, 0);
+            }
+            --l_left;
+            const bool nt = l_kc + BKE >= p.Cin;
+            l_kb += (nt ? p.Cin - l_kc : BKE) * ESZ;
+            const int kq1 = l_kq + (nt ? 1 : 0);
+            const bool wq = kq1 == p.kw;
+            l_kq = wq ? 0 : kq1;
+            l_kr += wq ? 1 : 0;
+            l_kc = nt ? 0 : l_kc + BKE;
+            l_koff = nt ? (l_kr * p.W + l_kq) * p.x_cstride * ESZ : l_koff + BKE * ESZ;
+        };
+        auto issue_lane = [&](const int buf) {
+            const int is_kr = (kt * p.kw_magic) >> 16;
+            const int is_kq = kt - is_kr * p.kw;
+            const int is_koff = (is_kr * p.W + is_kq) * p.x_cstride + kc;
+            const bool is_kok = kt < taps, is_kbok = kb < p.K;
+            dst = smem + buf * BUF_FLOATS + lds_wave_base;
+#pragma unroll
+            for (int i = 0; i < IA; ++i) {
+                const bool ok = (int)is_kok & (int)((unsigned)(a_iy0[i] + is_kr) < (unsigned)p.H) & (int)((unsigned)(a_ix0[i] + is_kq) < (unsigned)p.W);
+                unsigned long long src = ok ? reinterpret_cast<unsigned long long>(p.x + (a_off[i] + is_koff)) : reinterpret_cast<unsigned long long>(zero_page);
+                asm volatile("" : "+v"(src));
+                __builtin_amdgcn_global_load_lds((gvoid_cptr)src, (lds_ptr)(dst + STEP * i * BK), 16, 0, 0);
+            }
+#pragma unroll
+            for (int i = 0; i < IB; ++i) {
+                unsigned long long src = ((int)is_kbok & (int)(b_off[i] >= 0)) ? reinterpret_cast<unsigned long long>(p.w + b_off[i])
+                                                                               : reinterpret_cast<unsigned long long>(zero_page);
+                asm volatile("" : "+v"(src));
+                __builtin_amdgcn_global_load_lds((gvoid_cptr)src, (lds_ptr)(dst + (BM + STEP * i) * BK), 16, 0, 0);
+                b_off[i] += b_off[i] >= 0 ? BKE : 0;
+            }
+            kb += BKE;
+            kc += bk_rem;
+            kt += bk_taps;
+            const bool wrap = kc >= p.Cin;
+            kc -= wrap ? p.Cin : 0;
+            kt += wrap ? 1 : 0;
+        };
+        auto issue_any = [&](const int buf) {
+            if (kind == 0) issue_light(buf);
+            else if (kind == 1) issue_lean(buf);
+            else issue_lane(buf);
+        };
+        int buf_issue = 0;
+        auto steady = [&](auto& issue) {
+#pragma unroll 1
+            for (int c = -1; c < ne - 3; ++c) {
+                wait_vmcnt<INST>();
+                __builtin_amdgcn_s_barrier();
+                asm volatile("" ::: "memory");
+                issue(buf_issue);
+                buf_issue = next(buf_issue);
+            }
+        };
+        setup(tile0);
+        issue_any(0);
+        issue_any(1);
+        buf_issue = 2;
+#pragma unroll 1
+        for (int t = 0; t < ntiles; ++t) {
+            if (kind == 0) steady(issue_light);
+            else if (kind == 1) steady(issue_lean);
+            else steady(issue_lane);
+            const bool more = t + 1 < ntiles;
+            if (more) setup(tile0 + t + 1);
+            wait_vmcnt<INST>();
+            __builtin_amdgcn_s_barrier();
+            asm volatile("" ::: "memory");
+            if (more) issue_any(buf_issue);
+            buf_issue = next(buf_issue);
+            if (more) wait_vmcnt<INST>();
+            else wait_vmcnt<0>();
+            __builtin_amdgcn_s_barrier();
+            asm volatile("" ::: "memory");
+            if (more) issue_any(buf_issue);
+            buf_issue = next(buf_issue);
+            __builtin_amdgcn_s_barrier();
+            __builtin_amdgcn_s_barrier();
+            __builtin_amdgcn_s_barrier();
+            asm volatile("" ::: "memory");
+        }
+        return;
+    }
+
+    const int wk = wid_all;
+    const int fswz = swz<SEGS>(lane & 31);
+    const unsigned lds0 = (unsigned)(size_t)(lds_ptr)smem;
+    const int slot4 = ((2 * wk + (lane >> 5)) ^ fswz) * 4;
+    const unsigned fa = lds0 + 4u * ((lane & 31) * BK + slot4);
+    const unsigned fb = lds0 + 4u * ((BM + (lane & 31)) * BK + slot4);
+    v4f af[2], bf[2];
+    auto ds_read = [](v4f& dst, unsigned addr, auto off) {
+        asm volatile("ds_read_b128 %0, %1 offset:%2" : "=v"(dst) : "v"(addr), "n"(decltype(off)::value));
+    };
+    auto frags_landed = [&](const int par) {
+        asm volatile("s_waitcnt lgkmcnt(0)" ::: "memory");
+        asm volatile("" : "+v"(af[par]));
+        asm volatile("" : "+v"(bf[par]));
+        __builtin_amdgcn_sched_barrier(0);
+    };
+    f32x16 acc;
+#pragma unroll
+    for (int r = 0; r < 16; ++r) acc[r] = 0.f;
+    auto iteration = [&](auto u_c) {
+        constexpr int u = decltype(u_c)::value;
+        __builtin_amdgcn_s_barrier();
+        asm volatile("" ::: "memory");
+        frags_landed(u & 1);
+        constexpr int SB = ((u + 1) % NBUF) * BUF_FLOATS * 4;
+#pragma unroll
+        for (int g = 0; g < KS * MPS; ++g) {
+            acc = __builtin_amdgcn_mfma_f32_32x32x2f32(af[u & 1][g], bf[u & 1][g], acc, 0, 0, 0);
+            __builtin_amdgcn_sched_barrier(0);
+            if (g == 0) {
+                ds_read(af[(u + 1) & 1], fa, std::integral_constant<int, SB>{});
+                ds_read(bf[(u + 1) & 1], fb, std::integral_constant<int, SB>{});
+            }
+            __builtin_amdgcn_sched_barrier(0);
+        }
+    };
+    const int c4 = tid & 7, it = tid >> 3;
+    int ph = 0;
+#pragma unroll 1
+    for (int t = 0; t < ntiles; ++t) {
+        ConvP p;
+        const int tile = chain_fetch(ka, head, tile0 + t, p);
+        const int tile_m = fast_div(tile, p.tiles_n_magic);
+        const int tile_n = tile - tile_m * p.tiles_n;
+        const int m0 = tile_m * BM, n0 = tile_n * C::BN;
+        const int nchunks = p.lean_chunks > 0 ? p.lean_chunks : (p.K + BKE - 1) / BKE;
+        const int ne = nchunks > D ? nchunks : D;
+        const int n = n0 + 4 * c4;
+        float bias_v[4];
+#pragma unroll
+        for (int e = 0; e < 4; ++e)
+            bias_v[e] = p.bias ? *(const float __attribute__((address_space(1)))*)(p.bias + (n + e < p.Cout ? n + e : p.Cout - 1)) : 0.f;
+
+        __builtin_amdgcn_s_barrier();
+        asm volatile("" ::: "memory");
+        {
+            const unsigned sb = (unsigned)ph * (BUF_FLOATS * 4);
+            if (ph & 1) {
+                ds_read(af[1], fa + sb, std::integral_constant<int, 0>{});
+                ds_read(bf[1], fb + sb, std::integral_constant<int, 0>{});
+            } else {
+                ds_read(af[0], fa + sb, std::integral_constant<int, 0>{});
+                ds_read(bf[0], fb + sb, std::integral_constant<int, 0>{});
+            }
+        }
+        int c = 0;
+        if (ph != 0) {
+            if (ph <= 1 && c < ne) { iteration(std::integral_constant<int, 1>{}); ++c; }
+            if (ph <= 2 && c < ne) { iteration(std::integral_constant<int, 2>{}); ++c; }
+            if (c < ne) { iteration(std::integral_constant<int, 3>{}); ++c; }
+        }
+        while (c < ne) {
+            iteration(std::integral_constant<int, 0>{}); ++c;
+            if (c < ne) { iteration(std::integral_constant<int, 1>{}); ++c; }
+            if (c < ne) { iteration(std::integral_constant<int, 2>{}); ++c; }
+            if (c < ne) { iteration(std::integral_constant<int, 3>{}); ++c; }
+        }
+        frags_landed(0);
+        frags_landed(1);
+        __builtin_amdgcn_s_barrier();
+        asm volatile("" ::: "memory");
+        __builtin_amdgcn_sched_barrier(0);
+
+        const int phe = (ph + ne) & 3;
+        auto parked = [&](const int w) { return smem + ((phe + 2 + (w >> 1)) & 3) * BUF_FLOATS + (w & 1) * 1024; };
+        {
+            float* slab = parked(wk) + (lane >> 5) * 128 + (lane & 31);
+#pragma unroll
+            for (int r = 0; r < 16; ++r) slab[((r & 3) + 8 * (r >> 2)) * 32] = acc[r];
+#pragma unroll
+            for (int r = 0; r < 16; ++r) acc[r] = 0.f;
+        }
+        asm volatile("s_waitcnt lgkmcnt(0)" ::: "memory");
+        __builtin_amdgcn_s_barrier();
+        asm volatile("" ::: "memory");
+        const int m = m0 + it;
+        if (m < p.M && n < p.Cout) {
+            const bool do_relu = (p.flags & FCN_CONV_RELU) != 0;
+            const bool do_sig2 = (p.flags & FCN_CONV_SIGMOID2) != 0 && p.y2 != nullptr;
+            const bool do_mask = (p.flags & FCN_CONV_MASK) != 0 && p.y2 != nullptr;
+            const bool do_accum = (p.flags & FCN_CONV_ACCUM) != 0;
+            const bool vec = n + 3 < p.Cout && ((p.y_cstride | p.y_coffset) & 3) == 0 && ((p.y2_cstride | p.y2_coffset) & 3) == 0 &&
+                             ((unsigned)(size_t)p.y & 15) == 0 && ((unsigned)(size_t)p.y2 & 15) == 0;
+            const int lo = it * 32 + 4 * c4;
+            v4f v = *(const v4f*)(parked(0) + lo);
+#pragma unroll
+            for (int s = 1; s < WAVES_K; ++s) v += *(const v4f*)(parked(s) + lo);
+#pragma unroll
+            for (int e = 0; e < 4; ++e) v[e] += bias_v[e];
+            const size_t o = (size_t)m * p.y_cstride + p.y_coffset + n;
+            const size_t o2 = (size_t)m * p.y2_cstride + p.y2_coffset + n;
+            if (vec) {
+                float* dst = p.y + o;
+                if (do_accum) v += *(const v4f*)dst;
+                if (do_relu) for (int e = 0; e < 4; ++e) v[e] = fmaxf(v[e], 0.f);
+                if (do_mask) { const v4f a = *(const v4f*)(p.y2 + o2); for (int e = 0; e < 4; ++e) v[e] = a[e] > 0.f ? v[e] : 0.f; }
+                *(v4f*)dst = v;
+                if (do_sig2) {
+                    v4f sg;
+                    for (int e = 0; e < 4; ++e) sg[e] = 1.f / (1.f + expf(-v[e]));
+                    *(v4f*)(p.y2 + o2) = sg;
+                }
+            } else {
+                for (int e = 0; e < 4; ++e)
+                    if (n + e < p.Cout) {
+                        float tv = v[e];
+                        if (do_accum) tv += p.y[o + e];
+                        if (do_relu) tv = fmaxf(tv, 0.f);
+                        if (do_mask) tv = p.y2[o2 + e] > 0.f ? tv : 0.f;
+                        p.y[o + e] = tv;
+                        if (do_sig2) p.y2[o2 + e] = 1.f / (1.f + expf(-tv));
+                    }
+            }
+        }
+        asm volatile("s_waitcnt lgkmcnt(0)" ::: "memory");
+        ph = phe;
+    }
+}
+
+template <int WAVES_K, int BK, int NBUF>
+__global__ __launch_bounds__((Cfg<1, 1, 1, 1, WAVES_K, BK, NBUF, true>::NT)) __attribute__((amdgpu_waves_per_eu(8, 8))) void conv_fwd_group_chain(const int nprob, const int te0, const int te1, const int te2,
+                                                                                      const int te3, const int te4, const int te5, const int te6,
+                                                                                      const int te7, const int pool_wgs, const int snake, const int chain,
+                                                                                      const GroupArgs a) {
+    using C = Cfg<1, 1, 1, 1, WAVES_K, BK, NBUF, true>;
+    __shared__ __attribute__((aligned(16))) float smem[C::RING_FLOATS];
+    constexpr size_t kArgsOffset = (12 * sizeof(int) + alignof(GroupArgs) - 1) / alignof(GroupArgs) * alignof(GroupArgs);
+    group_kptr ka = (group_kptr)((const char __attribute__((address_space(4)))*)__builtin_amdgcn_kernarg_segment_ptr() + kArgsOffset);
+    const int head[1 + kMaxGroup] = {nprob, te0, te1, te2, te3, te4, te5, te6, te7};
+    if ((int)blockIdx.x < pool_wgs) {
+        const int w = (int)blockIdx.x;
+        if (w < a.pool[0].wg_end) pool_body<float, C::NT>(a.pool[0], w);
+        else pool_body<float, C::NT>(a.pool[1], w - a.pool[0].wg_end);
+        return;
+    }
+    int pos = blockIdx.x;
+    if (snake > 0) {
+        const int sh = snake & 255, rounds = snake >> 8;
+        const int r = pos >> sh, j = pos & ((1 << sh) - 1);
+        if (r > 0 && r < rounds - 1 && ((rounds - 1 - r) & 1)) pos = (r << sh) + ((1 << sh) - 1 - j);
+    }
+    int cpos = pos - pool_wgs;
+    if (snake < 0) {
+        cpos += snake;
+        cpos += cpos < 0 ? (int)gridDim.x - pool_wgs : 0;
+    }
+    const int tile0 = cpos * chain;
+    const int left = te7 - tile0;
+    conv_chain_body<WAVES_K, BK, NBUF>(ka, head, tile0, left < chain ? left : chain, smem);
+}
+
 constexpr int kD7Th = 8, kD7Tw = 32;
 constexpr int kD7Ph = 2 * kD7Th + 5, kD7Pw = 2 * kD7Tw + 6;
 constexpr int kD7RowF = kD7Pw * 3;
@@ -1852,8 +2342,25 @@
     }
 }
 
+constexpr bool chain_cfg_ok(int cfg) { return cfg == 23; }
+constexpr int kMaxChain = 8;
+void launch_group_chain(int cfg, const GroupArgs& ga, int pool_wgs, int snake, int chain, int total, hipStream_t st) {
+    switch (cfg) {
+    case 23:
+        hipLaunchKernelGGL((conv_fwd_group_chain<4, 32, 16 + 4>), dim3(total), dim3(Cfg<1, 1, 1, 1, 4, 32, 16 + 4, true>::NT), 0, st, ga.nprob,
+                           ga.tile_end[0], ga.tile_end[1], ga.tile_end[2], ga.tile_end[3], ga.tile_end[4], ga.tile_end[5], ga.tile_end[6],
+                           ga.tile_end[7], pool_wgs, snake, chain, ga);
+        break;
+    }
+}
+int forced_chain() {
+    const char* e = getenv("FCN_CONV_CHAIN");
+    const int v = e ? atoi(e) : 0;
+    return v < 1 ? 0 : v > kMaxChain ? kMaxChain : v;
+}
+
 struct HostTail { bool on; int finalize; int n; fcn_conv_desc heads[kTailMaxSlices]; float* scratch; unsigned* arrive; TailP t; };
-struct HostGroup { int n; ConvP ps[16]; int npool; PoolP pools[kMaxPool]; HostTail tail; };
+struct HostGroup { int n; ConvP ps[16]; int npool; PoolP pools[kMaxPool]; HostTail tail; int chain; };
 std::unordered_map<const void*, HostTail> g_tails;
 std::mutex g_groups_mu;
 std::unordered_map<const void*, HostGroup> g_groups;
@@ -2003,6 +2510,7 @@
                 cfg, kFirst7Cfg, kDot1x1Cfg);
     FCN_REQUIRE(total > 0, FCN_E_UNSUPPORTED, "conv group: too many tiles for the 32-bit tile decode");
     FCN_HIP(hipMemcpy(d_workspace, ps, sizeof(ConvP) * n, hipMemcpyHostToDevice));
+    const int chain = chain_cfg_ok(cfg) && !group_f16 && !tail.on && forced_chain() > 1 ? forced_chain() : 0;
     {
         std::lock_guard<std::mutex> lock(g_groups_mu);
         HostGroup& hg = g_groups[d_workspace];
@@ -2011,11 +2519,31 @@
         hg.npool = npools;
         for (int i = 0; i < kMaxPool; ++i) hg.pools[i] = pools[i];
         hg.tail = tail;
+        hg.chain = chain;
     }
     h_out->d_probs = d_workspace;
     h_out->n = n;
     h_out->cfg = cfg;
     h_out->total_tiles = total;
+    h_out->chain = chain;
+    return 0;
+}
+
+int fcn_conv2d_config_chain_lds_bytes(int cfg) {
+    return cfg >= 0 && cfg < kNumTileCfg && chain_cfg_ok(cfg) ? Cfg<1, 1, 1, 1, 4, 32, 16 + 4, true>::RING_FLOATS * 4 : -1;
+}
+
+int fcn_conv2d_group_set_chain(fcn_conv_group* g, int chain) {
+    FCN_REQUIRE(g && g->d_probs, FCN_E_ARG, "fcn_conv2d_group_set_chain: unprepared group");
+    FCN_REQUIRE(chain >= 1 && chain <= kMaxChain, FCN_E_ARG, "fcn_conv2d_group_set_chain: chain length %d outside 1..%d", chain, kMaxChain);
+    std::lock_guard<std::mutex> lock(g_groups_mu);
+    auto it = g_groups.find(g->d_probs);
+    FCN_REQUIRE(it != g_groups.end() && it->second.n == g->n, FCN_E_STATE, "fcn_conv2d_group_set_chain: group was not prepared by this library instance");
+    HostGroup& hg = it->second;
+    FCN_REQUIRE(chain_cfg_ok(g->cfg) && !(hg.ps[0].flags & FCN_CONV_F16) && !hg.tail.on, FCN_E_UNSUPPORTED,
+                "fcn_conv2d_group_set_chain: only float32 groups without a tail under a split-role 32 x 32 K-split configuration (23) have a chained form");
+    hg.chain = chain;
+    g->chain = chain;
     return 0;
 }
 
@@ -2144,7 +2672,9 @@
             ga.p[i] = src;
             ga.tile_end[i] = src.tile_end - base;
         }
-        int grid = ga.tile_end[ga.nprob - 1];
+        static const bool pool_last_exp = getenv("FCN_POOL_LAST") && atoi(getenv("FCN_POOL_LAST")) == 1;
+        const int chain = hg.chain > 1 && chain_cfg_ok(g->cfg) && !hg.tail.on && !(hg.ps[0].flags & FCN_CONV_F16) && !pool_last_exp ? hg.chain : 1;
+        int grid = (ga.tile_end[ga.nprob - 1] + chain - 1) / chain;
         int pool_wgs = 0;
         if (hg.npool > 0) {
             int end = 0;
@@ -2167,7 +2697,7 @@
                 int sh = 0;
                 while ((1 << sh) < cus) ++sh;
                 snake = ((grid + cus - 1) / cus) << 8 | sh;
-            } else if (getenv("FCN_CONV_XCD") && atoi(getenv("FCN_CONV_XCD")) == 1 && pool_wgs == 0 && first == 0 && hg.n <= kMaxGroup) {
+            } else if (chain == 1 && getenv("FCN_CONV_XCD") && atoi(getenv("FCN_CONV_XCD")) == 1 && pool_wgs == 0 && first == 0 && hg.n <= kMaxGroup) {
                 snake = (int)0x80000000;
             } else if (snake_ok && ga.nprob > 1 && pool_wgs == 0 && grid > cus && grid <= 2 * cus) {
                 snake = -(grid - cus);
@@ -2179,7 +2709,8 @@
             gt.g = ga;
             gt.tail = hg.tail.t;
             launch_group_tail(g->cfg, gt, pool_wgs, snake, grid, as_stream(s));
-        } else if (hg.ps[0].flags & FCN_CONV_F16) launch_group_cfg<f16_t>(g->cfg, ga, pool_wgs, snake, grid, as_stream(s));
+        } else if (chain > 1) launch_group_chain(g->cfg, ga, pool_wgs, snake, chain, grid, as_stream(s));
+        else if (hg.ps[0].flags & FCN_CONV_F16) launch_group_cfg<f16_t>(g->cfg, ga, pool_wgs, snake, grid, as_stream(s));
         else launch_group_cfg<float>(g->cfg, ga, pool_wgs, snake, grid, as_stream(s));
         FCN_LAUNCH_CHECK("conv_fwd_group");
     }
diff --git a/fcn_object_detector_amd/detector.py b/fcn_object_detector_amd/detector.py
--- a/fcn_object_detector_amd/detector.py
+++ b/fcn_object_detector_amd/detector.py
@@ -438,7 +438,7 @@
     def __init__(self, make_engine, depth: int = 3, **detector_kw):
         self.detectors: List[FCNObjectDetector] = []
         first = None
-        with replica_streams():
+        with replica_streams(max(int(depth), 1)):
             for _ in range(max(int(depth), 1)):
                 eng = make_engine(first)
                 first = first or eng
diff --git a/fcn_object_detector_amd/engine.py b/fcn_object_detector_amd/engine.py
--- a/fcn_object_detector_amd/engine.py
+++ b/fcn_object_detector_amd/engine.py
@@ -29,13 +29,16 @@
 
 class replica_streams:
 
+    def __init__(self, depth: int = 1):
+        self.depth = int(depth)
+
     def __enter__(self) -> "replica_streams":
-        self._outer = getattr(_replica_ctx, "next", None)
-        _replica_ctx.next = 0
+        self._outer = (getattr(_replica_ctx, "next", None), getattr(_replica_ctx, "depth", None))
+        _replica_ctx.next, _replica_ctx.depth = 0, self.depth
         return self
 
     def __exit__(self, *exc) -> None:
-        _replica_ctx.next = self._outer
+        _replica_ctx.next, _replica_ctx.depth = self._outer
 
 
 def _take_replica_index() -> Optional[int]:
@@ -295,7 +298,8 @@
                  params: Optional[Dict[str, List[np.ndarray]]] = None, device: int = 0,
                  fuse: bool = True, group_convs: bool = True, autotune: bool = True, dtype: str = "f32",
                  tune_from: Optional["Engine"] = None, tune_max_lds_kb: Optional[int] = None,
-                 share_params: Optional["Engine"] = None, score_outputs: bool = False, replica: Optional[int] = None):
+                 share_params: Optional["Engine"] = None, score_outputs: bool = False, replica: Optional[int] = None,
+                 in_flight: Optional[int] = None):
         if dtype not in ("f32", "f16"):
             raise ValueError("dtype must be 'f32' or 'f16'")
         if share_params is not None and (dtype != "f32" or share_params.f16):
@@ -313,6 +317,7 @@
         self.fuse = fuse
         self.group_convs = group_convs
         self.autotune = autotune
+        self.in_flight = max(int(in_flight if in_flight is not None else getattr(_replica_ctx, "depth", None) or 1), 1)
         L.call("fcn_init", device)
         sp = C.c_void_p()
         self.replica = replica if replica is not None else _take_replica_index()
@@ -991,8 +996,14 @@
         cfg = self.tuner.conv_cfg(tune_key, arr, len(chunk), ws, parr, len(fused)) if self.autotune else -1
         L.call("fcn_conv2d_group_prepare_fused", arr, len(chunk), parr, len(fused), ws.ptr, cfg, C.byref(grp))
         self._keep.extend([arr, parr, ws, grp])
+        if (self.autotune and self.in_flight > 1 and not self.f16 and self.spec.phase == "TEST" and not tailed and grp.chain == 0
+                and os.environ.get("FCN_TUNE_CHAIN", "0") == "1" and "FCN_CONV_CHAIN" not in os.environ
+                and int(lib.fcn_conv2d_config_chain_lds_bytes(grp.cfg)) >= 0):
+            chain = self.tuner.conv_chain(tune_key, arr, len(chunk), parr, len(fused), grp.cfg, self.in_flight)
+            if chain > 1:
+                L.call("fcn_conv2d_group_set_chain", C.byref(grp), chain)
         kind = "conv_group" if len(chunk) > 1 else "conv"
-        label = "%s [cfg%d %dwg]" % (name, grp.cfg, grp.total_tiles)
+        label = "%s [cfg%d %dwg%s]" % (name, grp.cfg, grp.total_tiles, " x%d" % grp.chain if grp.chain > 1 else "")
         if fused:
             label = "%s {+%s}" % (label, "+".join(pt.layer.name for pt in fused))
             byts += sum(pt.ops[0].bytes for pt in fused)
@@ -2002,6 +2013,7 @@
             max_lds_kb = int(os.environ["FCN_PIPE_LDS_KB"]) or None
         if max_lds_kb is not None:
             engine_kw.setdefault("tune_max_lds_kb", max_lds_kb)
+        engine_kw.setdefault("in_flight", depth)
         for i in range(depth):
             self.engines.append(Engine(make_spec(), params=params, device=device, tune_from=self.engines[0] if i else None, replica=i,
                                        **engine_kw))
diff --git a/fcn_object_detector_amd/lib.py b/fcn_object_detector_amd/lib.py
--- a/fcn_object_detector_amd/lib.py
+++ b/fcn_object_detector_amd/lib.py
@@ -35,7 +35,7 @@
 
 
 class ConvGroup(C.Structure):
-    _fields_ = [("d_probs", C.c_void_p), ("n", C.c_int32), ("cfg", C.c_int32), ("total_tiles", C.c_int32)]
+    _fields_ = [("d_probs", C.c_void_p), ("n", C.c_int32), ("cfg", C.c_int32), ("total_tiles", C.c_int32), ("chain", C.c_int32)]
 
 
 class TConvDesc(C.Structure):
@@ -205,6 +205,8 @@
     "fcn_conv2d_first_layer_config": (_i, []),
     "fcn_conv2d_config_lds_bytes": (_i, [_i]),
     "fcn_conv2d_config_waves_k": (_i, [_i]),
+    "fcn_conv2d_group_set_chain": (_i, [C.POINTER(ConvGroup), _i]),
+    "fcn_conv2d_config_chain_lds_bytes": (_i, [_i]),
     "fcn_conv2d_group_prepare": (_i, [C.POINTER(ConvDesc), _i, _vp, _i, C.POINTER(ConvGroup)]),
     "fcn_conv2d_group_prepare_fused": (_i, [C.POINTER(ConvDesc), _i, C.POINTER(PoolDesc), _i, _vp, _i, C.POINTER(ConvGroup)]),
     "fcn_conv2d_fwd_group_f32": (_i, [C.POINTER(ConvGroup), _vp]),
diff --git a/fcn_object_detector_amd/tune.py b/fcn_object_detector_amd/tune.py
--- a/fcn_object_detector_amd/tune.py
+++ b/fcn_object_detector_amd/tune.py
@@ -32,6 +32,12 @@
 WGRAD = Protocol(warm=2, reps=5, evict=False, samples=1, stat=min, contenders=3, margin=1.04, look=4, carry=True)
 
 FLUSH_BYTES = 64 << 20
+
+CHAIN_LENGTHS = (1, 2, 3, 4)
+CHAIN_SAMPLES = 9
+CHAIN_REPS = 4
+CHAIN_GATE_PASSES = 8
+CHAIN_MARGIN = 0.90
 
 
 def set_partitions(n: int) -> Iterable[List[int]]:
@@ -152,6 +158,93 @@
             L.call("fcn_conv2d_group_release", ws.ptr)
             ws.free()
 
+    def time_conv_chains(self, arr, n: int, parr, npool: int, cfg: int, depth: int) -> Dict[int, float]:
+        lib = L.load()
+        keep: List["E.DeviceBuffer"] = []
+        streams: List[C.c_void_p] = []
+        events: List[C.c_void_p] = []
+        groups = []
+
+        def private(nbytes: int) -> int:
+            keep.append(E.DeviceBuffer(max(int(nbytes), 16), zero=False))
+            return keep[-1].ptr
+
+        try:
+            for k in range(depth):
+                descs = (L.ConvDesc * n)()
+                for i in range(n):
+                    C.memmove(C.byref(descs[i]), C.byref(arr[i]), C.sizeof(L.ConvDesc))
+                    d = descs[i]
+                    if k:
+                        d.y = private(4 * d.N * d.OH * d.OW * d.y_cstride)
+                        if d.y2 and d.flags & L.CONV_SIGMOID2:
+                            d.y2 = private(4 * d.N * d.OH * d.OW * d.y2_cstride)
+                pools = (L.PoolDesc * max(npool, 1))()
+                for i in range(npool):
+                    C.memmove(C.byref(pools[i]), C.byref(parr[i]), C.sizeof(L.PoolDesc))
+                    q = pools[i]
+                    if k:
+                        q.y = private(4 * q.N * q.OH * q.OW * q.y_cstride)
+                        if q.idx:
+                            q.idx = private(4 * q.N * q.OH * q.OW * q.C)
+                ws = E.DeviceBuffer(int(lib.fcn_conv2d_group_workspace_bytes(n)), zero=False)
+                grp = L.ConvGroup()
+                groups.append((descs, pools, ws, grp))
+                L.call("fcn_conv2d_group_prepare_fused", descs, n, pools, npool, ws.ptr, cfg, C.byref(grp))
+                if lib.fcn_conv2d_group_set_chain(C.byref(grp), 1) != 0:
+                    return {}
+                sp, ev = C.c_void_p(), C.c_void_p()
+                L.call("fcn_stream_create", C.byref(sp))
+                streams.append(sp)
+                L.call("fcn_event_create", C.byref(ev))
+                events.append(ev)
+            if self.flush is None:
+                self.flush = E.DeviceBuffer(FLUSH_BYTES, zero=False)
+            for _ in range(2):
+                ev = C.c_void_p()
+                L.call("fcn_event_create", C.byref(ev))
+                events.append(ev)
+            gate, done = events[depth], events[depth + 1]
+
+            def one_round() -> float:
+                for _ in range(CHAIN_GATE_PASSES):
+                    L.call("fcn_memset_async", self.flush.ptr, 0, self.flush.nbytes, self.stream)
+                L.call("fcn_event_record", gate, self.stream)
+                for k in range(depth):
+                    L.call("fcn_stream_wait_event", streams[k], gate)
+                for _ in range(CHAIN_REPS):
+                    for k in range(depth):
+                        L.check(lib.fcn_conv2d_fwd_group_f32(C.byref(groups[k][3]), streams[k]))
+                for k in range(depth):
+                    L.call("fcn_event_record", events[k], streams[k])
+                    L.call("fcn_stream_wait_event", self.stream, events[k])
+                L.call("fcn_event_record", done, self.stream)
+                L.call("fcn_event_sync", done)
+                ms = C.c_float()
+                L.call("fcn_event_elapsed_ms", gate, done, C.byref(ms))
+                return ms.value / CHAIN_REPS
+
+            out: Dict[int, float] = {}
+            self.chain_samples: Dict[int, List[float]] = {}
+            for chain in CHAIN_LENGTHS:
+                for _, _, _, grp in groups:
+                    L.call("fcn_conv2d_group_set_chain", C.byref(grp), chain)
+                one_round()
+                self.chain_samples[chain] = [one_round() for _ in range(CHAIN_SAMPLES)]
+                out[chain] = lower_quartile(self.chain_samples[chain])
+            return out
+        finally:
+            for sp in streams:
+                L.call("fcn_stream_sync", sp)
+                L.call("fcn_stream_destroy", sp)
+            for ev in events:
+                L.call("fcn_event_destroy", ev)
+            for _, _, ws, _ in groups:
+                L.call("fcn_conv2d_group_release", ws.ptr)
+                ws.free()
+            for b in keep:
+                b.free()
+
     def choose(self, key: str, valid: Callable[[object], bool], search: Callable[[], object]):
         for known in (self.tune_from, self.cache):
             if known is not None and valid(known.get(key)):
@@ -177,6 +270,19 @@
         return self.choose(self.key(name), self._valid_cfg(int(L.load().fcn_conv2d_num_configs())),
                            lambda: self.time_conv_cfgs(arr, n, ws, parr, npool)[0])
 
+    @staticmethod
+    def pick_chain(ms: Dict[int, float], margin: float = CHAIN_MARGIN) -> int:
+        if 1 not in ms:
+            return 1
+        best = min(ms, key=lambda c: (ms[c], c))
+        return best if best > 1 and ms[best] <= margin * ms[1] else 1
+
+    def conv_chain(self, name: str, arr, n: int, parr, npool: int, cfg: int, depth: int) -> int:
+        if depth < 2:
+            return 1
+        return self.choose("chain:" + self.key(name) + "|x%d" % depth, lambda v: type(v) is int and 1 <= v <= 8,
+                           lambda: self.pick_chain(self.time_conv_chains(arr, n, parr, npool, cfg, depth)))
+
     def wgrad_cfgs(self, ops: Sequence["E.Op"]) -> None:
         ncfg = int(L.load().fcn_conv2d_wgrad_num_configs())
         for op in ops:
diff --git a/include/fcnhip.h b/include/fcnhip.h
--- a/include/fcnhip.h
+++ b/include/fcnhip.h
@@ -89,6 +89,7 @@
     int32_t n;
     int32_t cfg;
     int32_t total_tiles;
+    int32_t chain;
 } fcn_conv_group;
 size_t fcn_conv2d_group_workspace_bytes(int n);
 int  fcn_conv2d_num_configs(void);
@@ -105,6 +106,8 @@
 int  fcn_conv2d_group_attach_tail(void* d_workspace, const fcn_conv_tail* t);
 int  fcn_conv2d_config_lds_bytes(int cfg);
 int  fcn_conv2d_config_waves_k(int cfg);
+int  fcn_conv2d_group_set_chain(fcn_conv_group* h_group, int chain);
+int  fcn_conv2d_config_chain_lds_bytes(int cfg);
 int  fcn_conv2d_group_prepare(const fcn_conv_desc* h_descs, int n, void* d_workspace, int cfg_request, fcn_conv_group* h_out);
 int  fcn_conv2d_fwd_group_f32(const fcn_conv_group* h_group, fcn_stream_t s);
 typedef struct fcn_pool_desc {
```

Result: slower. 4524 frames/s (-1.2%).
